# MartinPippel/DAmar

Measured on AMD Instinct MI355X. Metric: aligned base-pairs/sec (daligner block-vs-block), higher is better.
Workload: dtype int32

## Files before the change

damar_amd/csrc/kernels/kernels.h:

```cpp
#ifndef DAMAR_KERNELS_H
#define DAMAR_KERNELS_H

#include "dev_common.h"

size_t damar_scan_workspace_bytes(u64 n);
void   damar_exclusive_scan_u32(const u32 *in, u32 *out, u64 n, void *work, u64 *total_dev, hipStream_t st);
#define DAMAR_SCAN_TILE 4096
void   damar_tile_offsets_u32(const u32 *in, u64 n, void *work, u64 *total_dev, hipStream_t st);
void   damar_scan_tile_counts(u32 *tcount, u32 ntiles, u64 *total_dev, hipStream_t st);
size_t damar_sort_workspace_bytes(u64 n);
void   damar_sort_set_threads(int threads);
const u32 *damar_sort_error_word(const void *work);
int    damar_radix_sort_keys_u64(u64 *k0, u64 *k1, u64 n, int lobit, int hibit, void *work, hipStream_t st);
void   damar_radix_sort_split_u64(u64 *k0, u64 *k1, u64 n, int lobit, int hibit, u32 *ohi, u32 *olo, void *work,
                                  hipStream_t st);
int    damar_radix_sort_u32(u32 *k0, u32 *v0, u32 *k1, u32 *v1, u64 n, int nbits, void *work, hipStream_t st);
int    damar_radix_sort_keys_u32(u32 *k0, u32 *k1, u64 n, int nbits, void *work, hipStream_t st);
int    damar_radix_sort_u64(u64 *k0, u32 *v0, u64 *k1, u32 *v1, u64 n, int nbits, void *work, hipStream_t st);

typedef struct
{ const u8  *bases;
  const u32 *pk;
  u32        rbias;
  const u32 *boff;
  const u32 *coarse;
  u32        nreads;
  u32        total;
  int        maxlen;
  int        rpbits;
  const u32 *moff;
  const int *mdat;
} DevBlock;

#define SEED_PRIO_VAR(name, dflt) static __device__ int name = dflt;  static int name##_host = dflt;
#define SEED_PRIO(name)     do { if (name) __builtin_amdgcn_s_setprio(3); } while (0)
#define SEED_PRIO_SETTER(fn, name) \
  void fn(int on) { if (on != name##_host) { HIP_CHECK(hipMemcpyToSymbol(HIP_SYMBOL(name), &on, sizeof(int)));  name##_host = on; } }

#define COARSE_SHIFT 9
#define PK_PAD 4

#ifdef __HIPCC__
__device__ __forceinline__ u32 read_of_pos(const DevBlock &b, u32 p)
{ u32 r = b.coarse[p >> COARSE_SHIFT];
  while (b.boff[r + 1] <= p)
    r += 1;
  return r;
}
__device__ __forceinline__ void pos_decode(const DevBlock &b, u32 v, u32 *r, u32 *x)
{ if (b.rpbits)
    { *r = v >> b.rpbits;
      *x = v & ((1u << b.rpbits) - 1u);
    }
  else
    { const u32 rr = read_of_pos(b, v);
      *r = rr;
      *x = v - b.boff[rr];
    }
}
__device__ __forceinline__ u32 pos_encode(const DevBlock &b, u32 r, u32 x, u32 p)
{ return b.rpbits ? ((r << b.rpbits) | x) : p; }
#endif

long long damar_pack_words(u32 total);
void damar_launch_pack_bases(const u8 *bases, u32 total, u32 *pk, hipStream_t st);
void damar_launch_unpack_bps(const u8 *raw, const u32 *foff, const DevBlock *blk, int comp, u8 *bases, hipStream_t st);

void damar_preload_index(void);  void damar_preload_scan(void);  void damar_preload_sort(void);
void damar_preload_merge(void);  void damar_preload_report(void);
void damar_sort_set_prio(int on);
void damar_merge_set_prio(int on);
void damar_index_set_prio(int on);
void damar_launch_kmer_tuples(const DevBlock *blk, int kmer, u32 nkmers, void *codes, int wide, u32 *pos, hipStream_t st);
void damar_launch_mask_flags(const DevBlock *blk, int kmer, const u32 *pos, u32 n, u32 *keep, hipStream_t st);
void damar_launch_biased_tuples(const DevBlock *blk, int kmer, const int *logbase, void *codes, int wide, u32 *pos,
                                u32 *keep, hipStream_t st);
void damar_launch_suppress_flags(const void *codes, int wide, u32 n, int suppress, u32 *keep, hipStream_t st);
void damar_launch_compact_pairs(const void *k, int wide, const u32 *v, const u32 *keep, const u32 *off, u32 n,
                                void *ko, u32 *vo, hipStream_t st);

void damar_launch_tandem_links(const DevBlock *blk, int kmer, const void *codes, int wide, const u32 *pos, u32 n,
                               int *dist, hipStream_t st);

typedef struct
{ const void *acode;  const u32 *apos;  u32 alen;
  const void *bcode;  const u32 *bpos;  u32 blen;
  int  wide;
  int  kbits;
  int  self, comp, identity;
  u32  limit;
  DevBlock ablk, bblk;
  int  pbits, abits;
  int  dbits;
} MergeArgs;

typedef struct { u32 b0, b1, ja, ia;
                 u32 sh, pad[3]; } MergeTile;

size_t damar_merge_workspace_bytes(u32 alen);
u32   *damar_merge_tile_counts(void *work, u32 alen);
u32    damar_merge_tiles(u32 alen);
void   damar_launch_merge_count(const MergeArgs *m, void *work, unsigned long long *gram, u32 ngram, hipStream_t st);
void damar_launch_merge_emit(const MergeArgs *m, void *work, u64 nhits, u64 *keys, u32 *vals, u32 *pid, hipStream_t st);
void damar_launch_pair_heads_ids(const u32 *pids, u64 nhits, int abits, int minhit, int nshift,
                                 u64 *send, u64 *bits, void *scan_work, u64 *total_dev, u32 *heads, hipStream_t st);
void damar_launch_pair_bitmap(const u32 *pids, const u32 *heads, u32 nheads, int abits, u32 b_lo, u32 b_hi, u32 *bitmap,
                              hipStream_t st);
void damar_launch_seed_cut_count(const u64 *keys, u64 nhits, int pbits, const u32 *bitmap, u32 *tcount, u64 *total_dev,
                                 hipStream_t st);
void damar_launch_seed_cut_scatter(const u64 *keys, const u32 *vals, u64 nhits, int pbits, const u32 *bitmap,
                                   const u32 *toff, u64 *okeys, u32 *ovals, hipStream_t st);
void damar_launch_pair_heads(const u64 *keys, u64 nhits, int pbits, int abits, int minhit, int nshift,
                             u64 *send , u64 *bits, void *scan_work, u64 *total_dev,
                             u32 *heads, hipStream_t st);
void damar_launch_pair_work(u64 *keys, const u32 *vals, u64 nhits, int ppos, int dbits, int abits, int minhit, int nshift,
                            u64 *send , u64 *bits, void *scan_work, u64 *total_dev ,
                            int binshift, int kmer, int hitmin, u32 b_lo, u32 b_hi, int unsorted, hipStream_t st);
void damar_launch_order_runs(u64 *keys, u64 nhits, int ppos, int dbits, const u32 *work, u32 nwork, hipStream_t st);
void damar_launch_pair_work_expand(const u64 *bits, const void *scan_work, u64 nhits, u32 *work, hipStream_t st);
#define WORK_COST_BITS 16
#define WORK_COST_MAX  ((1u << WORK_COST_BITS) - 1)
void damar_launch_work_cost(const u64 *keys, const u32 *vals, u64 nhits, int pbits, int abits, int dbits, const u32 *aboff,
                            const u32 *bboff, const u32 *work, u32 nwork, u32 coarse, u32 *key, u32 *val, hipStream_t st);
void damar_launch_pair_screen(const u64 *keys, const u32 *vals, u64 nhits, int pbits, int dbits, const u32 *heads, u32 nheads,
                              int minhit, int binshift, int kmer, int hitmin, int abits, u32 b_lo, u32 b_hi, u32 *keep, hipStream_t st);
void damar_launch_compact_u32(const u32 *src, const u32 *keep, const u32 *off, u32 n, u32 *out, hipStream_t st);
void damar_launch_compact_index(const u32 *flags, const u32 *off, u64 n, u32 *out, hipStream_t st);

#ifdef __HIPCC__
__device__ __forceinline__ int seed_diag(u64 k, const u32 *__restrict__ vals, u64 i, u64 pmask, int dbits)
{ if (dbits)
    return (int) ((k >> dbits) & pmask) - (int) (k & ((1ull << dbits) - 1));
  return (int) vals[i];
}
#endif

typedef struct
{ int abpos, bbpos, aepos, bepos, diffs;
  int atlen, btlen;
  int aread, bread;
  u32 item, seq;
  u32 toff;
} LaRecord;

typedef struct
{
  const u64 *keys;  const u32 *vals;  u64 nhits;
  const u32 *work;  u32 nwork;
  DevBlock ablk, bblk;
  int  pbits, abits, dbits;
  int  kmer, hitmin, binshift, minhit;
  int  comp, self, symmetric, minover, hgap_min;
  int  tspace, ave_path, reach;
  const short *score, *table;
  int  mscore, dscore;
  void *state;   u64 state_stride;   int span;
  int  *marks;   u64 marks_stride;
  void *cells;   u32 cell_cap;
  int  *buckets; u64 bucket_stride;  int bwidth;
  int  bucket_bits;
  u16  *ttmp;    u32 ttmp_stride;
  LaRecord *recs;  u32 rec_cap;
  u16  *tpool;     u32 tpool_cap;
  u32  *widemap;
  void *wcells;    u32 wcell_cap;
  u32  cell_max;
  int  t8, t8max;
  const u32 *order;
  u32  *counters;
  u32  *cursor;
  u32  *nfilt;
  int   job;
} ReportArgs;

#define DAMAR_MAX_JOBS 32
#define DAMAR_MAX_TSPACE 8192
#define DAMAR_CNT_CELLS     8
#define DAMAR_CNT_HALFSTEPS 10
#define DAMAR_CNT_ITERS     12
#define DAMAR_CNT_WIDE    14
#define DAMAR_ITEM_WIDE   0x80000000u
#define DAMAR_CNT_CURSOR  16
#define DAMAR_CNT_NFILT   (DAMAR_CNT_CURSOR + DAMAR_MAX_JOBS)
#define DAMAR_COUNTER_WORDS (DAMAR_CNT_NFILT + DAMAR_MAX_JOBS)
#define DAMAR_SEQ_BITS 24

#define DAMAR_ERR_CELLS   1u
#define DAMAR_ERR_RECS    2u
#define DAMAR_ERR_TPOOL   4u
#define DAMAR_ERR_BAND    8u
#define DAMAR_ERR_T8     32u
#define DAMAR_ERR_WIDE   16u

int  damar_report_waves_per_simd(void);
int  damar_report2_waves_per_simd(void);
int  damar_report2_slots_per_wave(void);
void damar_launch_report(const ReportArgs *jobs, int njobs, int nslots, hipStream_t st);
void damar_launch_report_wide(const ReportArgs *jobs, int njobs, int nslots, hipStream_t st);
void damar_launch_tandem_report(const ReportArgs *a, const int *dist, int nslots, hipStream_t st);

typedef struct { int aread, bread, diag, anti; } LaTask;
void damar_launch_la_batch(const ReportArgs *a, const LaTask *tasks, u32 ntasks, int nslots, hipStream_t st);
void damar_launch_report2(const ReportArgs *jobs, int njobs, const LaTask *tasks, u32 ntasks, int nslots, hipStream_t st);
void damar_launch_tandem_report2(const ReportArgs *a, const int *dist, int nslots, hipStream_t st);
void damar_launch_tandem_report_wide(const ReportArgs *a, const int *dist, int nslots, hipStream_t st);
void damar_launch_la_batch_wide(const ReportArgs *a, const LaTask *tasks, u32 ntasks, int nslots, hipStream_t st);
#define DAMAR_MAX_MARKS 16000
#define DAMAR_MAX_CELLS (1u << 18)

u64 damar_report_state_stride(int span);

typedef struct
{ u32 aread, bread;
  u32 flags;
  int abpos, bbpos, aepos, bepos;
  u32 poff;
  int tlen;
  u32 seg0;
  u32 stage0;
  int dmax;
  u32 slots;
} TraceRecIn;

typedef struct
{ u32 apos, bpos;
  int a0, b0;
  u32 mn;
  u32 flags;
  u32 stage;
  u32 rec;
} TraceSeg;

typedef struct
{ const TraceSeg *segs;
  const u32 *list;  u32 nwork;
  const u8 *abases, *bbases;
  const u32 *apk, *bpk;
  short *vf;  signed char *hf;  u32 cap;
  int *stage;  u32 *count;  int *dist;
  int *mid;
  u32 *over;  u32 over_cap;  u32 *nover;  u32 *need;  u32 *err;
  u32 *next;
} TraceArgs;

#define DAMAR_TRACE_ERR_POINTS 1u
#define DAMAR_TRACE_ERR_ALIGN  2u
#define DAMAR_TRACE_ERR_INTERNAL 4u

void damar_launch_trace_layout(const TraceRecIn *recs, u32 nrecs, const void *pts, int tbytes, int tspace,
                               const DevBlock *ablk, const DevBlock *bblk, TraceSeg *segs, u32 *key, u32 *val, u32 *err,
                               hipStream_t st);
void damar_launch_trace_waves(const TraceArgs *t, int mode, int kind, u32 nblocks, hipStream_t st);
size_t damar_trace_slot_area_cells(void);
size_t damar_trace_slot_vf_bytes(int mode, int kind);
void damar_launch_trace_waves_slots(const TraceArgs *t, int mode, int kind, u32 nblocks, hipStream_t st);
void damar_launch_trace_gather(const TraceRecIn *recs, u32 nrecs, int mid, const u32 *count, const int *dist, u32 *segoff,
                               u32 *tlen, int *diffs, hipStream_t st);
void damar_launch_trace_mid_layout(const TraceRecIn *recs, u32 nrecs, const TraceSeg *segs, const int *mid,
                                   const DevBlock *ablk, const DevBlock *bblk, TraceSeg *out, u32 *key, u32 *val, u32 *err,
                                   hipStream_t st);
void damar_launch_trace_pack(const TraceSeg *segs, u32 nsegs, const u32 *count, const u32 *segoff, const u32 *recoff,
                             const int *stage, int *script, hipStream_t st);
#endif
```

damar_amd/csrc/kernels/kmer_index.hip:

```cpp
#include "dev_common.h"
#include "kernels.h"

SEED_PRIO_VAR(g_index_prio, 0)
SEED_PRIO_SETTER(damar_index_set_prio, g_index_prio)


template <typename CodeT, bool PACK>
__global__ __launch_bounds__(256)
void kmer_tuples(DevBlock blk, int kmer, u32 nkmers, CodeT *__restrict__ codes, u32 *__restrict__ pos)
{ SEED_PRIO(g_index_prio);
  const u32 p = blockIdx.x * 256u + threadIdx.x;
  if (p >= blk.total)
    return;
  const u32 r = read_of_pos(blk, p), b0 = blk.boff[r];
  if (p - b0 < (u32) (kmer - 1) || p + 1 == blk.boff[r + 1])
    return;
  const u32 i = p - (r + 1) * (u32) kmer + 1;
  if (i >= nkmers)
    return;
  CodeT c = 0;
  if (PACK)
    {
      const u32 f = p - (u32) (kmer - 1), wq = f >> 4, o = (f & 15) << 1;
      u64 win = ((u64) blk.pk[wq + 1] << 32) | (u64) blk.pk[wq];
      win >>= o;
      u64 r = __brevll(win);
      r = ((r >> 1) & 0x5555555555555555ull) | ((r & 0x5555555555555555ull) << 1);
      c = (CodeT) (r >> (64 - 2 * kmer));
    }
  else
    { const u8 *s = blk.bases + (p - (u32) (kmer - 1));
      for (int j = 0; j < kmer; j++)
        c = (CodeT) (c << 2) | (CodeT) s[j];
    }
  const u32 pw = pos_encode(blk, r, p - b0, p);
  if (PACK)
    codes[i] = (CodeT) ((u64) c << 32) | (CodeT) pw;
  else
    { codes[i] = c;
      pos[i]   = pw;
    }
}

void damar_launch_kmer_tuples(const DevBlock *blk, int kmer, u32 nkmers, void *codes, int wide, u32 *pos, hipStream_t st)
{ if (nkmers == 0)
    return;
  if (wide)
    hipLaunchKernelGGL((kmer_tuples<u64, false>), dim3((blk->total + 255) / 256), dim3(256), 0, st, *blk, kmer, nkmers, (u64 *) codes, pos);
  else if (pos == NULL)
    hipLaunchKernelGGL((kmer_tuples<u64, true>), dim3((blk->total + 255) / 256), dim3(256), 0, st, *blk, kmer, nkmers, (u64 *) codes, pos);
  else
    hipLaunchKernelGGL((kmer_tuples<u32, false>), dim3((blk->total + 255) / 256), dim3(256), 0, st, *blk, kmer, nkmers, (u32 *) codes, pos);
}

__global__ __launch_bounds__(256)
void mask_flags(DevBlock blk, int kmer, const u32 *__restrict__ pos, u32 n, u32 *__restrict__ keep)
{ u32 i = blockIdx.x * 256u + threadIdx.x;
  if (i >= n)
    return;
  u32 r, x;
  pos_decode(blk, pos[i], &r, &x);
  const int e = (int) x, s = e - (kmer - 1);
  u32 lo = blk.moff[r] >> 1, hi = blk.moff[r + 1] >> 1;
  const u32 end = hi;
  while (lo < hi)
    { const u32 mid = (lo + hi) >> 1;
      if (blk.mdat[2 * mid + 1] > s) hi = mid; else lo = mid + 1;
    }
  keep[i] = (lo < end && blk.mdat[2 * lo] <= e) ? 0u : 1u;
}

void damar_launch_mask_flags(const DevBlock *blk, int kmer, const u32 *pos, u32 n, u32 *keep, hipStream_t st)
{ if (n == 0)
    return;
  hipLaunchKernelGGL(mask_flags, dim3((n + 255) / 256), dim3(256), 0, st, *blk, kmer, pos, n, keep);
}

template <typename CodeT>
__global__ __launch_bounds__(64)
void biased_tuples(DevBlock blk, int kmer, int lb0, int lb1, int lb2, int lb3,
                   CodeT *__restrict__ codes, u32 *__restrict__ pos, u32 *__restrict__ keep)
{ const u32 r = blockIdx.x * 64u + threadIdx.x;
  if (r >= blk.nreads)
    return;
  const int  LogNorm = 10000 * kmer, LogThresh = 10000 * (kmer - 2);
  const u64  kmask = (kmer == 32) ? ~0ull : ((1ull << (2 * kmer)) - 1);
  const u32  b0 = blk.boff[r];
  const int  rlen = (int) (blk.boff[r + 1] - b0) - 1;
  const u8  *s = blk.bases + b0;
  const bool masked = blk.moff != NULL;
  const u32  sb = masked ? blk.moff[r] : 0, sf = masked ? blk.moff[r + 1] : 0;
#define LB(x) ((x) == 0 ? lb0 : ((x) == 1 ? lb1 : ((x) == 2 ? lb2 : lb3)))
  for (u32 sa = sb; sa <= sf; sa += 2)
    { int p = (sa == sb) ? 0 : blk.mdat[sa - 1];
      const int q = (sa == sf) ? rlen : blk.mdat[sa];
      if (p + kmer > q)
        continue;
      u64 c = 0;
      int a = 0, k = 1;
      bool stop = false;
      while (p < q)
        { int x = s[p];
          a += LB(x);
          c = (c << 2) | (u64) x;
          while (a < LogNorm && k < kmer)
            { if (++p >= q)
                { stop = !masked;
                  break;
                }
              k += 1;
              x = s[p];
              a += LB(x);
              c = (c << 2) | (u64) x;
            }
          if (stop)
            break;
          for (;;)
            { const int u = a - LB((int) s[p - k + 1]);
              if (u < LogNorm) break;
              a = u;
              k -= 1;
            }
          if (a > LogThresh)
            { const u32 P = b0 + (u32) p;
              codes[P] = (CodeT) ((c << (2 * kmer - 2 * k)) & kmask);
              pos[P]   = pos_encode(blk, r, (u32) p, P);
              keep[P]  = 1u;
            }
          p += 1;
          a -= LB((int) s[p - k]);
        }
    }
#undef LB
}

void damar_launch_biased_tuples(const DevBlock *blk, int kmer, const int *logbase, void *codes, int wide, u32 *pos,
                                u32 *keep, hipStream_t st)
{ if (blk->nreads == 0)
    return;
  if (wide)
    hipLaunchKernelGGL(biased_tuples<u64>, dim3((blk->nreads + 63) / 64), dim3(64), 0, st, *blk, kmer,
                       logbase[0], logbase[1], logbase[2], logbase[3], (u64 *) codes, pos, keep);
  else
    hipLaunchKernelGGL(biased_tuples<u32>, dim3((blk->nreads + 63) / 64), dim3(64), 0, st, *blk, kmer,
                       logbase[0], logbase[1], logbase[2], logbase[3], (u32 *) codes, pos, keep);
}

template <typename CodeT>
__global__ __launch_bounds__(256)
void suppress_flags(const CodeT *__restrict__ codes, u32 n, u32 suppress, u32 *__restrict__ keep)
{ const u32 i = blockIdx.x * 256u + threadIdx.x;
  if (i >= n)
    return;
  const CodeT c = codes[i];
  u32 lo = i, step = 1;
  while (lo >= step && codes[lo - step] == c)
    { lo -= step;
      step <<= 1;
    }
  { u32 a = (lo >= step) ? lo - step + 1 : 0, b = lo;
    while (a < b)
      { const u32 mid = (a + b) >> 1;
        if (codes[mid] == c) b = mid; else a = mid + 1;
      }
    lo = a;
  }
  u32 hi = i;
  step = 1;
  while (hi + step < n && codes[hi + step] == c)
    { hi += step;
      step <<= 1;
    }
  { u32 a = hi, b = (hi + step < n) ? hi + step - 1 : n - 1;
    while (a < b)
      { const u32 mid = (a + b + 1) >> 1;
        if (codes[mid] == c) a = mid; else b = mid - 1;
      }
    hi = a;
  }
  keep[i] = (hi - lo + 1 < suppress) ? 1u : 0u;
}

void damar_launch_suppress_flags(const void *codes, int wide, u32 n, int suppress, u32 *keep, hipStream_t st)
{ if (n == 0)
    return;
  if (wide)
    hipLaunchKernelGGL(suppress_flags<u64>, dim3((n + 255) / 256), dim3(256), 0, st, (const u64 *) codes, n, (u32) suppress, keep);
  else
    hipLaunchKernelGGL(suppress_flags<u32>, dim3((n + 255) / 256), dim3(256), 0, st, (const u32 *) codes, n, (u32) suppress, keep);
}

template <typename CodeT>
__global__ __launch_bounds__(256)
void compact_pairs(const CodeT *__restrict__ k, const u32 *__restrict__ v, const u32 *__restrict__ keep,
                   const u32 *__restrict__ off, u32 n, CodeT *__restrict__ ko, u32 *__restrict__ vo)
{ u32 i = blockIdx.x * 256u + threadIdx.x;
  if (i < n && keep[i])
    { ko[off[i]] = k[i];
      vo[off[i]] = v[i];
    }
}

__global__ __launch_bounds__(256)
void compact_pack(const u32 *__restrict__ k, const u32 *__restrict__ v, const u32 *__restrict__ keep,
                  const u32 *__restrict__ off, u32 n, u64 *__restrict__ ko)
{ u32 i = blockIdx.x * 256u + threadIdx.x;
  if (i < n && keep[i])
    ko[off[i]] = ((u64) k[i] << 32) | (u64) v[i];
}

void damar_launch_compact_pairs(const void *k, int wide, const u32 *v, const u32 *keep, const u32 *off, u32 n,
                                void *ko, u32 *vo, hipStream_t st)
{ if (n == 0)
    return;
  if (wide)
    hipLaunchKernelGGL(compact_pairs<u64>, dim3((n + 255) / 256), dim3(256), 0, st, (const u64 *) k, v, keep, off, n, (u64 *) ko, vo);
  else if (vo == NULL)
    hipLaunchKernelGGL(compact_pack, dim3((n + 255) / 256), dim3(256), 0, st, (const u32 *) k, v, keep, off, n, (u64 *) ko);
  else
    hipLaunchKernelGGL(compact_pairs<u32>, dim3((n + 255) / 256), dim3(256), 0, st, (const u32 *) k, v, keep, off, n, (u32 *) ko, vo);
}

template <typename CodeT>
__global__ __launch_bounds__(256)
void tandem_links(DevBlock blk, int kmer, const CodeT *__restrict__ codes, const u32 *__restrict__ pos, u32 n,
                  int *__restrict__ dist)
{ u32 i = blockIdx.x * 256u + threadIdx.x;
  if (i >= n)
    return;
  u32 r, x;
  pos_decode(blk, pos[i], &r, &x);
  const u32 p = blk.boff[r] + x;
  int d = 0;
  if (i == 0)
    d = (int) codes[0];
  else if (codes[i] == codes[i - 1])
    { u32 rq, xq;
      pos_decode(blk, pos[i - 1], &rq, &xq);
      if (rq == r)
        d = (int) (x - xq);
    }
  dist[p - (r + 1) * (u32) kmer + 1] = d;
}

void damar_launch_tandem_links(const DevBlock *blk, int kmer, const void *codes, int wide, const u32 *pos, u32 n,
                               int *dist, hipStream_t st)
{ if (n == 0)
    return;
  if (wide)
    hipLaunchKernelGGL(tandem_links<u64>, dim3((n + 255) / 256), dim3(256), 0, st, *blk, kmer, (const u64 *) codes, pos, n, dist);
  else
    hipLaunchKernelGGL(tandem_links<u32>, dim3((n + 255) / 256), dim3(256), 0, st, *blk, kmer, (const u32 *) codes, pos, n, dist);
}

__global__ __launch_bounds__(256)
void pack_bases(const u8 *__restrict__ bases, long long nwords, long long total, u32 *__restrict__ pk)
{ long long w = (long long) blockIdx.x * 256 + threadIdx.x - PK_PAD;
  if (w >= nwords - PK_PAD)
    return;
  const u8 *s = bases + 16 * w;
  u32 v = 0, r = 0;
  for (int j = 0; j < 16; j++)
    { v |= (u32) (s[j] & 3) << (2 * j);
      const long long q = total - 1 - (16 * w + j);
      const u32 c = (q >= -64 && q < total + 64) ? (u32) (bases[q] & 3) : 0u;
      r |= c << (2 * j);
    }
  pk[w] = v;
  pk[nwords + w] = r;
}

__global__ __launch_bounds__(256)
void unpack_bps(const u8 *__restrict__ raw, const u32 *__restrict__ foff, DevBlock blk, int comp, u8 *__restrict__ bases)
{ const u32 p0 = (blockIdx.x * 256u + threadIdx.x) * 4u;
  if (p0 >= blk.total)
    return;
  u32 r = read_of_pos(blk, p0);
  u32 b0 = blk.boff[r], len = blk.boff[r + 1] - b0 - 1, fo = foff[r];
  u32 word = 0;
#pragma unroll
  for (int j = 0; j < 4; j++)
    { const u32 p = p0 + (u32) j;
      u32 v = 4;
      if (p < blk.total)
        { if (p >= b0 + len + 1)
            { r += 1;
              b0 = blk.boff[r];  len = blk.boff[r + 1] - b0 - 1;  fo = foff[r];
            }
          const u32 x = p - b0;
          if (x < len)
            { const u32 y = comp ? len - 1 - x : x;
              v = ((u32) raw[fo + (y >> 2)] >> (6 - 2 * (y & 3))) & 3u;
              if (comp)
                v = 3 - v;
            }
        }
      word |= v << (8 * j);
    }
  *(u32 *) (bases + p0) = word;
}

void damar_launch_unpack_bps(const u8 *raw, const u32 *foff, const DevBlock *blk, int comp, u8 *bases, hipStream_t st)
{ if (blk->total == 0)
    return;
  hipLaunchKernelGGL(unpack_bps, dim3((blk->total / 4 + 256) / 256), dim3(256), 0, st, raw, foff, *blk, comp, bases);
}

long long damar_pack_words(u32 total) { return (long long) (total >> 4) + 1 + 2 * PK_PAD; }

void damar_launch_pack_bases(const u8 *bases, u32 total, u32 *pk, hipStream_t st)
{ const long long nwords = damar_pack_words(total);
  hipLaunchKernelGGL(pack_bases, dim3((u32) ((nwords + 255) / 256)), dim3(256), 0, st, bases, nwords, (long long) total, pk);
}

void damar_preload_index(void)
{ hipFuncAttributes fa;
  (void) hipFuncGetAttributes(&fa, (const void *) pack_bases);
}
```

damar_amd/csrc/kernels/radix_sort.hip:

```cpp
#include <atomic>
#include <type_traits>
#include "dev_common.h"
#include "kernels.h"

SEED_PRIO_VAR(g_sort_prio, 1)
SEED_PRIO_SETTER(damar_sort_set_prio, g_sort_prio)

#ifndef OS_THREADS
#define OS_THREADS 1024
#endif
#ifndef OS_MINW
#define OS_MINW    4
#endif
#ifndef OS_RANK_LDS
#define OS_RANK_LDS 1
#endif
#define OS_MINTILE (256 * 8)
#define OS_MAXPASS 8

#define OH_ITEMS   16

#define LB_COUNT   1u
#define LB_PREFIX  2u
#define LB_SPINS   (1u << 24)
#ifndef LB_AHEAD
#define LB_AHEAD   8
#endif

#define WS_HIST    256
#define WS_CTR     (256 + OS_MAXPASS * 256 * 4)
#define WS_LB      16384

template <typename GT> __device__ __forceinline__ GT lb_load(const GT *p)
{ return __hip_atomic_load(p, __ATOMIC_RELAXED, __HIP_MEMORY_SCOPE_AGENT); }
template <typename GT> __device__ __forceinline__ void lb_store(GT *p, GT v)
{ __hip_atomic_store(p, v, __ATOMIC_RELAXED, __HIP_MEMORY_SCOPE_AGENT); }

__device__ __forceinline__ u32 os_scan256(u32 v, u32 *lds4)
{ const int l = lane_id(), w = threadIdx.x >> 6;
  const u32 inc = (u32) wave_incl_scan_i((int) v);
  if (l == 63 && w < 4) lds4[w] = inc;
  __syncthreads();
  u32 base = 0;
  for (int i = 0; i < 4; i++)
    if (i < w) base += lds4[i];
  __syncthreads();
  return base + inc - v;
}


#define OH_THREADS 1024
#define OH_BINMAX  61440

template <typename KeyT>
__global__ __launch_bounds__(OH_THREADS)
void onesweep_hist(const KeyT *__restrict__ keys, u64 n, int lobit, int npass, u64 dsh ,
                   u64 dwd , u32 *__restrict__ ghist, uint4 *__restrict__ clr, u64 clr16)
{ extern __shared__ u32 sh[];
  constexpr u32 nthr = OH_THREADS;
  const int nw = npass * 128 * 32;
  for (int j = threadIdx.x; j < nw; j += nthr)
    sh[j] = 0;
  __syncthreads();
  const u32 c = threadIdx.x & 31u;
  const u64 ntile = (n + (u64) nthr * OH_ITEMS - 1) / ((u64) nthr * OH_ITEMS);
  for (u64 t = blockIdx.x; t < ntile; t += gridDim.x)
    { const u64 base = t * ((u64) nthr * OH_ITEMS);
      KeyT k[OH_ITEMS];
#pragma unroll
      for (int r = 0; r < OH_ITEMS; r++)
        { const u64 i = base + (u64) r * nthr + threadIdx.x;
          k[r] = (i < n) ? keys[i] : (KeyT) 0;
        }
#pragma unroll
      for (int r = 0; r < OH_ITEMS; r++)
        { const u64 i = base + (u64) r * nthr + threadIdx.x;
          if (i < n)
            { const KeyT x = k[r] >> lobit;
              for (int p = 0; p < npass; p++)
                { const u32 d = (u32) (x >> (int) ((dsh >> (8 * p)) & 0xffu)) & (u32) ((dwd >> (8 * p)) & 0xffu);
                  atomicAdd(&sh[((u32) p << 12) + ((d >> 1) << 5) + c], 1u << ((d & 1u) << 4));
                }
            }
        }
    }
  __syncthreads();
  for (int j = threadIdx.x; j < npass * 256; j += nthr)
    { const u32 pl = (u32) j >> 8, d = (u32) j & 0xffu, sft = (d & 1u) << 4;
      u32 sum = 0;
#pragma unroll 8
      for (u32 q = 0; q < 32; q++)
        sum += (sh[(pl << 12) + ((d >> 1) << 5) + ((q + threadIdx.x) & 31u)] >> sft) & 0xffffu;
      if (sum)
        atomicAdd(&ghist[j], sum);
    }
  const uint4 z = make_uint4(0, 0, 0, 0);
  for (u64 i = (u64) blockIdx.x * nthr + threadIdx.x; i < clr16; i += (u64) gridDim.x * nthr)
    clr[i] = z;
}

#define OH_COPIES  8
template <typename KeyT>
__global__ __launch_bounds__(256)
void onesweep_hist8(const KeyT *__restrict__ keys, u64 n, int lobit, int npass, u64 dsh ,
                   u64 dwd , u32 *__restrict__ ghist, uint4 *__restrict__ clr, u64 clr16)
{ SEED_PRIO(g_sort_prio);
  extern __shared__ u32 sh[];
  const int nb = npass * 256 * OH_COPIES;
  for (int j = threadIdx.x; j < nb; j += 256)
    sh[j] = 0;
  __syncthreads();
  const u32 c = threadIdx.x & (OH_COPIES - 1);
  const u64 ntile = (n + 256 * OH_ITEMS - 1) / (256 * OH_ITEMS);
  for (u64 t = blockIdx.x; t < ntile; t += gridDim.x)
    { const u64 base = t * (256 * OH_ITEMS);
      KeyT k[OH_ITEMS];
#pragma unroll
      for (int r = 0; r < OH_ITEMS; r++)
        { const u64 i = base + (u64) r * 256 + threadIdx.x;
          k[r] = (i < n) ? keys[i] : (KeyT) 0;
        }
#pragma unroll
      for (int r = 0; r < OH_ITEMS; r++)
        { const u64 i = base + (u64) r * 256 + threadIdx.x;
          if (i < n)
            { const KeyT x = k[r] >> lobit;
              for (int p = 0; p < npass; p++)
                { const u32 d = (u32) (x >> (int) ((dsh >> (8 * p)) & 0xffu)) & (u32) ((dwd >> (8 * p)) & 0xffu);
                  atomicAdd(&sh[(((u32) p << 8) + d) * OH_COPIES + c], 1u);
                }
            }
        }
    }
  __syncthreads();
  for (int j = threadIdx.x; j < npass * 256; j += 256)
    { u32 s = 0;
#pragma unroll
      for (int q = 0; q < OH_COPIES; q++)
        s += sh[j * OH_COPIES + q];
      if (s)
        atomicAdd(&ghist[j], s);
    }
  const uint4 z = make_uint4(0, 0, 0, 0);
  for (u64 i = (u64) blockIdx.x * 256 + threadIdx.x; i < clr16; i += (u64) gridDim.x * 256)
    clr[i] = z;
}


template <typename KeyT, typename GT, bool HV, bool SPLIT, int TH, int IT>
__global__ __launch_bounds__(TH, (IT <= 8 ? 8 : OS_MINW))
void onesweep_pass(const KeyT *__restrict__ kin, const u32 *__restrict__ vin, KeyT *__restrict__ kout,
                   u32 *__restrict__ vout, u32 *__restrict__ ohi, u64 n, int shift, u32 mask,
                   const u32 *__restrict__ ghist, GT *__restrict__ lb, GT *__restrict__ lbclear,
                   u32 *__restrict__ ctr, u32 *__restrict__ err)
{ SEED_PRIO(g_sort_prio);
  constexpr int OS_TILE = TH * IT, OS_WAVES = TH / 64, OS_WSPAN = 64 * IT;
  __shared__ __attribute__((aligned(16))) KeyT skey[OS_TILE];
  u32 *const sval = (u32 *) skey;
  typedef typename std::conditional<(OS_WAVES > 8), u16, u32>::type CntT;
  __shared__ CntT cnt[OS_WAVES][256];
  __shared__ u32  dstart[256];
  __shared__ u32  gadj[256];
  __shared__ u32  lds4[4];
  __shared__ u32  s_tile;
  constexpr int SH = (int) sizeof(GT) * 8 - 2;
  constexpr GT  VM = (((GT) 1) << SH) - 1;

  const int l = lane_id(), w = threadIdx.x >> 6;
  if (threadIdx.x == 0)
    s_tile = atomicAdd(ctr, 1u);
  for (int i = 0; i < OS_WAVES; i++)
    if (threadIdx.x < 256)
      cnt[i][threadIdx.x] = 0;
#if OS_RANK_LDS
  static_assert((size_t) OS_TILE * sizeof(KeyT) >= (size_t) OS_WAVES * 256 * sizeof(u64), "the rank words do not fit the stage");
  for (int i = threadIdx.x; i < OS_WAVES * 256; i += TH)
    ((u64 *) skey)[i] = 0;
#endif
  __syncthreads();
  const u32 tile  = (u32) __builtin_amdgcn_readfirstlane((int) s_tile);
  const u64 tbase = (u64) tile * OS_TILE;
  const u32 have = (n - tbase < (u64) OS_TILE) ? (u32) (n - tbase) : (u32) OS_TILE;
  const u32 t0 = (u32) w * OS_WSPAN + (u32) l;
  const KeyT *const tin = kin + tbase;

  KeyT key[IT];
  u32  rnk[IT];
#pragma unroll
  for (int r = 0; r < IT; r++)
    { const u32 ti = t0 + (u32) r * 64;
      key[r] = tin[ti < have ? ti : have - 1];
    }
#if OS_RANK_LDS
  u64 *const wmask = (u64 *) skey + (u32) w * 256u;
  const u64 lanebit = 1ull << l;
#pragma unroll
  for (int r = 0; r < IT; r++)
    { const bool ok = t0 + (u32) r * 64 < have;
      const u32  d  = (u32) (key[r] >> shift) & mask;
      if (ok)
        __hip_atomic_fetch_or(&wmask[d], lanebit, __ATOMIC_RELAXED, __HIP_MEMORY_SCOPE_WAVEFRONT);
      __builtin_amdgcn_fence(__ATOMIC_SEQ_CST, "wavefront");
      const u64 peers  = __hip_atomic_load(&wmask[d], __ATOMIC_RELAXED, __HIP_MEMORY_SCOPE_WAVEFRONT);
      const u32 before = cnt[w][d];
      __builtin_amdgcn_fence(__ATOMIC_SEQ_CST, "wavefront");
      const u32 mine   = __builtin_amdgcn_mbcnt_hi((u32) (peers >> 32), __builtin_amdgcn_mbcnt_lo((u32) peers, 0u));
      rnk[r] = before + mine;
      if (ok && mine == 0)
        { cnt[w][d] = (CntT) (before + (u32) __popcll(peers));
          __hip_atomic_store(&wmask[d], 0ull, __ATOMIC_RELAXED, __HIP_MEMORY_SCOPE_WAVEFRONT);
        }
      __builtin_amdgcn_fence(__ATOMIC_SEQ_CST, "wavefront");
    }
#else
#pragma unroll
  for (int r = 0; r < IT; r++)
    { const bool ok = t0 + (u32) r * 64 < have;
      const u32  d  = (u32) (key[r] >> shift) & mask;
      const u64 okm = __ballot(ok);
      u32 plo = (u32) okm, phi = (u32) (okm >> 32);
#pragma unroll
      for (int b = 0; b < 8; b++)
        { const int t  = ((int) (d << (31 - b))) >> 31;
          const u64 nm = ~__ballot(t < 0);
          plo &= (u32) nm ^ (u32) t;
          phi &= (u32) (nm >> 32) ^ (u32) t;
        }
      const u32 before = cnt[w][d];
      const u32 mine   = __builtin_amdgcn_mbcnt_hi(phi, __builtin_amdgcn_mbcnt_lo(plo, 0u));
      rnk[r] = before + mine;
      if (ok && mine == 0)
        cnt[w][d] = (CntT) (before + (u32) __popc(plo) + (u32) __popc(phi));
    }
#endif
  __syncthreads();

  u32 tot = 0;
  if (threadIdx.x < 256)
    { u32 run = 0;
#pragma unroll
      for (int i = 0; i < OS_WAVES; i++)
        { const u32 c = cnt[i][threadIdx.x];
          cnt[i][threadIdx.x] = (CntT) run;
          run += c;
        }
      tot = run;
      lb_store<GT>(&lb[(u64) tile * 256 + threadIdx.x],
                   ((GT) (tile == 0 ? LB_PREFIX : LB_COUNT) << SH) | (GT) tot);
      lbclear[(u64) tile * 256 + threadIdx.x] = 0;
    }
  const u32 dbase = os_scan256(threadIdx.x < 256 ? ghist[threadIdx.x] : 0u, lds4);
  const u32 ex    = os_scan256(tot, lds4);
  if (threadIdx.x < 256)
    dstart[threadIdx.x] = ex;
  __syncthreads();

#pragma unroll
  for (int r = 0; r < IT; r++)
    { if (t0 + (u32) r * 64 < have)
        { const u32 d  = (u32) (key[r] >> shift) & mask;
          const u32 lp = dstart[d] + cnt[w][d] + rnk[r];
          rnk[r] = lp;
          skey[lp] = key[r];
        }
    }

  if (threadIdx.x < 256)
    { GT before = 0;
      if (tile > 0 && threadIdx.x <= mask)
        { u32 t = tile - 1, spins = 0;
#ifdef OS_STATS
          u32 nstep = 0;
#endif
          bool found = false;
          while (!found)
            { GT g[LB_AHEAD];
#pragma unroll
              for (int k = 0; k < LB_AHEAD; k++)
                g[k] = lb_load<GT>(&lb[(u64) (t >= (u32) k ? t - (u32) k : 0u) * 256 + threadIdx.x]);
              int used = LB_AHEAD;
#pragma unroll
              for (int k = 0; k < LB_AHEAD; k++)
                if (used == LB_AHEAD)
                  { const u32 st = (u32) (g[k] >> SH);
                    if (st == 0)
                      used = k;
                    else
                      { before += g[k] & VM;
#ifdef OS_STATS
                        nstep += 1;
#endif
                        if (st == LB_PREFIX)
                          { found = true;  used = -1; }
                      }
                  }
              if (found)
                break;
              t -= (u32) used;
              if (used < LB_AHEAD)
                { if (++spins > LB_SPINS)
                    { atomicOr(err, 1u);
                      break;
                    }
                  __builtin_amdgcn_s_sleep(1);
                }
            }
#ifdef OS_STATS
          if (threadIdx.x == 0)
            { atomicAdd(err + 1, nstep);  atomicAdd(err + 2, spins);  atomicAdd(err + 3, 1u); }
#endif
          lb_store<GT>(&lb[(u64) tile * 256 + threadIdx.x], ((GT) LB_PREFIX << SH) | ((before + tot) & VM));
        }
      gadj[threadIdx.x] = dbase + (u32) before - ex;
    }
  __syncthreads();

  u32 gdst[HV ? IT : 1];
#pragma unroll
  for (int q = 0; q < IT; q++)
    { const u32 i = threadIdx.x + (u32) q * TH;
      if (i < have)
        { const KeyT k = skey[i];
          const u32  d = (u32) (k >> shift) & mask;
          const u32  g = gadj[d] + i;
          if (HV) gdst[q] = g;
          if (SPLIT)
            { ohi[g]  = (u32) ((u64) k >> 32);
              vout[g] = (u32) k;
            }
          else
            kout[g] = k;
        }
    }
  if (HV)
    { const u32 *const tvin = vin + tbase;
      __syncthreads();
#pragma unroll
      for (int r = 0; r < IT; r++)
        { const u32 ti = t0 + (u32) r * 64;
          if (ti < have)
            sval[rnk[r]] = tvin[ti];
        }
      __syncthreads();
#pragma unroll
      for (int q = 0; q < IT; q++)
        { const u32 i = threadIdx.x + (u32) q * TH;
          if (i < have)
            vout[gdst[q]] = sval[i];
        }
    }
}


static int G_sort_threads = 0;

void damar_sort_set_threads(int threads) { G_sort_threads = (threads == 256 || threads == 512) ? threads : 1024; }

static int sort_threads(void)
{ if (G_sort_threads == 0)
    { const char *e = getenv("DAMAR_SORT_THREADS");
      damar_sort_set_threads(e ? atoi(e) : OS_THREADS);
    }
  return G_sort_threads;
}

size_t damar_sort_workspace_bytes(u64 n)
{ const u64 ntiles = (n + OS_MINTILE - 1) / OS_MINTILE;
  return (size_t) WS_LB + 2 * (((size_t) ntiles * 256 * sizeof(u64) + 255) & ~(size_t) 255) + 256;
}

const u32 *damar_sort_error_word(const void *work) { return (const u32 *) work; }

template <typename KeyT, typename GT, bool HV, int TH, int IT>
static void onesweep_passes(KeyT *k0, u32 *v0, KeyT *k1, u32 *v1, u64 n, int lobit, int hibit, u32 *ohi, u32 *olo,
                            char *ws, hipStream_t st)
{ constexpr int OS_TILE = TH * IT;
  const u32 ntiles = (u32) ((n + OS_TILE - 1) / OS_TILE);
  const int npass  = (hibit - lobit + 7) / 8;
  int dshift[OS_MAXPASS], dwidth[OS_MAXPASS];
  u64 dsh = 0, dwd = 0;
  { const int bits = hibit - lobit, base = bits / npass, extra = bits % npass;
    int at = 0;
    static int even = -1;
    if (even < 0)
      { const char *e = getenv("DAMAR_SORT_EVEN");
        even = e ? atoi(e) : 1;
      }
    for (int p = 0; p < npass; p++)
      { dshift[p] = at;
        dwidth[p] = even ? base + (p < extra ? 1 : 0) : (p < npass - 1 ? 8 : bits - 8 * (npass - 1));
        at += dwidth[p];
        dsh |= (u64) dshift[p] << (8 * p);
        dwd |= (u64) ((1u << dwidth[p]) - 1u) << (8 * p);
      }
  }
  const size_t region = ((size_t) ntiles * 256 * sizeof(GT) + 255) & ~(size_t) 255;
  u32 *err = (u32 *) ws, *ghist = (u32 *) (ws + WS_HIST), *ctr = (u32 *) (ws + WS_CTR);
  GT  *lbr[2] = { (GT *) (ws + WS_LB), (GT *) (ws + WS_LB + region) };
  HIP_CHECK(hipMemsetAsync(ws, 0, WS_LB, st));
  if (sort_threads() >= 512)
    { const u64 nt = (n + (u64) OH_THREADS * OH_ITEMS - 1) / ((u64) OH_THREADS * OH_ITEMS);
      const u64 maxit = OH_BINMAX / ((OH_THREADS / 32) * OH_ITEMS);
      u64 grid = nt < 512 ? nt : 512;
      if ((nt + grid - 1) / grid > maxit)
        grid = (nt + maxit - 1) / maxit;
      const size_t lds = (size_t) npass * 128 * 32 * sizeof(u32);
      {
        static std::atomic<unsigned long long> big_lds(0ull);
        int dev = 0;
        HIP_CHECK(hipGetDevice(&dev));
        const unsigned long long bit = 1ull << (dev & 63);
        if (!(big_lds.load(std::memory_order_acquire) & bit))
          { HIP_CHECK(hipFuncSetAttribute((const void *) onesweep_hist<u32>, hipFuncAttributeMaxDynamicSharedMemorySize, 8 * 16384));
            HIP_CHECK(hipFuncSetAttribute((const void *) onesweep_hist<u64>, hipFuncAttributeMaxDynamicSharedMemorySize, 8 * 16384));
            big_lds.fetch_or(bit, std::memory_order_release);
          }
      }
      hipLaunchKernelGGL(onesweep_hist<KeyT>, dim3((u32) grid), dim3(OH_THREADS), lds, st,
                         k0, n, lobit, npass, dsh, dwd, ghist, (uint4 *) lbr[0], (u64) (region / 16));
      HIP_CHECK(hipGetLastError());
    }
  else
    { const u64 nt = (n + 256 * OH_ITEMS - 1) / (256 * OH_ITEMS);
      const u32 grid = (u32) (nt < 2048 ? nt : 2048);
      hipLaunchKernelGGL(onesweep_hist8<KeyT>, dim3(grid), dim3(256), (size_t) npass * 256 * OH_COPIES * sizeof(u32), st,
                         k0, n, lobit, npass, dsh, dwd, ghist, (uint4 *) lbr[0], (u64) (region / 16));
    }
  for (int p = 0; p < npass; p++)
    { const int  side = p & 1;
      const bool last = (p == npass - 1);
      KeyT *ki = side ? k1 : k0, *ko = side ? k0 : k1;
      u32  *vi = side ? v1 : v0, *vo = side ? v0 : v1;
      const u32 mask = (1u << dwidth[p]) - 1u;
      if (last && ohi != NULL)
        hipLaunchKernelGGL((onesweep_pass<KeyT, GT, false, true, TH, IT>), dim3(ntiles), dim3(TH), 0, st,
                           ki, (const u32 *) NULL, (KeyT *) NULL, olo, ohi, n, lobit + dshift[p], mask,
                           ghist + 256 * p, lbr[side], lbr[side ^ 1], ctr + p, err);
      else
        hipLaunchKernelGGL((onesweep_pass<KeyT, GT, HV, false, TH, IT>), dim3(ntiles), dim3(TH), 0, st,
                           ki, vi, ko, vo, (u32 *) NULL, n, lobit + dshift[p], mask,
                           ghist + 256 * p, lbr[side], lbr[side ^ 1], ctr + p, err);
    }
}

template <typename KeyT, bool HV>
static int onesweep_impl(KeyT *k0, u32 *v0, KeyT *k1, u32 *v1, u64 n, int lobit, int hibit, u32 *ohi, u32 *olo,
                         void *work, hipStream_t st)
{ const int npass = (hibit - lobit + 7) / 8;
  if (n == 0 || npass <= 0)
    return 0;
  if (npass > OS_MAXPASS || n >= 0xfffffff0ull)
    { fprintf(stderr, "damar: internal error, radix sort of %llu items on %d bits\n", (unsigned long long) n, hibit - lobit);
      fflush(NULL);
      _exit(1);
    }
  const int shape = sort_threads();
  static int lb64 = -1;
  if (lb64 < 0)
    lb64 = getenv("DAMAR_SORT_LB64") != NULL;
  if (n < (1ull << 30) && !lb64)
    { if (shape == 1024)     onesweep_passes<KeyT, u32, HV, 1024, 8>(k0, v0, k1, v1, n, lobit, hibit, ohi, olo, (char *) work, st);
      else if (shape == 512) onesweep_passes<KeyT, u32, HV, 512, 16>(k0, v0, k1, v1, n, lobit, hibit, ohi, olo, (char *) work, st);
      else              onesweep_passes<KeyT, u32, HV, 256, 16>(k0, v0, k1, v1, n, lobit, hibit, ohi, olo, (char *) work, st);
    }
  else
    onesweep_passes<KeyT, u64, HV, 256, 16>(k0, v0, k1, v1, n, lobit, hibit, ohi, olo, (char *) work, st);
  return npass & 1;
}

int damar_radix_sort_u32(u32 *k0, u32 *v0, u32 *k1, u32 *v1, u64 n, int nbits, void *work, hipStream_t st)
{ return onesweep_impl<u32, true>(k0, v0, k1, v1, n, 0, nbits, NULL, NULL, work, st); }

int damar_radix_sort_keys_u32(u32 *k0, u32 *k1, u64 n, int nbits, void *work, hipStream_t st)
{ return onesweep_impl<u32, false>(k0, NULL, k1, NULL, n, 0, nbits, NULL, NULL, work, st); }

int damar_radix_sort_u64(u64 *k0, u32 *v0, u64 *k1, u32 *v1, u64 n, int nbits, void *work, hipStream_t st)
{ return onesweep_impl<u64, true>(k0, v0, k1, v1, n, 0, nbits, NULL, NULL, work, st); }

int damar_radix_sort_keys_u64(u64 *k0, u64 *k1, u64 n, int lobit, int hibit, void *work, hipStream_t st)
{ return onesweep_impl<u64, false>(k0, NULL, k1, NULL, n, lobit, hibit, NULL, NULL, work, st); }

void damar_radix_sort_split_u64(u64 *k0, u64 *k1, u64 n, int lobit, int hibit, u32 *ohi, u32 *olo, void *work,
                                hipStream_t st)
{ onesweep_impl<u64, false>(k0, NULL, k1, NULL, n, lobit, hibit, ohi, olo, work, st); }

void damar_preload_sort(void)
{ hipFuncAttributes fa;
  (void) hipFuncGetAttributes(&fa, (const void *) onesweep_hist<u64>);
}
```

damar_amd/csrc/kernels/seed_merge.hip:

```cpp
#include "dev_common.h"
#include "kernels.h"

SEED_PRIO_VAR(g_merge_prio, 0)
SEED_PRIO_SETTER(damar_merge_set_prio, g_merge_prio)


__device__ __forceinline__ u32 count_below(const u32 *__restrict__ bpos, u32 jb, u32 ib, u32 bound)
{ u32 a = jb, b = ib;
  while (a < b)
    { u32 m = (a + b) >> 1;
      if (bpos[m] < bound) a = m + 1; else b = m;
    }
  return a - jb;
}


#ifndef MT_PER
#define MT_PER  4
#endif
#define MT_A    (MT_PER * 256)
#define MT_BCAP (3 * MT_A)
#define MT_HITS 4
#define MT_NBK  2048

// ... 281 lines not shown
      { re[k] = (cb == NONE || cb > nat) ? nat : cb;
        if ((hbits >> k) & 1) cb = e0 + k;
      }
  }

  u32 n[MT_PER];
#pragma unroll
  for (int k = 0; k < MT_PER; k++)
    { n[k] = 0;
      if (k < nv && nb[k] > 0)
        { if (!m.self)
            { const u32 ja = rs_open[k] ? tl.ja : a0 + rs[k];
              const u32 ia = (re[k] >= nat) ? tl.ia : a0 + re[k];
              if ((u64) (ia - ja) * (u64) nb[k] < (u64) m.limit)
                n[k] = nb[k];
            }
          else
            n[k] = self_hits(m, m.apos[a0 + e0 + k], tl.b0 + jb[k], nb[k]);
        }
    }

  u64 T64;
  for (int round = 0; ; round++)
    { u32 s = 0;
      u64 s64 = 0;
#pragma unroll
      for (int k = 0; k < MT_PER; k++)
        { s += n[k];  s64 += n[k]; }
      u32 inc = (u32) wave_incl_scan_i((int) s);
      if (l == 63) sw4[w] = inc;
      __syncthreads();
      u32 ex = inc - s;
      for (int i = 0; i < 4; i++)
        if (i < w) ex += sw4[i];
      __syncthreads();
#pragma unroll
      for (int k = 0; k < MT_PER; k++)
        { loc[e0 + k] = ex;
          ex += n[k];
        }
      if (threadIdx.x == 255)
        loc[MT_A] = ex;
      T64 = block_sum_u64(s64, red);
      if (!m.self || round == 1)
        break;
      u64 xhead = 0, xtail = 0;
      if (tl.ja < a0)
        { if (threadIdx.x == 0) { sjb[0] = jb[0];  sjb[1] = nb[0]; }
          __syncthreads();
          const u32 j0 = tl.b0 + sjb[0], nn = sjb[1];
          u64 acc = 0;
          if (nn > 0)
            for (u32 i = tl.ja + threadIdx.x; i < a0; i += 256)
              acc += self_hits(m, m.apos[i], j0, nn);
          xhead = block_sum_u64(acc, red);
        }
      if (tl.ia > a1)
        { const u32 le = nat - 1;
          if (threadIdx.x == le / MT_PER)
            {
#pragma unroll
              for (int k = 0; k < MT_PER; k++)
                if (k == (int) (le % MT_PER)) { sjb[0] = jb[k];  sjb[1] = nb[k]; }
            }
          __syncthreads();
          const u32 j0 = tl.b0 + sjb[0], nn = sjb[1];
          u64 acc = 0;
          if (nn > 0)
            for (u32 i = a1 + threadIdx.x; i < tl.ia; i += 256)
              acc += self_hits(m, m.apos[i], j0, nn);
          xtail = block_sum_u64(acc, red);
        }
#pragma unroll
      for (int k = 0; k < MT_PER; k++)
        if (k < nv && nb[k] > 0)
          { u64 tot = (u64) (loc[re[k]] - loc[rs[k]]);
            if (rs_open[k]) tot += xhead;
            if (re[k] >= nat) tot += xtail;
            if (gram != NULL && ((hbits >> k) & 1) && tot < (u64) m.limit && tot < (u64) ngram)
              atomicAdd(&gram[tot], 1ull);
            if (tot >= (u64) m.limit)
              n[k] = 0;
          }
      __syncthreads();
    }

  if (!m.self && gram != NULL)
    {
#pragma unroll
      for (int k = 0; k < MT_PER; k++)
        if (k < nv && nb[k] > 0 && ((hbits >> k) & 1))
          { const u32 ia = (re[k] >= nat) ? tl.ia : a0 + re[k];
            const u64 ct = (u64) (ia - (a0 + e0 + k)) * (u64) nb[k];
            if (ct < (u64) ngram)
              atomicAdd(&gram[ct], 1ull);
          }
    }
  if (threadIdx.x == 0)
    tcount[tile] = (T64 > 0xffffffffull) ? 0xffffffffu : (u32) T64;
  typedef u32 V4 __attribute__((ext_vector_type(4)));
  if (nv == MT_PER && MT_PER == 4)
    { V4 vc, vj;
#pragma unroll
      for (int k = 0; k < 4; k++)
        { vc[k] = n[k];  vj[k] = tl.b0 + jb[k]; }
      *(V4 *) (cnt + a0 + e0) = vc;
      *(V4 *) (jbg + a0 + e0) = vj;
    }
  else
    {
#pragma unroll
      for (int k = 0; k < MT_PER; k++)
        if (k < nv)
          { cnt[a0 + e0 + k] = n[k];
            jbg[a0 + e0 + k] = tl.b0 + jb[k];
          }
    }
}

static_assert(MT_BCAP + 16 < (1 << 16), "a packed entry holds the piece-relative start and the hits in 16 bits each");
struct MergeFastArgs
{ const void *acode, *bcode;
  const u32  *apos, *bpos;
  u32 alen, blen;
  int self, identity, comp, rpbits;
};

template <typename CodeT>
__global__ __launch_bounds__(256, 8)
void merge_fast(MergeFastArgs m, MergeTile *__restrict__ tiles, u32 *__restrict__ tcount, u32 *__restrict__ cnt)
{ SEED_PRIO(g_merge_prio);
  __shared__ __attribute__((aligned(16))) CodeT sb[MT_BCAP + 16 / sizeof(CodeT)];
  __shared__ __attribute__((aligned(16))) u16 first[MT_NBK];
  __shared__ u32 wsum[4];
  __shared__ u32 deep;
  const CodeT *acode = (const CodeT *) m.acode, *bcode = (const CodeT *) m.bcode;
  const u32 tile = blockIdx.x;
  const MergeTile tl = tiles[tile];
  const u32 a0 = tile * (u32) MT_A, a1 = min(m.alen, a0 + (u32) MT_A), nat = a1 - a0;
  const u32 nbt = tl.b1 - tl.b0;
  if (nbt > MT_BCAP || (m.self && m.rpbits == 0))
    { if (threadIdx.x == 0)
        tiles[tile].pad[0] = 1;
      return;
    }
  const u32 e0 = threadIdx.x * MT_PER;
  const int nv = (e0 >= nat) ? 0 : (int) min((u32) MT_PER, nat - e0);
  const u32 sh = tl.sh, nmax = tl.pad[1];
  constexpr u32 VPK = 16 / sizeof(CodeT);
  typedef CodeT VecT __attribute__((ext_vector_type(16 / sizeof(CodeT))));
  typedef u32 V4 __attribute__((ext_vector_type(4)));

  const CodeT c0 = acode[a0];
  CodeT a[MT_PER];
  if (nv == MT_PER)
    {
#pragma unroll
      for (int q = 0; q < MT_PER / (int) VPK; q++)
        { const VecT v = ((const VecT *) (acode + a0 + e0))[q];
#pragma unroll
          for (int e = 0; e < (int) VPK; e++)
            a[q * VPK + e] = v[e];
        }
    }
  else
    {
#pragma unroll
      for (int k = 0; k < MT_PER; k++)
        a[k] = (k < nv) ? acode[a0 + e0 + k] : (CodeT) 0;
    }
  const u32 b0a = tl.b0 & ~(VPK - 1), shf = tl.b0 - b0a;
  { const u32 nvec = (tl.b1 - b0a + VPK - 1) / VPK;
    const u32 whole = (m.blen - b0a) / VPK;
    VecT v[MT_BCAP / (int) VPK / 256 + 1];
#pragma unroll
    for (int r = 0; r < MT_BCAP / (int) VPK / 256 + 1; r++)
      { const u32 x = threadIdx.x + (u32) r * 256;
        if (x < nvec)
          { if (x < whole)
              v[r] = ((const VecT *) (bcode + b0a))[x];
            else
              {
#pragma unroll
                for (int e = 0; e < (int) VPK; e++)
                  v[r][e] = (b0a + x * VPK + e < m.blen) ? bcode[b0a + x * VPK + e] : (CodeT) 0;
              }
          }
      }
    { const V4 ones = { 0xffffffffu, 0xffffffffu, 0xffffffffu, 0xffffffffu };
      ((V4 *) first)[threadIdx.x] = ones;
    }
    if (threadIdx.x == 0)
      deep = 0;
#pragma unroll
    for (int r = 0; r < MT_BCAP / (int) VPK / 256 + 1; r++)
      { const u32 x = threadIdx.x + (u32) r * 256;
        if (x < nvec)
          ((VecT *) sb)[x] = v[r];
      }
  }
  const CodeT *B = sb + shf;
  __syncthreads();
  for (u32 j = threadIdx.x; j < nbt; j += 256)
    { const u32 bk = (u32) ((B[j] - c0) >> sh);
      if (j == 0 || (u32) ((B[j - 1] - c0) >> sh) != bk)
        first[bk] = (u16) j;
    }
  __syncthreads();

  u32 jb[MT_PER], n[MT_PER];
  u32 longest = 0;
#pragma unroll
  for (int k = 0; k < MT_PER; k++)
    { jb[k] = 0;  n[k] = 0;
      if (k < nv)
        { const CodeT c = a[k];
          if (k > 0 && c == a[k - 1])
            { jb[k] = jb[k - 1];  n[k] = n[k - 1]; }
          else
            { u32 p = first[(u32) ((c - c0) >> sh)];
              if (p != 0xffffu)
                { int steps = 0;
                  while (p < nbt && B[p] < c)
                    { p += 1;
                      if (++steps == 4) { p = lower_bound_c<CodeT>(B, p, nbt, c);  break; }
                    }
                  u32 q = p;
                  steps = 0;
                  while (q < nbt && B[q] == c)
                    { q += 1;
                      if (++steps == 4) { q = upper_bound_c<CodeT>(B, q, nbt, c);  break; }
                    }
                  jb[k] = p;  n[k] = q - p;
                }
            }
          longest = max(longest, n[k]);
        }
    }
  if (longest > nmax)
    deep = 1;
  u32 sum = 0;
  if (m.self)
    { const int rp = m.rpbits;
#pragma unroll
      for (int k = 0; k < MT_PER; k++)
        if (n[k] > 0)
          { const u32 p = m.apos[a0 + e0 + k], ra = p >> rp;
            u32 bound = m.identity ? (m.comp ? (ra + 1) << rp : p) : ra << rp;
            if (!(m.identity && m.comp && ((ra + 1) >> (32 - rp)) != 0))
              n[k] = count_below(m.bpos, tl.b0 + jb[k], tl.b0 + jb[k] + n[k], bound);
          }
    }
#pragma unroll
  for (int k = 0; k < MT_PER; k++)
    sum += n[k];
  sum = (u32) wave_sum_i((int) sum);
  if (lane_id() == 0)
    wsum[threadIdx.x >> 6] = sum;
  __syncthreads();
  if (deep)
    { if (threadIdx.x == 0)
        tiles[tile].pad[0] = 1;
      return;
    }
  if (threadIdx.x == 0)
    { tcount[tile] = wsum[0] + wsum[1] + wsum[2] + wsum[3];
      tiles[tile].pad[2] = 1;
    }
  if (nv == MT_PER && MT_PER == 4)
    { V4 vc;
#pragma unroll
      for (int k = 0; k < 4; k++)
        vc[k] = (n[k] << 16) | jb[k];
      *(V4 *) (cnt + a0 + e0) = vc;
    }
  else
    {
#pragma unroll
      for (int k = 0; k < MT_PER; k++)
        if (k < nv)
          cnt[a0 + e0 + k] = (n[k] << 16) | jb[k];
    }
}

template <typename CodeT>
__global__ __launch_bounds__(256, 8)
void merge_sweep(MergeArgs m, const MergeTile *__restrict__ tiles, u32 *__restrict__ tcount, u32 *__restrict__ cnt,
                 u32 *__restrict__ jbg, unsigned long long *__restrict__ gram, u32 ngram, int only_flagged)
{ SEED_PRIO(g_merge_prio);
  __shared__ __attribute__((aligned(16))) CodeT sb[MT_BCAP + 16 / sizeof(CodeT)];
  __shared__ u32 loc[MT_A + 1];
  __shared__ u32 sjb[2];
  __shared__ u32 sw4[4];
  __shared__ u64 red[4];
  const MergeTile tl = tiles[blockIdx.x];
  if (only_flagged && tl.pad[0] == 0)
    return;
  if (tl.b1 - tl.b0 <= MT_BCAP)
    merge_sweep_tile<CodeT, true>(m, tl, blockIdx.x, tcount, cnt, jbg, gram, ngram, sb, loc, sjb, sw4, red);
  else
    merge_sweep_tile<CodeT, false>(m, tl, blockIdx.x, tcount, cnt, jbg, gram, ngram, sb, loc, sjb, sw4, red);
}

__global__ __launch_bounds__(256, 8)
void merge_emit(MergeArgs m, const MergeTile *__restrict__ tiles, const u32 *__restrict__ cnt, const u32 *__restrict__ jbg,
                const u32 *__restrict__ toff, u64 nhits, u64 *__restrict__ keys, u32 *__restrict__ vals, u32 *__restrict__ pid)
{ SEED_PRIO(g_merge_prio);
  __shared__ u32 loc[MT_A + 1];
  __shared__ u32 sjb[MT_A];
  __shared__ u32 sw4[4];
  const int l = lane_id(), w = threadIdx.x >> 6;
  const u32 tile = blockIdx.x;
  const u32 a0 = tile * (u32) MT_A, a1 = min(m.alen, a0 + (u32) MT_A), nat = a1 - a0;
  const u32 e0 = threadIdx.x * MT_PER;
  const u64 h0 = toff[tile];
  const u64 hn = (tile + 1 < gridDim.x) ? (u64) toff[tile + 1] : nhits;
  if (hn == h0)
    return;
  u32 n[MT_PER], s = 0;
  const bool packed = tiles[tile].pad[2] != 0;
  const u32 pb0 = tiles[tile].b0;
#pragma unroll
  for (int k = 0; k < MT_PER; k++)
    { const bool ok = e0 + k < nat;
      const u32 w = ok ? cnt[a0 + e0 + k] : 0;
      n[k] = packed ? w >> 16 : w;
      sjb[e0 + k] = !ok ? 0 : packed ? pb0 + (w & 0xffffu) : jbg[a0 + e0 + k];
      s += n[k];
    }
  u32 inc = (u32) wave_incl_scan_i((int) s);
  if (l == 63) sw4[w] = inc;
  __syncthreads();
  u32 ex = inc - s;
  for (int i = 0; i < 4; i++)
    if (i < w) ex += sw4[i];
#pragma unroll
  for (int k = 0; k < MT_PER; k++)
    { loc[e0 + k] = ex;
      ex += n[k];
    }
  if (threadIdx.x == 255)
    loc[MT_A] = ex;
  __syncthreads();
  const u32 T = loc[MT_A];
  for (u32 t0 = threadIdx.x; t0 < T; t0 += 256 * MT_HITS)
    { u32 ai[MT_HITS], bi[MT_HITS], pa[MT_HITS], pb[MT_HITS];
#pragma unroll
      for (int x = 0; x < MT_HITS; x++)
        { const u32 t = t0 + (u32) x * 256;
          u32 lo = 0, hi = MT_A;
          if (t < T)
            while (hi - lo > 1)
              { const u32 mid = (lo + hi) >> 1;
                if (loc[mid] <= t) lo = mid; else hi = mid;
              }
          ai[x] = a0 + lo;
          bi[x] = (t < T) ? sjb[lo] + (t - loc[lo]) : 0;
        }
#pragma unroll
      for (int x = 0; x < MT_HITS; x++)
        { const bool ok = t0 + (u32) x * 256 < T;
          pa[x] = ok ? m.apos[ai[x]] : 0;
          pb[x] = ok ? m.bpos[bi[x]] : 0;
        }
      u32 ra[MT_HITS], rb[MT_HITS], xa[MT_HITS], xb[MT_HITS];
      if (m.ablk.rpbits && m.bblk.rpbits)
        {
#pragma unroll
          for (int x = 0; x < MT_HITS; x++)
            { ra[x] = pa[x] >> m.ablk.rpbits;  xa[x] = pa[x] & ((1u << m.ablk.rpbits) - 1u);
              rb[x] = pb[x] >> m.bblk.rpbits;  xb[x] = pb[x] & ((1u << m.bblk.rpbits) - 1u);
            }
        }
      else
        {
#pragma unroll
          for (int x = 0; x < MT_HITS; x++)
            { pos_decode(m.ablk, pa[x], &ra[x], &xa[x]);
              pos_decode(m.bblk, pb[x], &rb[x], &xb[x]);
            }
        }
#pragma unroll
      for (int x = 0; x < MT_HITS; x++)
        { const u32 t = t0 + (u32) x * 256;
          const u64 h = h0 + t;
          if (t < T && h < nhits)
            { const u64 key = ((u64) rb[x] << (m.abits + m.pbits)) | ((u64) ra[x] << m.pbits) | (u64) xa[x];
              if (m.dbits)
                keys[h] = (key << m.dbits) | (u64) xb[x];
              else
                { keys[h] = key;
                  vals[h] = (u32) ((int) xa[x] - (int) xb[x]);
                }
              if (pid != NULL)
                pid[h] = (rb[x] << m.abits) | ra[x];
            }
        }
    }
}

static size_t mw_tiles(u32 alen)  { return ((size_t) alen + MT_A - 1) / MT_A; }
static size_t mw_off_counts(u32 alen) { return (mw_tiles(alen) * sizeof(MergeTile) + 255) & ~(size_t) 255; }
static size_t mw_off_cnt(u32 alen)    { return mw_off_counts(alen) + (((mw_tiles(alen) + 1) * sizeof(u32) + 255) & ~(size_t) 255); }
static size_t mw_off_jb(u32 alen)     { return mw_off_cnt(alen) + (((size_t) alen * sizeof(u32) + 255) & ~(size_t) 255); }

size_t damar_merge_workspace_bytes(u32 alen)
{ return mw_off_jb(alen) + (((size_t) alen * sizeof(u32) + 255) & ~(size_t) 255); }

u32 *damar_merge_tile_counts(void *work, u32 alen) { return (u32 *) ((char *) work + mw_off_counts(alen)); }

u32 damar_merge_tiles(u32 alen) { return (u32) mw_tiles(alen); }

void damar_launch_merge_count(const MergeArgs *m, void *work, unsigned long long *gram, u32 ngram, hipStream_t st)
{ if (m->alen == 0)
    return;
  const u32 ntiles = (u32) mw_tiles(m->alen);
  MergeTile *tiles = (MergeTile *) work;
  u32 *tcount = damar_merge_tile_counts(work, m->alen);
  u32 *cnt = (u32 *) ((char *) work + mw_off_cnt(m->alen)), *jb = (u32 *) ((char *) work + mw_off_jb(m->alen));
  static int general = -1;
  if (general < 0)
    general = getenv("DAMAR_MERGE_GENERAL") != NULL;
  const bool fast = gram == NULL && !general;
  MergeFastArgs f;
  f.acode = m->acode;  f.bcode = m->bcode;  f.apos = m->apos;  f.bpos = m->bpos;  f.alen = m->alen;  f.blen = m->blen;
  f.self = m->self;  f.identity = m->identity;  f.comp = m->comp;  f.rpbits = m->ablk.rpbits;
  if (m->wide)
    { hipLaunchKernelGGL(merge_tiles<u64>, dim3((ntiles + 255) / 256), dim3(256), 0, st, *m, ntiles, tiles);
      if (fast)
        hipLaunchKernelGGL(merge_fast<u64>, dim3(ntiles), dim3(256), 0, st, f, tiles, tcount, cnt);
      hipLaunchKernelGGL(merge_sweep<u64>, dim3(ntiles), dim3(256), 0, st, *m, tiles, tcount, cnt, jb, gram, ngram, fast ? 1 : 0);
    }
  else
    { hipLaunchKernelGGL(merge_tiles<u32>, dim3((ntiles + 255) / 256), dim3(256), 0, st, *m, ntiles, tiles);
      if (fast)
        hipLaunchKernelGGL(merge_fast<u32>, dim3(ntiles), dim3(256), 0, st, f, tiles, tcount, cnt);
      hipLaunchKernelGGL(merge_sweep<u32>, dim3(ntiles), dim3(256), 0, st, *m, tiles, tcount, cnt, jb, gram, ngram, fast ? 1 : 0);
    }
}

void damar_launch_merge_emit(const MergeArgs *m, void *work, u64 nhits, u64 *keys, u32 *vals, u32 *pid, hipStream_t st)
{ if (nhits == 0)
    return;
  const u32 ntiles = (u32) mw_tiles(m->alen);
  const u32 *toff = damar_merge_tile_counts(work, m->alen);
  const u32 *cnt = (const u32 *) ((char *) work + mw_off_cnt(m->alen)), *jb = (const u32 *) ((char *) work + mw_off_jb(m->alen));
  hipLaunchKernelGGL(merge_emit, dim3(ntiles), dim3(256), 0, st, *m, (const MergeTile *) work, cnt, jb, toff, nhits, keys, vals, pid);
}

#define SCREEN_MAX   48
#define SCREEN_PANEL 50000
template <typename K>
__global__ __launch_bounds__(64)
void slice_ends(const K *__restrict__ keys, u64 nhits, int bshift, int nshift, u64 *__restrict__ send)
{ const int nthr = 1 << nshift, t = threadIdx.x;
  if (t >= nthr)
    return;
  u64 e;
  if (t == nthr - 1)
    e = nhits;
  else
    { e = (nhits * (u64) (t + 1)) >> nshift;
      if (e > 0)
        { u64 d = keys[e - 1] >> bshift, a = e, b = nhits;
          while (a < b)
            { u64 mid = (a + b) >> 1;
              if ((keys[mid] >> bshift) == d) a = mid + 1; else b = mid;
            }
          e = a;
        }
    }
  send[t] = e;
}

#define PH_ROUNDS (DAMAR_SCAN_TILE / 256)
template <typename K>
__global__ __launch_bounds__(256)
void pair_heads_mark(const K *__restrict__ keys, u64 nhits, int pbits, int minhit, int nshift,
                     const u64 *__restrict__ send, u64 *__restrict__ bits, u32 *__restrict__ tcount)
{ SEED_PRIO(g_merge_prio);
  __shared__ u32 wsum[4];
  const int nthr = nshift < 0 ? 0 : 1 << nshift;
  const int l = lane_id(), w = threadIdx.x >> 6;
  const u64 base = (u64) blockIdx.x * DAMAR_SCAN_TILE;
  u32 mine = 0;
  u64 e0 = ~0ull, e1 = ~0ull;
  for (int t = 0; t < nthr; t++)
    { const u64 e = send[t];
      if (e > base)
        { e0 = e;
          if (t + 1 < nthr)
            e1 = send[t + 1];
          break;
        }
    }
  for (int r0 = 0; r0 < PH_ROUNDS; r0 += 4)
    { K k0[4], km[4], kp[4];
#pragma unroll
      for (int q = 0; q < 4; q++)
        { const u64 i = base + (u64) (r0 + q) * 256u + threadIdx.x;
          const u64 ic = i < nhits ? i : nhits - 1;
          const u64 ip = ic + (u64) (minhit - 1);
          k0[q] = keys[ic];
          km[q] = keys[ic > 0 ? ic - 1 : 0];
          kp[q] = keys[ip < nhits ? ip : nhits - 1];
        }
#pragma unroll
      for (int q = 0; q < 4; q++)
        { const int r = r0 + q;
          const u64 i = base + (u64) r * 256u + threadIdx.x;
          bool f = false;
          if (i < nhits)
            { const K pr = k0[q] >> pbits;
              if ((i == 0 || (km[q] >> pbits) != pr) && i + (u64) (minhit - 1) < nhits && (kp[q] >> pbits) == pr)
                { f = true;
                  if (i < e0)
                    { if (i + (u64) minhit >= e0) f = false; }
                  else if (i < e1)
                    { if (i + (u64) minhit >= e1) f = false; }
                  else
                    for (int t = 0; t < nthr; t++)
                      { u64 e = send[t];
                        if (i < e)
                          { if (i + (u64) minhit >= e) f = false;
                            break;
                          }
                      }
                }
            }
          const u64 m = __ballot(f);
          if (l == 0)
            { bits[(base >> 6) + (u64) r * 4 + w] = m;
              mine += (u32) __popcll(m);
            }
        }
    }
  if (l == 0) wsum[w] = mine;
  __syncthreads();
  if (threadIdx.x == 0)
    tcount[blockIdx.x] = wsum[0] + wsum[1] + wsum[2] + wsum[3];
}

__global__ __launch_bounds__(64)
void pair_heads_expand(const u64 *__restrict__ bits, const u32 *__restrict__ toff, u32 *__restrict__ heads)
{ const u64 wi = (u64) blockIdx.x * 64u + threadIdx.x;
  u64 m = bits[wi];
  const int c = __popcll(m);
  u32 o = toff[blockIdx.x] + (u32) (wave_incl_scan_i(c) - c);
  const u32 first = (u32) (wi << 6);
  while (m)
    { const int b = __ffsll((long long) m) - 1;
      m &= m - 1;
      heads[o++] = first + (u32) b;
    }
}

template <typename K>
static void pair_heads_impl(const K *keys, u64 nhits, int pbits, int abits, int minhit, int nshift,
                            u64 *send , u64 *bits, void *scan_work, u64 *total_dev,
                            u32 *heads, hipStream_t st)
{ if (nhits == 0)
    { HIP_CHECK(hipMemsetAsync(total_dev, 0, sizeof(u64), st));
      return;
    }
  if (nshift > 6)
    nshift = 6;
  const u32 ntiles = (u32) ((nhits + DAMAR_SCAN_TILE - 1) / DAMAR_SCAN_TILE);
  u32 *tcount = (u32 *) scan_work;
  if (nshift >= 0)
    hipLaunchKernelGGL(slice_ends<K>, dim3(1), dim3(64), 0, st, keys, nhits, abits + pbits, nshift, send);
  hipLaunchKernelGGL(pair_heads_mark<K>, dim3(ntiles), dim3(256), 0, st, keys, nhits, pbits, minhit, nshift, send, bits, tcount);
  damar_scan_tile_counts(tcount, ntiles, total_dev, st);
  hipLaunchKernelGGL(pair_heads_expand, dim3(ntiles), dim3(64), 0, st, bits, tcount, heads);
}

void damar_launch_pair_heads(const u64 *keys, u64 nhits, int pbits, int abits, int minhit, int nshift,
                             u64 *send, u64 *bits, void *scan_work, u64 *total_dev, u32 *heads, hipStream_t st)
{ pair_heads_impl<u64>(keys, nhits, pbits, abits, minhit, nshift, send, bits, scan_work, total_dev, heads, st);
}


void damar_launch_pair_heads_ids(const u32 *pids, u64 nhits, int abits, int minhit, int nshift,
                                 u64 *send, u64 *bits, void *scan_work, u64 *total_dev, u32 *heads, hipStream_t st)
{ pair_heads_impl<u32>(pids, nhits, 0, abits, minhit, nshift, send, bits, scan_work, total_dev, heads, st);
}

__global__ __launch_bounds__(256)
void pair_bitmap_set(const u32 *__restrict__ pids, const u32 *__restrict__ heads, u32 nheads, int abits, u32 b_lo, u32 b_hi,
                     u32 *__restrict__ bitmap)
{ const u32 t = blockIdx.x * 256u + threadIdx.x;
  if (t >= nheads)
    return;
  const u32 p = pids[heads[t]], rb = p >> abits;
  if (rb < b_lo || rb >= b_hi)
    return;
  atomicOr(&bitmap[p >> 5], 1u << (p & 31));
}

void damar_launch_pair_bitmap(const u32 *pids, const u32 *heads, u32 nheads, int abits, u32 b_lo, u32 b_hi, u32 *bitmap,
                              hipStream_t st)
{ if (nheads == 0)
    return;
  hipLaunchKernelGGL(pair_bitmap_set, dim3((nheads + 255) / 256), dim3(256), 0, st, pids, heads, nheads, abits, b_lo, b_hi, bitmap);
}

__global__ __launch_bounds__(256)
void seed_cut_count(const u64 *__restrict__ keys, u64 nhits, int pbits, const u32 *__restrict__ bitmap, u32 *__restrict__ tcount)
{ __shared__ u32 wsum[4];
  const int l = lane_id(), w = threadIdx.x >> 6;
  const u64 base = (u64) blockIdx.x * DAMAR_SCAN_TILE;
  u32 mine = 0;
  for (int r = 0; r < PH_ROUNDS; r++)
    { const u64 i = base + (u64) r * 256u + threadIdx.x;
      bool f = false;
      if (i < nhits)
        { const u32 p = (u32) (keys[i] >> pbits);
          f = (bitmap[p >> 5] >> (p & 31)) & 1;
        }
      mine += (u32) __popcll(__ballot(f));
    }
  if (l == 0) wsum[w] = mine;
  __syncthreads();
  if (threadIdx.x == 0)
    tcount[blockIdx.x] = wsum[0] + wsum[1] + wsum[2] + wsum[3];
}

__global__ __launch_bounds__(256)
void seed_cut_scatter(const u64 *__restrict__ keys, const u32 *__restrict__ vals, u64 nhits, int pbits,
                      const u32 *__restrict__ bitmap, const u32 *__restrict__ toff, u64 *__restrict__ okeys, u32 *__restrict__ ovals)
{ __shared__ u32 wsum[PH_ROUNDS][4];
  const int l = lane_id(), w = threadIdx.x >> 6;
  const u64 base = (u64) blockIdx.x * DAMAR_SCAN_TILE;
  u64 key[PH_ROUNDS];
  u64 mask[PH_ROUNDS];
  for (int r = 0; r < PH_ROUNDS; r++)
    { const u64 i = base + (u64) r * 256u + threadIdx.x;
      bool f = false;
      key[r] = 0;
      if (i < nhits)
        { key[r] = keys[i];
          const u32 p = (u32) (key[r] >> pbits);
          f = (bitmap[p >> 5] >> (p & 31)) & 1;
        }
      mask[r] = __ballot(f);
      if (l == 0) wsum[r][w] = (u32) __popcll(mask[r]);
    }
  __syncthreads();
  u32 o = toff[blockIdx.x];
  for (int r = 0; r < PH_ROUNDS; r++)
    { u32 before = 0;
      for (int x = 0; x < 4; x++)
        { const u32 c = wsum[r][x];
          if (x < w) before += c;
        }
      const u64 i = base + (u64) r * 256u + threadIdx.x;
      if ((mask[r] >> l) & 1)
        { const u32 g = o + before + (u32) __popcll(mask[r] & lanes_below(l));
          okeys[g] = key[r];
          if (vals != NULL)
            ovals[g] = vals[i];
        }
      o += wsum[r][0] + wsum[r][1] + wsum[r][2] + wsum[r][3];
    }
}

void damar_launch_seed_cut_count(const u64 *keys, u64 nhits, int pbits, const u32 *bitmap, u32 *tcount, u64 *total_dev,
                                 hipStream_t st)
{ const u32 ntiles = (u32) ((nhits + DAMAR_SCAN_TILE - 1) / DAMAR_SCAN_TILE);
  hipLaunchKernelGGL(seed_cut_count, dim3(ntiles), dim3(256), 0, st, keys, nhits, pbits, bitmap, tcount);
  damar_scan_tile_counts(tcount, ntiles, total_dev, st);
}

void damar_launch_seed_cut_scatter(const u64 *keys, const u32 *vals, u64 nhits, int pbits, const u32 *bitmap,
                                   const u32 *toff, u64 *okeys, u32 *ovals, hipStream_t st)
{ const u32 ntiles = (u32) ((nhits + DAMAR_SCAN_TILE - 1) / DAMAR_SCAN_TILE);
  hipLaunchKernelGGL(seed_cut_scatter, dim3(ntiles), dim3(256), 0, st, keys, vals, nhits, pbits, bitmap, toff, okeys, ovals);
}

__global__ __launch_bounds__(256)
void pair_screen(const u64 *__restrict__ keys, const u32 *__restrict__ vals, u64 nhits, int pbits, int dbits,
                 const u32 *__restrict__ heads, u32 nheads, int minhit, int binshift, int kmer, int hitmin,
                 int abits, u32 b_lo, u32 b_hi, u32 *__restrict__ keep)
{ SEED_PRIO(g_merge_prio);
  u32 t = blockIdx.x * 256u + threadIdx.x;
  if (t >= nheads)
    return;
  const u64 i = heads[t];
  const u64 pmask = (1ull << pbits) - 1;
  pbits += dbits;
  const u64 pr = keys[i] >> pbits;
  u32 f = 1;
  int n = minhit;
  { const u32 rb = (u32) (pr >> abits);
    if (rb < b_lo || rb >= b_hi)
      { keep[t] = 0;
        return;
      }
  }
  while (n <= SCREEN_MAX && i + (u64) n < nhits && (keys[i + (u64) n] >> pbits) == pr)
    n += 1;
  if (n <= SCREEN_MAX && (int) ((keys[i + (u64) (n - 1)] >> dbits) & pmask) <= SCREEN_PANEL)
    { bool ok = false;
      int dlast = 0x7fffffff;
      for (int x = 0; x < n && !ok; x++)
        { const int dx = seed_diag(keys[i + (u64) x], vals, i + (u64) x, pmask, dbits) >> binshift;
          if (dx == dlast)
            continue;
          dlast = dx;
          int s0 = 0, s1 = 0, p0 = 0, p1 = 0;
          for (int y = 0; y < n; y++)
            { const u64 ky = keys[i + (u64) y];
              const int dy = seed_diag(ky, vals, i + (u64) y, pmask, dbits) >> binshift;
              const int ap = (int) ((ky >> dbits) & pmask);
              if (dy == dx)
                { s0 += (ap - p0 >= kmer) ? kmer : ap - p0;  p0 = ap; }
              else if (dy == dx + 1)
                { s1 += (ap - p1 >= kmer) ? kmer : ap - p1;  p1 = ap; }
            }
          ok = s0 + s1 >= hitmin;
        }
      if (!ok)
        f = 0;
    }
  keep[t] = f;
}

void damar_launch_pair_screen(const u64 *keys, const u32 *vals, u64 nhits, int pbits, int dbits, const u32 *heads, u32 nheads,
                              int minhit, int binshift, int kmer, int hitmin, int abits, u32 b_lo, u32 b_hi,
                              u32 *keep, hipStream_t st)
{ if (nheads == 0)
    return;
  hipLaunchKernelGGL(pair_screen, dim3((nheads + 255) / 256), dim3(256), 0, st, keys, vals, nhits, pbits, dbits, heads, nheads,
                     minhit, binshift, kmer, hitmin, abits, b_lo, b_hi, keep);
}

#define PW_HALO 64
#define PW_SMALL 8
#define PW_SHORT 4

template <int N, bool UNS>
__device__ __forceinline__ bool pw_screen_small(const u64 *run, int n, u64 pmask, int dbits, int binshift, int kmer, int hitmin)
{ int d[N], c[N];
  const u64 dmask = (1ull << dbits) - 1;
  int top = 0;
#pragma unroll
  for (int q = 0; q < N; q++)
    { const u64 k = run[q < n ? q : 0];
      c[q] = (int) ((k >> dbits) & pmask);
      d[q] = (q < n) ? ((c[q] - (int) (k & dmask)) >> binshift) : 0x40000000 + 4 * q;
      if (UNS)
// ... 476 lines not shown
```

damar_amd/csrc/shim.hip:

```cpp
#include <algorithm>
#include <vector>
#include <deque>
#include <string>
#include <thread>
#include <atomic>
#include <mutex>
#include <condition_variable>
#include <functional>
#include <string.h>
#include <unistd.h>

#include "kernels/dev_common.h"
#include <ctype.h>
#include "kernels/kernels.h"

extern "C" {
#include "damar_filter.h"
#include "damar_hip.h"
#include "host/damar_host.h"
}

#define MAXGRAM 10000

static void die(void)
// ... 339 lines not shown

static int G_debug = -1;
static void stage(const char *name)
{ if (G_debug < 0)
    G_debug = (getenv("DAMAR_DEBUG") != NULL);
  if (G_debug)
    { hipError_t e = hipStreamSynchronize(G_st);
      fprintf(stderr, "[damar] stage %-14s %s\n", name, hipGetErrorName(e));
      fflush(stderr);
    }
}
static void stream_wait(hipStream_t st)
{ static int spin = -1;
  if (spin < 0)
    { const char *e = getenv("DAMAR_SYNC_SPIN");
      spin = e ? atoi(e) : 0;
    }
  if (spin)
    { hipError_t q;
      while ((q = hipStreamQuery(st)) == hipErrorNotReady)
        __builtin_ia32_pause();
      HIP_CHECK(q);
      return;
    }
  HIP_CHECK(hipStreamSynchronize(st));
}

static void  tick(int i)            { HIP_CHECK(hipEventRecord(G_ev[i], G_st)); }
static void  tick_on(int i, hipStream_t st) { HIP_CHECK(hipEventRecord(G_ev[i], st)); }
static float lap(int i, int j)      { float ms = 0; HIP_CHECK(hipEventElapsedTime(&ms, G_ev[i], G_ev[j])); return ms; }

extern "C" void damar_last_timings(double *ms)  { memcpy(ms, G_ms, sizeof(G_ms)); }
extern "C" void damar_last_counters(int64 *c)   { memcpy(c, G_cnt, sizeof(G_cnt)); }
extern "C" int  damar_last_limit(void)          { return G_limit; }


struct damar_dev_block
{ DevBlock d;
  float freq[4];
  int   minlen;
  u32 *pk_alloc;
  u32 *moff;
  int *mdat;
  u8  *bases_alloc;
  u32 *boff, *coarse;
  int  nreads;
};

static damar_dev_block *block_upload_on(const HITS_DB *block, hipStream_t st, const damar_packed *pk = NULL, int comp = 0);

extern "C" damar_dev_block *damar_block_upload(const HITS_DB *block)
{ ensure_init();
  return block_upload_on(block, G_st);
}

static std::mutex PL_mu;
static std::vector<std::pair<const void *, damar_dev_block *>> PL_ready;
static hipStream_t PL_st = NULL;
static std::atomic<int> PL_state(0);
static hipStream_t preload_stream(void)
{ int s = PL_state.load(std::memory_order_acquire);
  if (s == 2)
    return PL_st;
  int zero = 0;
  if (s == 0 && PL_state.compare_exchange_strong(zero, 1))
    { HIP_CHECK(hipStreamCreateWithFlags(&PL_st, hipStreamNonBlocking));
      PL_state.store(2, std::memory_order_release);
      return PL_st;
    }
  while (PL_state.load(std::memory_order_acquire) != 2)
    usleep(50);
  return PL_st;
}

extern "C" void damar_block_preload(const HITS_DB *block)
{ ensure_init();
  HIP_CHECK(hipSetDevice(G_device));
  (void) preload_stream();
  damar_dev_block *b = block_upload_on(block, PL_st);
  std::lock_guard<std::mutex> lk(PL_mu);
  PL_ready.push_back(std::make_pair((const void *) block->bases, b));
}

extern "C" damar_dev_block *damar_block_upload_bg(const HITS_DB *block)
{ ensure_init();
  HIP_CHECK(hipSetDevice(G_device));
  (void) preload_stream();
  return block_upload_on(block, PL_st);
}

static std::mutex PK_mu;
static std::vector<std::pair<const HITS_READ *, const damar_packed *>> PK_reg;

extern "C" damar_dev_block *damar_block_upload_packed(const HITS_DB *block, const damar_packed *pk, int comp)
{ ensure_init();
  HIP_CHECK(hipSetDevice(G_device));
  (void) preload_stream();
  { std::lock_guard<std::mutex> lk(PK_mu);
    bool have = false;
    for (auto &e : PK_reg)
      if (e.first == block->reads)
        { e.second = pk;  have = true; }
    if (!have)
      PK_reg.push_back(std::make_pair((const HITS_READ *) block->reads, pk));
  }
  return block_upload_on(block, PL_st, pk, comp);
}

extern "C" void damar_packed_forget(const HITS_DB *block)
{ std::lock_guard<std::mutex> lk(PK_mu);
  for (size_t i = 0; i < PK_reg.size(); i++)
    if (PK_reg[i].first == block->reads)
      { PK_reg.erase(PK_reg.begin() + i);
        break;
      }
}

static const char *host_read(const HITS_DB *block, int r, int comp, std::vector<char> &buf)
{ if (block->bases != NULL)
    return (const char *) block->bases + block->reads[r].boff;
  const damar_packed *pk = NULL;
  { std::lock_guard<std::mutex> lk(PK_mu);
    for (auto &e : PK_reg)
      if (e.first == block->reads)
        pk = e.second;
  }
  if (pk == NULL)
    { fprintf(stderr, "damar: internal error, a block without bases that was never uploaded packed\n");
      die();
    }
  buf.resize((size_t) block->reads[r].rlen + 2);
  damar_unpack_read(pk, block, r, comp, buf.data() + 1);
  return buf.data() + 1;
}

static damar_dev_block *take_preloaded(const HITS_DB *block)
{ std::lock_guard<std::mutex> lk(PL_mu);
  for (size_t i = 0; i < PL_ready.size(); i++)
    if (PL_ready[i].first == (const void *) block->bases)
      { damar_dev_block *b = PL_ready[i].second;
        PL_ready.erase(PL_ready.begin() + i);
        return b;
      }
  return NULL;
}

struct PackStage { u8 *raw; size_t nraw; u32 *foff; size_t nfoff; int64 holds; };
static thread_local PackStage TL_stage = { NULL, 0, NULL, 0, 0 };

static damar_dev_block *block_upload_on(const HITS_DB *block, hipStream_t st, const damar_packed *pk, int comp)
{ damar_dev_block *b = (damar_dev_block *) calloc(1, sizeof(damar_dev_block));
  int    n = block->nreads;
  int64  total = block->reads[n].boff;
  if (total > 0x7fffffffll)
    { fprintf(stderr, "damar: Fatal error, DB blocks are greater than 2Gbp!\n");
      die();
    }
  std::vector<u32> boff((size_t) n + 1);
  for (int i = 0; i <= n; i++)
    boff[i] = (u32) block->reads[i].boff;
  int minlen = 0x7fffffff;
  for (int i = 0; i < n; i++)
    minlen = std::min(minlen, (int) (boff[i + 1] - boff[i]) - 1);
  size_t nq = ((size_t) total >> COARSE_SHIFT) + 2;
  std::vector<u32> coarse(nq);
  { u32 r = 0;
    for (size_t q = 0; q < nq; q++)
      { u64 p = (u64) q << COARSE_SHIFT;
        while (r + 1 < (u32) n && (u64) boff[r + 1] <= p)
          r += 1;
        coarse[q] = r;
      }
  }
  b->bases_alloc = (u8 *) dmalloc((size_t) total + 192);
  HIP_CHECK(hipMemsetAsync(b->bases_alloc, 4, (size_t) total + 192, st));
  b->boff   = (u32 *) dmalloc(sizeof(u32) * ((size_t) n + 1));
  b->coarse = (u32 *) dmalloc(sizeof(u32) * nq);
  if (pk == NULL)
    HIP_CHECK(hipMemcpyAsync(b->bases_alloc + 63, ((const char *) block->bases) - 1, (size_t) total + 1,
                             hipMemcpyHostToDevice, st));
  HIP_CHECK(hipMemcpyAsync(b->boff, boff.data(), sizeof(u32) * ((size_t) n + 1), hipMemcpyHostToDevice, st));
  HIP_CHECK(hipMemcpyAsync(b->coarse, coarse.data(), sizeof(u32) * nq, hipMemcpyHostToDevice, st));
  if (pk != NULL)
    {
      DevBlock tmp;
      memset(&tmp, 0, sizeof(tmp));
      tmp.boff = b->boff;  tmp.coarse = b->coarse;  tmp.total = (u32) total;  tmp.nreads = (u32) n;
      if (TL_stage.holds != pk->serial)
        { if (TL_stage.nraw < (size_t) pk->nraw + 64)
            { if (TL_stage.raw) HIP_CHECK(hipFree(TL_stage.raw));
              TL_stage.nraw = (size_t) pk->nraw + ((size_t) pk->nraw >> 3) + 4096;
              TL_stage.raw  = (u8 *) dmalloc(TL_stage.nraw);
            }
          if (TL_stage.nfoff < (size_t) n + 1)
            { if (TL_stage.foff) HIP_CHECK(hipFree(TL_stage.foff));
              TL_stage.nfoff = (size_t) n + ((size_t) n >> 3) + 1024;
              TL_stage.foff  = (u32 *) dmalloc(sizeof(u32) * TL_stage.nfoff);
            }
          HIP_CHECK(hipMemcpyAsync(TL_stage.raw, pk->raw, (size_t) pk->nraw, hipMemcpyHostToDevice, st));
          HIP_CHECK(hipMemcpyAsync(TL_stage.foff, pk->foff, sizeof(u32) * (size_t) n, hipMemcpyHostToDevice, st));
          TL_stage.holds = pk->serial;
        }
      damar_launch_unpack_bps(TL_stage.raw, TL_stage.foff, &tmp, comp, b->bases_alloc + 64, st);
    }
  HIP_CHECK(hipStreamSynchronize(st));
  b->d.bases  = b->bases_alloc + 64;
  b->pk_alloc = (u32 *) dmalloc(sizeof(u32) * 2 * (size_t) damar_pack_words((u32) total));
  b->d.pk     = b->pk_alloc + PK_PAD;
  b->d.rbias  = (u32) (16 * damar_pack_words((u32) total) + 16 * PK_PAD);
  damar_launch_pack_bases(b->d.bases, (u32) total, b->pk_alloc + PK_PAD, st);
  HIP_CHECK(hipStreamSynchronize(st));
  b->d.boff   = b->boff;
  b->d.coarse = b->coarse;
  for (int i = 0; i < 4; i++)
    b->freq[i] = block->freq[i];
  b->minlen = minlen;
  b->d.nreads = (u32) n;
  b->d.total  = (u32) total;
  b->d.maxlen = block->maxlen;
  { const int pb = std::max(1, ilog2_ceil((u64) block->maxlen + 1)), ab = std::max(1, ilog2_ceil((u64) n));
    static int rp_on = -1;
    if (rp_on < 0)
      { const char *e = getenv("DAMAR_PACK_POS");
        rp_on = e ? atoi(e) : 1;
      }
    b->d.rpbits = (rp_on && pb + ab <= 32 && pb < 32) ? pb : 0;
  }
  if (block->tracks != NULL)
    { const int64 *anno = (const int64 *) block->tracks->anno;
      const int   *data = (const int *) block->tracks->data;
      std::vector<u32> moff((size_t) n + 1);
      for (int i = 0; i <= n; i++)
        moff[i] = (u32) anno[i];
      b->moff = (u32 *) dmalloc(sizeof(u32) * ((size_t) n + 1));
      b->mdat = (int *) dmalloc(sizeof(int) * ((size_t) anno[n] + 2));
      HIP_CHECK(hipMemcpyAsync(b->moff, moff.data(), sizeof(u32) * ((size_t) n + 1), hipMemcpyHostToDevice, st));
      if (anno[n] > 0)
        HIP_CHECK(hipMemcpyAsync(b->mdat, data, sizeof(int) * (size_t) anno[n], hipMemcpyHostToDevice, st));
      HIP_CHECK(hipStreamSynchronize(st));
      b->d.moff = b->moff;
      b->d.mdat = b->mdat;
    }
  b->nreads   = n;
  return b;
}


extern "C" void damar_block_free(damar_dev_block *b)
{ if (b == NULL)
    return;
  finish_all();
  HIP_CHECK(hipStreamSynchronize(G_st));
  HIP_CHECK(hipFree(b->bases_alloc));
  HIP_CHECK(hipFree(b->pk_alloc));
  if (b->moff) HIP_CHECK(hipFree(b->moff));
  if (b->mdat) HIP_CHECK(hipFree(b->mdat));
  HIP_CHECK(hipFree(b->boff));
  HIP_CHECK(hipFree(b->coarse));
  free(b);
}


struct damar_dev_index
{ size_t codes_bytes, pos_bytes;
  damar_dev_block *blk;
  int   own_block;
  void *codes;
  u32  *pos;
  u32   n;
  int   kbits, wide;
};

static u32 *H_serr = NULL;
static int  H_nserr = 0;
static void sort_verify(void)
{ for (int i = 0; i < H_nserr; i++)
    if (H_serr[i] != 0)
      { fprintf(stderr, "damar: FATAL: the radix sort's look-back timed out\n");
        die();
      }
  H_nserr = 0;
}
static void sort_check(const void *sw)
{ if (H_serr == NULL)
    HIP_CHECK(hipHostMalloc((void **) &H_serr, 64 * sizeof(u32), hipHostMallocDefault));
  if (H_nserr == 64)
    { HIP_CHECK(hipStreamSynchronize(G_st));
      sort_verify();
    }
  HIP_CHECK(hipMemcpyAsync(&H_serr[H_nserr++], damar_sort_error_word(sw), sizeof(u32), hipMemcpyDeviceToHost, G_st));
}

static bool overlap_on(void);
static bool corun_on(void);
static void pick_sort_shape(void)
{ static int forced = -1;
  if (forced < 0)
    { const char *e = getenv("DAMAR_SORT_THREADS");
      forced = e ? atoi(e) : 0;
    }
  damar_sort_set_threads(forced ? forced : 1024);
}

static int ilog2_ceil(u64 n)
{ int b = 0;
  while ((1ull << b) < n)
    b += 1;
  return b;
}

static int  B_have = 0, B_log[4];

extern "C" void damar_bias_reset(void) { B_have = 0; }

static damar_dev_index *index_build_k(damar_dev_block *blk, int own_block, int *len, int K, int suppress, int use_bias)
{ ensure_init();
  pick_sort_shape();
  if (K > 32)
    { fprintf(stderr, "damar: FATAL: -k%d: a k-mer code holds at most 32 bases\n", K);
      die();
    }
  if (blk->nreads > 0 && blk->minlen < K)
    { fprintf(stderr, "[ERROR] - daligner: Block contains reads < %dbp long !  Run DBsplit.\n", K);
      die();
    }
  int64 nk64 = (int64) blk->d.total - (int64) K * blk->nreads;
  if (nk64 <= 0)
    { *len = 0;
      if (own_block)
        damar_block_free(blk);
      return NULL;
    }
  u32 nk = (u32) nk64;
  const int kbits = 2 * K;
  const int wide = K > 16;
  const size_t cs = wide ? sizeof(u64) : sizeof(u32);
  const bool masked = blk->d.moff != NULL;
  const bool biased = use_bias != 0;
  if (biased && !B_have)
    { const double scale = -10000. / log(4.);
      for (int i = 0; i < 4; i++)
        B_log[i] = (int) ceil(scale * log((double) blk->freq[i]));
      B_have = 1;
    }
  const u32 cap = biased ? blk->d.total : nk;
  const int npass = (kbits + 7) / 8;
  damar_dev_index *ix = (damar_dev_index *) calloc(1, sizeof(damar_dev_index));
  ix->blk = blk;  ix->own_block = own_block;  ix->kbits = kbits;  ix->wide = wide;
  if (wide)
    { ix->codes = dpool_get(cs * (size_t) cap, &ix->codes_bytes);
      ix->pos   = (u32 *) dpool_get(sizeof(u32) * (size_t) cap, &ix->pos_bytes);
    }
  else
    { ix->codes = dpool_get(2 * sizeof(u32) * (size_t) cap, &ix->codes_bytes);
      ix->pos   = (u32 *) ix->codes + cap;
    }

  size_t swb = damar_sort_workspace_bytes(cap);
  arena_reserve(&G_work, pad256(sizeof(u64) * (size_t) cap) + 3 * pad256(sizeof(u32) * (size_t) cap) + pad256(swb) +
                         pad256(damar_scan_workspace_bytes(cap)) + (1 << 16));
  void *tk = arena_take(&G_work, sizeof(u64) * (size_t) cap);
  u32 *tv = (u32 *) arena_take(&G_work, sizeof(u32) * (size_t) cap);
  void *sw = arena_take(&G_work, swb);
  u32 *keep = NULL, *off = NULL;
  void *scw = NULL;
  u64 *tot = NULL;
  if (masked || biased || suppress > 0)
    { keep = (u32 *) arena_take(&G_work, sizeof(u32) * (size_t) cap);
      off  = (u32 *) arena_take(&G_work, sizeof(u32) * (size_t) cap);
      scw  = arena_take(&G_work, damar_scan_workspace_bytes(cap));
      tot  = (u64 *) arena_take(&G_work, 64);
    }

  void *k0, *k1;
  u32  *v0, *v1;
  if (wide)
    { k0 = (npass & 1) ? tk : ix->codes;  k1 = (npass & 1) ? ix->codes : tk;
      v0 = (npass & 1) ? tv : ix->pos;    v1 = (npass & 1) ? ix->pos : tv;
    }
  else
    { k0 = (npass & 1) ? tk : ix->codes;  k1 = (npass & 1) ? ix->codes : tk;
      v0 = v1 = NULL;
    }

  tick(0);
  if (biased || masked)
    {
      void *k9 = k1;
      u32  *v9 = wide ? ((v0 == tv) ? ix->pos : tv) : (u32 *) k1 + cap;
      u64   kept = 0;
      u32   nin = nk;
      if (biased)
        { nin = cap;
          HIP_CHECK(hipMemsetAsync(keep, 0, sizeof(u32) * (size_t) cap, G_st));
          damar_launch_biased_tuples(&blk->d, K, B_log, k9, wide, v9, keep, G_st);
        }
      else
        { damar_launch_kmer_tuples(&blk->d, K, nk, k9, wide, v9, G_st);
          damar_launch_mask_flags(&blk->d, K, v9, nk, keep, G_st);
        }
      damar_exclusive_scan_u32(keep, off, nin, scw, tot, G_st);
      damar_launch_compact_pairs(k9, wide, v9, keep, off, nin, k0, v0, G_st);
      HIP_CHECK(hipMemcpyAsync(&kept, tot, sizeof(u64), hipMemcpyDeviceToHost, G_st));
      HIP_CHECK(hipStreamSynchronize(G_st));
      nk = (u32) kept;
      if (nk == 0)
        { damar_index_free(ix);
          *len = 0;
          return NULL;
        }
      if (VERBOSE && biased)
        printf("\n   Revised kmer count = %u\n", nk);
    }
  else
    damar_launch_kmer_tuples(&blk->d, K, nk, k0, wide, v0, G_st);
  tick(1);
  if (wide)
    { int side = damar_radix_sort_u64((u64 *) k0, v0, (u64 *) k1, v1, nk, kbits, sw, G_st);
      if ((side ? k1 : k0) != ix->codes)
        { fprintf(stderr, "damar: internal error, sort ended on the wrong side\n");
          die();
        }
    }
  else
    damar_radix_sort_split_u64((u64 *) k0, (u64 *) k1, nk, 32, 32 + kbits, (u32 *) ix->codes, ix->pos, sw, G_st);
  sort_check(sw);
  tick(2);
  u32 n = nk;
  if (suppress > 0)
    { u64  kept = 0;
      damar_launch_suppress_flags(ix->codes, wide, n, suppress, keep, G_st);
      damar_exclusive_scan_u32(keep, off, n, scw, tot, G_st);
      damar_launch_compact_pairs(ix->codes, wide, ix->pos, keep, off, n, tk, tv, G_st);
      HIP_CHECK(hipMemcpyAsync(&kept, tot, sizeof(u64), hipMemcpyDeviceToHost, G_st));
      HIP_CHECK(hipStreamSynchronize(G_st));
      n = (u32) kept;
      HIP_CHECK(hipMemcpyAsync(ix->codes, tk, cs * (size_t) n, hipMemcpyDeviceToDevice, G_st));
      HIP_CHECK(hipMemcpyAsync(ix->pos, tv, sizeof(u32) * (size_t) n, hipMemcpyDeviceToDevice, G_st));
    }
  tick(3);
  HIP_CHECK(hipStreamSynchronize(G_st));
  sort_verify();
  G_ms[DAMAR_T_TUPLES] = lap(0, 1);
  G_ms[DAMAR_T_KSORT]  = lap(1, 2);
  G_ms[DAMAR_T_TABLE]  = lap(2, 3);
  ix->n = n;
  if (VERBOSE)
    { printf("\n   Kmer count = %u\n   Index occupies %.2fGb of HBM\n", n, ((cs + 4.) * n) / 1073741824.);
      fflush(stdout);
    }
  if (n == 0)
    { damar_index_free(ix);
      *len = 0;
      return NULL;
    }
  *len = (int) n;
  return ix;
}

extern "C" damar_dev_index *damar_index_build(damar_dev_block *blk, int own_block, int *len)
{ double t0 = now_ms();
  damar_dev_index *ix = index_build_k(blk, own_block, len, P_kmer, P_suppress, BIASED);
  H_ms[0] += now_ms() - t0;
  return ix;
}

extern "C" void damar_index_free(damar_dev_index *ix)
{ if (ix == NULL)
    return;
  HIP_CHECK(hipStreamSynchronize(G_st));
  dpool_put(ix->codes, ix->codes_bytes);
  if (ix->pos_bytes)
    dpool_put(ix->pos, ix->pos_bytes);
  if (ix->own_block)
    damar_block_free(ix->blk);
  free(ix);
}

extern "C" void damar_hbm_info(uint64_t *free_bytes, uint64_t *total_bytes)
{ ensure_init();
  size_t f = 0, t = 0;
  HIP_CHECK(hipMemGetInfo(&f, &t));
  if (free_bytes)  *free_bytes = (uint64_t) f + (uint64_t) DP_bytes;
  if (total_bytes) *total_bytes = (uint64_t) t;
}

extern "C" uint64_t damar_block_bytes(const damar_dev_block *b)
{ if (b == NULL)
    return 0;
  const uint64_t tot = b->d.total;
  return tot + 128 + (tot >> 2) + 64 + sizeof(u32) * ((uint64_t) b->nreads + 1) + sizeof(u32) * ((tot >> COARSE_SHIFT) + 2);
}

extern "C" void damar_pool_trim(void)
{ finish_all();
  HIP_CHECK(hipStreamSynchronize(G_st));
  for (size_t i = 0; i < DP_free.size(); i++)
    HIP_CHECK(hipFree(DP_free[i].p));
  DP_free.clear();
  DP_bytes = 0;
}

extern "C" uint64_t damar_index_bytes(const damar_dev_index *ix)
{ return ix == NULL ? 0 : (uint64_t) (ix->codes_bytes + ix->pos_bytes); }

extern "C" void damar_index_download(const damar_dev_index *ix, void *out)
{ struct KP { uint64 code; int rpos; int read; } *kp = (KP *) out;
  std::vector<u32> pos(ix->n), boff((size_t) ix->blk->nreads + 1);
  std::vector<u64> codes(ix->n);
  if (ix->wide)
    HIP_CHECK(hipMemcpy(codes.data(), ix->codes, sizeof(u64) * (size_t) ix->n, hipMemcpyDeviceToHost));
  else
    { std::vector<u32> c32(ix->n);
      HIP_CHECK(hipMemcpy(c32.data(), ix->codes, sizeof(u32) * (size_t) ix->n, hipMemcpyDeviceToHost));
      for (u32 i = 0; i < ix->n; i++)
        codes[i] = c32[i];
    }
  HIP_CHECK(hipMemcpy(pos.data(), ix->pos, sizeof(u32) * (size_t) ix->n, hipMemcpyDeviceToHost));
  HIP_CHECK(hipMemcpy(boff.data(), ix->blk->boff, sizeof(u32) * boff.size(), hipMemcpyDeviceToHost));
  const int rp = ix->blk->d.rpbits;
  for (u32 i = 0; i < ix->n; i++)
    { kp[i].code = codes[i];
      if (rp)
        { kp[i].rpos = (int) (pos[i] & ((1u << rp) - 1u));
          kp[i].read = (int) (pos[i] >> rp);
        }
      else
        { u32 r = (u32) (std::upper_bound(boff.begin(), boff.end(), pos[i]) - boff.begin()) - 1;
          kp[i].rpos = (int) (pos[i] - boff[r]);
          kp[i].read = (int) r;
        }
    }
}

extern "C" void *Sort_Kmers(HITS_DB *block, int *len)
{
  damar_dev_block *b = take_preloaded(block);
  if (b == NULL)
    b = damar_block_upload(block);
  return (void *) damar_index_build(b, 1, len);
}


struct ReportScratch
{ int nslots_wanted; int   nslots, span, bwidth;
  u32   cell_cap;
  u32   ttmp_stride;
  void *state;  int *marks;  void *cells;  int *buckets;  u16 *ttmp;
  u64   state_stride, marks_stride, bucket_stride;
  short *tables;
  const void *tables_of;
  u32  *counters;
  LaRecord *recs;  u32 rec_cap;
  u16  *tpool;     u32 tpool_cap;
  u32  *ctr;
  LaRecord *recs_set[2];  u16 *tpool_set[2];  u32 rec_cap_set[2], tpool_cap_set[2];  int cur;
  u32  *widemap[2];  u32 widemap_cap[2];
  void *wcells;  u32 wcell_cap;  int wslots;
};
static ReportScratch RS = {};

static bool overlap_on(void);
static bool corun_on(void);

static int default_slots(void)
{ const char *e = getenv("DAMAR_SLOTS");
  if (e && atoi(e) > 0)
    return atoi(e);
  if (const char *w = getenv("DAMAR_REPORT_WPS"))
    if (atoi(w) > 0)
      return G_prop.multiProcessorCount * 4 * damar_report2_slots_per_wave() * std::min(atoi(w), damar_report2_waves_per_simd());
  if (corun_on())
    return G_prop.multiProcessorCount * 4 * damar_report2_slots_per_wave() * (damar_report2_waves_per_simd() >= 8 ? 8 : std::min(4, damar_report2_waves_per_simd()));
  return G_prop.multiProcessorCount * 4 * std::max(damar_report_waves_per_simd(), damar_report2_slots_per_wave() * damar_report2_waves_per_simd());
}

static int G_ring = 0;
#define DEFAULT_CELLS (1u << 13)

static u32 max_cells(void)
{ static u32 m = 0;
  if (m == 0)
    { const char *e = getenv("DAMAR_TEST_MAX_CELLS");
      m = (e && atoi(e) >= 16) ? std::min<u32>((u32) atoi(e), DAMAR_MAX_CELLS) : DAMAR_MAX_CELLS;
    }
  return m;
}

static u32 grow_cells(u32 cell_cap)
{ if (cell_cap >= max_cells())
    { fprintf(stderr, "damar: FATAL: an alignment needs more than %u trace pebbles; use a larger trace spacing (-s)\n", max_cells());
      die();
    }
  return std::min(cell_cap * 4, max_cells());
}

static void marks_must_fit(int amax, int bmax, int tspace)
{ if (tspace > 0 && std::max(amax, bmax) / tspace + 8 > DAMAR_MAX_MARKS)
    { fprintf(stderr, "damar: FATAL: reads of %d bases need a trace spacing (-s) of at least %d here\n", std::max(amax, bmax),
              std::max(amax, bmax) / (DAMAR_MAX_MARKS - 8) + 1);
      die();
    }
}

static void scratch_prepare(int amax, int bmax, int binshift, int tspace, u32 cell_cap, hipStream_t st)
{ if (tspace <= 0)
    { fprintf(stderr, "damar: FATAL: trace spacing %d\n", tspace);
      die();
    }
  if (tspace > DAMAR_MAX_TSPACE)
    { fprintf(stderr, "damar: FATAL: a trace spacing (-s) above %d is not supported by this build\n", DAMAR_MAX_TSPACE);
      die();
    }
  if (G_last_d2h[RS.cur] != NULL)
    { HIP_CHECK(hipStreamWaitEvent(st, G_last_d2h[RS.cur], 0));
      G_last_d2h[RS.cur] = NULL;
    }
  if (G_ring == 0)
    { const char *e = getenv("DAMAR_RING");
      G_ring = e ? atoi(e) : 1024;
      if (G_ring < 128) G_ring = 128;
      while (G_ring & (G_ring - 1)) G_ring += G_ring & -G_ring;
    }
  int span = 128;
  while (span < amax + bmax + 72) span *= 2;
  if (span > G_ring) span = G_ring;
  int bwidth = (amax >> binshift) - ((-bmax) >> binshift) + 1;
  int mtp    = 2 * (std::max(amax, bmax) / tspace + 2) + 8;
  u32 tstr   = (u32) (4 * mtp + 32);
  if (RS.bwidth < bwidth)      bwidth = ((bwidth + bwidth / 4) + 255) & ~255;
  if (RS.ttmp_stride < tstr)   tstr   = ((tstr + tstr / 4) + 255u) & ~255u;
  int nslots = default_slots();
  bool grow = RS.span < span || RS.bwidth < bwidth || RS.cell_cap < cell_cap || RS.ttmp_stride < tstr;
  if (grow || (RS.nslots != nslots && RS.nslots_wanted != nslots))
    { const double g0 = now_ms();
      HIP_CHECK(hipStreamSynchronize(G_st));
      late_streams();
      HIP_CHECK(hipStreamSynchronize(G_rep));
      if (RS.state)   { HIP_CHECK(hipFree(RS.state)); HIP_CHECK(hipFree(RS.marks)); HIP_CHECK(hipFree(RS.cells));
                        HIP_CHECK(hipFree(RS.buckets)); HIP_CHECK(hipFree(RS.ttmp)); RS.state = NULL; }
      RS.nslots_wanted = nslots;
      { size_t freeb = 0, totb = 0;
        const u64 nspan = (u64) std::max(RS.span, span), ncell = std::max(RS.cell_cap, cell_cap);
        const u64 per = damar_report_state_stride((int) nspan) + 4ull * 2 * nspan + 8ull * ncell +
                        4ull * (3ull * std::max(RS.bwidth, bwidth) + 16) + 2ull * std::max(RS.ttmp_stride, tstr);
        const double g1 = now_ms();
        HIP_CHECK(hipMemGetInfo(&freeb, &totb));
        if (getenv("DAMAR_HOSTPROF")) fprintf(stderr, "damar: scratch grow: sync+free %.1f ms, hipMemGetInfo %.1f ms\n", g1 - g0, now_ms() - g1);
        const u64 budget = (u64) (freeb * 0.6);
        if ((u64) nslots * per > budget)
          { int fit = (int) (budget / per);
            if (fit < 64)
              { fprintf(stderr, "damar: FATAL: not enough device memory for the alignment scratch (%.1f MB per wave slot, %.1f GB free)\n",
                        per / 1048576., freeb / 1073741824.);
                die();
              }
            if (VERBOSE)
              fprintf(stderr, "damar: %d instead of %d resident alignments (%.1f MB of scratch each)\n", fit, nslots, per / 1048576.);
            nslots = fit - fit % damar_report2_slots_per_wave();
          }
      }
      RS.nslots = nslots;
      RS.span   = std::max(RS.span, span);
      RS.bwidth = std::max(RS.bwidth, bwidth);
      RS.cell_cap = std::max(RS.cell_cap, cell_cap);
      RS.ttmp_stride = std::max(RS.ttmp_stride, tstr);
      RS.state_stride  = damar_report_state_stride(RS.span);
      RS.marks_stride  = (u64) 2 * RS.span;
      RS.bucket_stride = (u64) 3 * RS.bwidth + 16;
      const double g2 = now_ms();
      RS.state   = dmalloc((size_t) RS.state_stride * nslots);
      RS.marks   = (int *) dmalloc(sizeof(int) * (size_t) RS.marks_stride * nslots);
      RS.cells   = dmalloc((size_t) 8 * RS.cell_cap * nslots);
      RS.buckets = (int *) dmalloc(sizeof(int) * (size_t) RS.bucket_stride * nslots);
      RS.ttmp    = (u16 *) dmalloc(sizeof(u16) * (size_t) RS.ttmp_stride * nslots);
      HIP_CHECK(hipMemsetAsync(RS.state, 0, (size_t) RS.state_stride * nslots, st));
      HIP_CHECK(hipMemsetAsync(RS.marks, 0, sizeof(int) * (size_t) RS.marks_stride * nslots, st));
      if (getenv("DAMAR_HOSTPROF"))
        fprintf(stderr, "damar: scratch grow: 5 allocations of %.2f GB in all %.1f ms (span %d bwidth %d cells %u)\n",
                ((double) RS.state_stride + 4. * RS.marks_stride + 8. * RS.cell_cap + 4. * RS.bucket_stride + 2. * RS.ttmp_stride) * nslots / 1073741824.,
                now_ms() - g2, RS.span, RS.bwidth, RS.cell_cap);
    }
  if (RS.counters == NULL)
    { RS.counters = (u32 *) dmalloc(sizeof(u32) * DAMAR_COUNTER_WORDS * 2);
      RS.tables   = (short *) dmalloc(sizeof(short) * 65536 * DAMAR_MAX_JOBS);
    }
  HIP_CHECK(hipMemsetAsync(RS.buckets, 0, sizeof(int) * (size_t) RS.bucket_stride * RS.nslots, st));
}

static void scratch_outputs(u32 rec_cap, u32 tpool_cap)
{ const int c = RS.cur;
  if (RS.rec_cap_set[c] < rec_cap || RS.tpool_cap_set[c] < tpool_cap)
    { late_streams();
      HIP_CHECK(hipStreamSynchronize(G_copy));
      G_last_d2h[c] = NULL;
      if (RS.rec_cap_set[c] < rec_cap)
        { RS.rec_cap_set[c] = rec_cap + (rec_cap >> 2);
          if (RS.recs_set[c]) HIP_CHECK(hipFree(RS.recs_set[c]));
          RS.recs_set[c] = (LaRecord *) dmalloc(sizeof(LaRecord) * (size_t) RS.rec_cap_set[c]);
        }
      if (RS.tpool_cap_set[c] < tpool_cap)
        { RS.tpool_cap_set[c] = tpool_cap + (tpool_cap >> 2);
          if (RS.tpool_set[c]) HIP_CHECK(hipFree(RS.tpool_set[c]));
          RS.tpool_set[c] = (u16 *) dmalloc(sizeof(u16) * (size_t) RS.tpool_cap_set[c]);
        }
    }
  RS.recs  = RS.recs_set[c];   RS.rec_cap   = RS.rec_cap_set[c];
  RS.tpool = RS.tpool_set[c];  RS.tpool_cap = RS.tpool_cap_set[c];
  RS.ctr   = RS.counters + (size_t) c * DAMAR_COUNTER_WORDS;
}

static void fill_report_args(ReportArgs *ra, const damar_dev_block *ab, const damar_dev_block *bb,
                             int comp, int self, Align_Spec *spec, hipStream_t st, int job, int tslot, const JobParams &jp)
{ memset(ra, 0, sizeof(*ra));
  ra->job = job;
  ra->ablk = ab->d;  ra->bblk = bb->d;
  ra->kmer = jp.kmer;  ra->hitmin = jp.hitmin;  ra->binshift = jp.binshift;
  ra->minhit = (jp.hitmin - 1) / jp.kmer + 1;
  ra->comp = comp;  ra->self = self;  ra->symmetric = jp.symmetric;
  ra->minover = jp.minover;  ra->hgap_min = jp.hgap_min;
  ra->tspace = Trace_Spacing(spec);
  ra->ave_path = damar_spec_ave_path(spec);
  ra->reach = Overlap_If_Possible(spec);
  {
    static short *shadow = NULL;
    static bool   valid[DAMAR_MAX_JOBS];
// ... 519 lines not shown
          A_tail_ms += now_ms() - t0;
        }
      stage_done(A_s1);
    }
}

static void write_worker(void)
{ for (;;)
    { TailJob *job = stage_next(A_s2);
      if (job == NULL)
        return;
      double t0 = now_ms();
      damar_write_detached(&job->wp, job->bufs, job->has1 ? job->d1.c_str() : NULL,
                           job->has2 ? job->d2.c_str() : NULL, job->a.c_str(), job->b.c_str(), job->last);
      delete job;
      { std::lock_guard<std::mutex> lk(A_mu);
        A_write_ms += now_ms() - t0;
      }
      stage_done(A_s2);
    }
}

static void async_submit(TailJob *job)
{ stage_submit(A_s1, job);
}

extern "C" void damar_async_drain(void)
{ if (!A_on)
    return;
  finish_all();
  stage_drain(A_s1);
  stage_drain(A_s2);
}

extern "C" void damar_set_async(int on)
{ if (on && !A_on)
    { A_s1.quit = A_s2.quit = false;
      A_s1.threads.push_back(new std::thread(tail_worker));
      { const char *e = getenv("DAMAR_WRITE_THREADS");
        int n = e ? atoi(e) : 2;
        if (n < 1) n = 1;
        if (n > 16) n = 16;
        for (int i = 0; i < n; i++)
          A_s2.threads.push_back(new std::thread(write_worker));
      }
      A_on = true;
    }
  else if (!on && A_on)
    { damar_async_drain();
      Stage *st[2] = { &A_s1, &A_s2 };
      for (int i = 0; i < 2; i++)
        { { std::lock_guard<std::mutex> lk(st[i]->mu);
            st[i]->quit = true;
          }
          st[i]->cv.notify_all();
          for (std::thread *th : st[i]->threads)
            { th->join();
              delete th;
            }
          st[i]->threads.clear();
        }
      A_on = false;
      helpers_join();
    }
}

extern "C" void damar_async_totals(int64 *ncheck, double *tail_ms, double *write_ms)
{ const double d0 = now_ms();
  damar_async_drain();
  H_ms[7] += now_ms() - d0;
  if (getenv("DAMAR_HOSTPROF"))
    { fprintf(stderr, "damar host wall ms:");
      for (int i = 0; i < 8; i++)
        { fprintf(stderr, " %s=%.1f", H_name[i], H_ms[i]);
          H_ms[i] = 0;
        }
      fprintf(stderr, " | between calls=%.1f launch->next front=%.1f flush->exit=%.1f entry->front=%.1f front->tick0=%.1f\n",
              Q_ms[2], Q_ms[3], Q_seg[0], Q_seg[2], Q_seg[3]);
      Q_ms[2] = Q_ms[3] = 0;  Q_exit = 0;  Q_seg[0] = Q_seg[2] = Q_seg[3] = 0;
    }
  std::lock_guard<std::mutex> lk(A_mu);
  if (ncheck)   *ncheck = A_ncheck;
  if (tail_ms)  *tail_ms = A_tail_ms;
  if (write_ms) *write_ms = A_write_ms;
  A_ncheck = 0;  A_tail_ms = 0;  A_write_ms = 0;
}

extern "C" double damar_async_d2h_ms(void)
{ damar_async_drain();
  std::lock_guard<std::mutex> lk(A_mu);
  double v = A_d2h_ms;
  A_d2h_ms = 0;
  return v;
}


static std::vector<u64> G_seed_keys;
static std::vector<u32> G_seed_vals;
static int  G_seed_pbits = 0, G_seed_abits = 0, G_seed_dbits = 0;
static int  G_keep_seeds = 0;

static int64 sizeof_db(const HITS_DB *db)
{ return (int64) sizeof(HITS_DB) + (int64) sizeof(HITS_READ) * (db->nreads + 2) + db->totlen + db->nreads + 4 +
         (db->path ? (int64) strlen(db->path) + 1 : 0);
}


struct Front
{ const u64 *keys;  const u32 *vals;  u64 total;
  const u32 *work;  u32 nwork;
  const u32 *order;
  int pbits, abits, dbits;
  JobParams jp;
  size_t bytes;
  double t_entry;
};

static bool match_front(damar_match_job *job, int slot, Front *f)
{ const HITS_DB *ablock = job->ablock, *bblock = job->bblock;
  damar_dev_index *aidx = job->aidx, *bidx = job->bidx;
  const int self = job->self, comp = job->comp;
  Arena &G_hits = G_hitsJ[slot], &G_ord = G_ordJ[slot];
  int64 nhits = 0;
  const double t_entry = now_ms();
  pick_sort_shape();
  memset(f, 0, sizeof(*f));
  f->t_entry = t_entry;
  f->jp = params_now();
  job->counts[0] = job->counts[1] = job->counts[2] = 0;
  if (aidx == NULL || bidx == NULL || aidx->n == 0 || bidx->n == 0)
    return false;
  if (aidx->kbits != bidx->kbits)
    { fprintf(stderr, "damar: internal error, index parameters differ\n");
      die();
    }
  const u32 alen = aidx->n, blen = bidx->n;
  MergeArgs m;
  memset(&m, 0, sizeof(m));
  m.acode = aidx->codes;  m.apos = aidx->pos;  m.alen = alen;
  m.bcode = bidx->codes;  m.bpos = bidx->pos;  m.blen = blen;
  m.wide = aidx->wide;
  m.kbits = aidx->kbits;
  m.self = self;  m.comp = comp;  m.identity = IDENTITY;
  m.limit = (MEM_LIMIT > 0) ? MAXGRAM : 0x7fffffffu;
  m.ablk = aidx->blk->d;  m.bblk = bidx->blk->d;
  m.pbits = std::max(1, ilog2_ceil((u64) ablock->maxlen + 1));
  m.abits = std::max(1, ilog2_ceil((u64) ablock->nreads));
  int bbits = std::max(1, ilog2_ceil((u64) bblock->nreads));
  if (m.pbits + m.abits + bbits > 64)
    { fprintf(stderr, "damar: FATAL: seed key needs %d bits (> 64)\n", m.pbits + m.abits + bbits);
      die();
    }
  { static int pack_on = -1;
    if (pack_on < 0)
      { const char *e = getenv("DAMAR_PACK_SEEDS");
        pack_on = e ? atoi(e) : 1;
      }
    const int db = std::max(1, ilog2_ceil((u64) bblock->maxlen + 1));
    m.dbits = (pack_on && m.pbits + m.abits + bbits + db <= 64) ? db : 0;
  }

  const u32 mtiles = damar_merge_tiles(alen);
  void *mw;
  u32  *tcount;
  u64  *tot;
  u64   total = 0;

  if (Q_flush > 0)
    { Q_ms[3] += now_ms() - Q_flush;  Q_flush = 0; }
  Q_seg[3] += now_ms() - f->t_entry;
  tick(0);
  arena_reserve(&G_work, pad256(damar_merge_workspace_bytes(alen)) + pad256(damar_scan_workspace_bytes(mtiles)) + 4096);
  mw = arena_take(&G_work, damar_merge_workspace_bytes(alen));
  tcount = damar_merge_tile_counts(mw, alen);
  tot = (u64 *) arena_take(&G_work, 64);
  void *mscw = arena_take(&G_work, damar_scan_workspace_bytes(mtiles));
  damar_launch_merge_count(&m, mw, NULL, 0, G_st);
  stage("merge_count");
  damar_exclusive_scan_u32(tcount, tcount, mtiles, mscw, tot, G_st);
  stage("merge_scan");
  HIP_CHECK(hipMemcpyAsync(&total, tot, sizeof(u64), hipMemcpyDeviceToHost, G_st));
  stream_wait(G_st);
  if (MEM_LIMIT > 0)
    {
      int   limit = MAXGRAM;
      int64 avail = (int64) (MEM_LIMIT - (uint64) (sizeof_db(ablock) + sizeof_db(bblock))) / 16;
      if (aidx == bidx || avail > (int64) alen + 2 * (int64) blen)
        avail = (avail - alen) / 2;
      else
        avail = avail - ((int64) alen + blen);
      avail = (int64) (avail * .98);
      if ((int64) total > avail)
        { std::vector<unsigned long long> histo(MAXGRAM);
          unsigned long long *dgram = (unsigned long long *) dmalloc(sizeof(unsigned long long) * MAXGRAM);
          HIP_CHECK(hipMemsetAsync(dgram, 0, sizeof(unsigned long long) * MAXGRAM, G_st));
          damar_launch_merge_count(&m, mw, dgram, MAXGRAM, G_st);
          HIP_CHECK(hipMemcpyAsync(histo.data(), dgram, sizeof(unsigned long long) * MAXGRAM, hipMemcpyDeviceToHost, G_st));
          HIP_CHECK(hipStreamSynchronize(G_st));
          HIP_CHECK(hipFree(dgram));
          int64 tom = 0;
          int   j;
          for (j = 0; j < MAXGRAM; j++)
            { tom += (int64) j * (int64) histo[j];
              if (tom > avail)
                break;
            }
          limit = j;
          if (limit <= 1)
            { fprintf(stderr, "\nError: Insufficient ");
              if (MEM_LIMIT == MEM_PHYSICAL)
                fprintf(stderr, " physical memory (%.1fGb), reduce block size\n", (1. * MEM_LIMIT) / 0x40000000ll);
              else
                { fprintf(stderr, " memory allocation (%.1fGb),", (1. * MEM_LIMIT) / 0x40000000ll);
                  fprintf(stderr, " reduce block size or increase allocation\n");
                }
              fflush(stderr);
              exit(1);
            }
          if (limit < 10)
            { fprintf(stderr, "\nWarning: Sensitivity hampered by low ");
              if (MEM_LIMIT == MEM_PHYSICAL)
                fprintf(stderr, " physical memory (%.1fGb), reduce block size\n", (1. * MEM_LIMIT) / 0x40000000ll);
              else
                { fprintf(stderr, " memory allocation (%.1fGb),", (1. * MEM_LIMIT) / 0x40000000ll);
                  fprintf(stderr, " reduce block size or increase allocation\n");
                }
              fflush(stderr);
            }
          m.limit = (u32) limit;
          damar_launch_merge_count(&m, mw, NULL, 0, G_st);
          damar_exclusive_scan_u32(tcount, tcount, mtiles, mscw, tot, G_st);
          HIP_CHECK(hipMemcpyAsync(&total, tot, sizeof(u64), hipMemcpyDeviceToHost, G_st));
          HIP_CHECK(hipStreamSynchronize(G_st));
        }
      G_limit = limit;
      if (VERBOSE)
        printf("\n   Capping mutual k-mer matches over %d (effectively -t%d)\n", limit, (int) sqrt(1. * limit));
    }
  else
    G_limit = 0x7fffffff;
  nhits = (int64) total;
  if (VERBOSE)
    { printf("   Hit count = %lld\n", (long long) nhits);
      fflush(stdout);
    }
  if (total >= 0xfffffff0ull)
    { fprintf(stderr, "damar: FATAL: %llu seed pairs exceed the 32-bit seed index of this build\n",
              (unsigned long long) total);
      die();
    }
  if (total == 0)
    return false;

  const int sbits = m.pbits + m.abits + bbits;
  const int spasses = (sbits + 7) / 8;
  const int minhit = (P_hitmin - 1) / P_kmer + 1;
  const int idbits = m.abits + bbits;
  static int cut_on = -1;
  if (cut_on < 0)
    { const char *e = getenv("DAMAR_EARLY_CUT");
      cut_on = e ? atoi(e) : 0;
    }
  const bool ranged = P_bread_lo > 0 || P_bread_hi != 0xffffffffu;
  const bool cut = (cut_on || ranged) && !G_keep_seeds && idbits <= 32;
  static int two_step = -1;
  if (two_step < 0)
    { const char *e = getenv("DAMAR_WORK_TWOSTEP");
      two_step = (e && atoi(e) > 0) ? 1 : 0;
    }
  static int pair_sort = -1;
  static long long pair_ratio = 4000;
  static u64 prev_seeds = 0, prev_work = 1;
  if (pair_sort < 0)
    { const char *e = getenv("DAMAR_SORT_PAIR"), *r = getenv("DAMAR_ADAPT_RATIO");
      pair_sort = e ? atoi(e) : 2;
      if (r)
        pair_ratio = atoll(r);
    }
  const bool pair_on = pair_sort == 1 || (pair_sort == 2 && pair_ratio > 0 && prev_seeds / prev_work > (u64) pair_ratio);
  bool psort = pair_on && !cut && !two_step && !G_keep_seeds && m.dbits != 0 && m.pbits + 11 <= 32 && m.pbits >= 8;
  const int spasses_used = psort ? (sbits - m.pbits + 7) / 8 : spasses;
  u64 *keys, *tk;
  u32 *vals, *flags, *foff;
  void *scw2, *resort_ws = NULL;
  u64 *sends;
  int  hshift = P_nshift;
  if (!cut)
    { arena_reserve(&G_hits, pad256(sizeof(u64) * (size_t) total) + pad256(sizeof(u32) * (size_t) total) + 4096);
      arena_reserve(&G_tmp,  pad256(sizeof(u64) * (size_t) total) + 3 * pad256(sizeof(u32) * (size_t) total) +
                             pad256(damar_sort_workspace_bytes(total)) + pad256(damar_scan_workspace_bytes(total)) + 8192);
      u64 *pk = (u64 *) arena_take(&G_hits, sizeof(u64) * (size_t) total);
      u32 *pv = m.dbits ? NULL : (u32 *) arena_take(&G_hits, sizeof(u32) * (size_t) total);
      tk = (u64 *) arena_take(&G_tmp, sizeof(u64) * (size_t) total);
      u32 *tv = m.dbits ? NULL : (u32 *) arena_take(&G_tmp, sizeof(u32) * (size_t) total);
      u64 *k0 = (spasses_used & 1) ? tk : pk, *k1 = (spasses_used & 1) ? pk : tk;
      u32 *v0 = (spasses_used & 1) ? tv : pv, *v1 = (spasses_used & 1) ? pv : tv;
      void *sw = arena_take(&G_tmp, damar_sort_workspace_bytes(total));
      resort_ws = sw;
      flags = (u32 *) arena_take(&G_tmp, sizeof(u32) * (size_t) total);
      foff  = (u32 *) arena_take(&G_tmp, std::max(sizeof(u32) * (size_t) total, bit_words_bytes(total)));
      scw2  = arena_take(&G_tmp, damar_scan_workspace_bytes(total));
      sends = (u64 *) arena_take(&G_tmp, 64 * sizeof(u64));

      damar_launch_merge_emit(&m, mw, total, k0, v0, NULL, G_st);
      stage("merge_emit");
      tick(1);
      int side = m.dbits ? damar_radix_sort_keys_u64(k0, k1, total, m.dbits + (psort ? m.pbits : 0), m.dbits + sbits, sw, G_st)
                         : damar_radix_sort_u64(k0, v0, k1, v1, total, sbits, sw, G_st);
      sort_check(sw);
      keys = side ? k1 : k0;
      vals = side ? v1 : v0;
      if (keys != pk)
        { fprintf(stderr, "damar: internal error, the seed sort ended on the wrong side\n");
          die();
        }
    }
  else
    {
      const size_t bmwords = (((size_t) 1 << idbits) + 31) / 32;
      arena_reserve(&G_tmp, pad256(sizeof(u64) * (size_t) total) + 4 * pad256(sizeof(u32) * (size_t) total) +
                            pad256(sizeof(u32) * ((size_t) total / minhit + 64)) +
                            pad256(damar_sort_workspace_bytes(total)) + pad256(damar_scan_workspace_bytes(total)) +
                            pad256(sizeof(u32) * bmwords) + 16384);
      u64 *uk   = (u64 *) arena_take(&G_tmp, sizeof(u64) * (size_t) total);
      u32 *uv   = (u32 *) arena_take(&G_tmp, sizeof(u32) * (size_t) total);
      u32 *pid0 = (u32 *) arena_take(&G_tmp, sizeof(u32) * (size_t) total);
      u32 *pid1 = (u32 *) arena_take(&G_tmp, sizeof(u32) * (size_t) total);
      u32 *hbit = (u32 *) arena_take(&G_tmp, sizeof(u32) * (size_t) total);
      u32 *hd   = (u32 *) arena_take(&G_tmp, sizeof(u32) * ((size_t) total / minhit + 64));
      void *sw  = arena_take(&G_tmp, damar_sort_workspace_bytes(total));
      void *scc = arena_take(&G_tmp, damar_scan_workspace_bytes(total));
      u32 *bitmap = (u32 *) arena_take(&G_tmp, sizeof(u32) * bmwords);
      u64 *snd  = (u64 *) arena_take(&G_tmp, 64 * sizeof(u64));

      damar_launch_merge_emit(&m, mw, total, uk, uv, pid0, G_st);
      stage("merge_emit");
      tick(1);
      const u32 *spid = damar_radix_sort_keys_u32(pid0, pid1, total, idbits, sw, G_st) ? pid1 : pid0;
      sort_check(sw);
      u64 n64 = 0;
      damar_launch_pair_heads_ids(spid, total, m.abits, minhit, P_nshift, snd, (u64 *) hbit, scc, tot, hd, G_st);
      HIP_CHECK(hipMemsetAsync(bitmap, 0, sizeof(u32) * bmwords, G_st));
      HIP_CHECK(hipMemcpyAsync(&n64, tot, sizeof(u64), hipMemcpyDeviceToHost, G_st));
      HIP_CHECK(hipStreamSynchronize(G_st));
      damar_launch_pair_bitmap(spid, hd, (u32) n64, m.abits, P_bread_lo, P_bread_hi, bitmap, G_st);
      damar_launch_seed_cut_count(uk, total, m.pbits + m.dbits, bitmap, (u32 *) scc, tot, G_st);
      HIP_CHECK(hipMemcpyAsync(&n64, tot, sizeof(u64), hipMemcpyDeviceToHost, G_st));
      HIP_CHECK(hipStreamSynchronize(G_st));
      stage("early_cut");
      const u64 nsurv = n64;
      G_cnt[6] += (int64) nsurv;
      if (nsurv == 0)
        { tick(2);  tick(3);
          G_ms[DAMAR_T_MERGE] += lap(0, 1);
          G_ms[DAMAR_T_SSORT] += lap(1, 2);
          G_cnt[0] += nhits;
          job->counts[0] = nhits;
          return false;
        }
      arena_reserve(&G_hits, pad256(sizeof(u64) * (size_t) nsurv) + pad256(sizeof(u32) * (size_t) nsurv) + 4096);
      arena_reserve(&G_tmp2, pad256(sizeof(u64) * (size_t) nsurv) + 3 * pad256(sizeof(u32) * (size_t) nsurv) +
                             pad256(damar_sort_workspace_bytes(nsurv)) + pad256(damar_scan_workspace_bytes(nsurv)) + 8192);
      u64 *pk = (u64 *) arena_take(&G_hits, sizeof(u64) * (size_t) nsurv);
      u32 *pv = m.dbits ? NULL : (u32 *) arena_take(&G_hits, sizeof(u32) * (size_t) nsurv);
      tk = (u64 *) arena_take(&G_tmp2, sizeof(u64) * (size_t) nsurv);
      u32 *tv = m.dbits ? NULL : (u32 *) arena_take(&G_tmp2, sizeof(u32) * (size_t) nsurv);
      u64 *k0 = (spasses & 1) ? tk : pk, *k1 = (spasses & 1) ? pk : tk;
      u32 *v0 = (spasses & 1) ? tv : pv, *v1 = (spasses & 1) ? pv : tv;
      void *sw2 = arena_take(&G_tmp2, damar_sort_workspace_bytes(nsurv));
      flags = (u32 *) arena_take(&G_tmp2, sizeof(u32) * (size_t) nsurv);
      foff  = (u32 *) arena_take(&G_tmp2, std::max(sizeof(u32) * (size_t) nsurv, bit_words_bytes(nsurv)));
      scw2  = arena_take(&G_tmp2, damar_scan_workspace_bytes(nsurv));
      sends = (u64 *) arena_take(&G_tmp2, 64 * sizeof(u64));
      damar_launch_seed_cut_scatter(uk, m.dbits ? NULL : uv, total, m.pbits + m.dbits, bitmap, (const u32 *) scc, k0, v0, G_st);
      int side = m.dbits ? damar_radix_sort_keys_u64(k0, k1, nsurv, m.dbits, m.dbits + sbits, sw2, G_st)
                         : damar_radix_sort_u64(k0, v0, k1, v1, nsurv, sbits, sw2, G_st);
      sort_check(sw2);
      keys = side ? k1 : k0;
      vals = side ? v1 : v0;
      if (keys != pk)
        { fprintf(stderr, "damar: internal error, the seed sort ended on the wrong side\n");
          die();
        }
      total  = nsurv;
      hshift = -1;
    }
  stage("seed_sort");
  tick(2);

  u64 nwork64 = 0;
  u32 *work = NULL;
  if (!two_step)
    {
      u64 got[2] = { 0, 0 };
      if (cut)
        psort = false;
      damar_launch_pair_work(keys, vals, total, m.pbits, m.dbits, m.abits, minhit, hshift, sends, (u64 *) foff ,
                             scw2, tot, P_binshift, P_kmer, P_hitmin, P_bread_lo, P_bread_hi, psort ? 1 : 0, G_st);
      stage("run_heads");
      tick(3);
      HIP_CHECK(hipMemcpyAsync(got, tot, 2 * sizeof(u64), hipMemcpyDeviceToHost, G_st));
      stream_wait(G_st);
      if (psort && got[1] != 0)
        {
          G_cnt[7] += 1;
          u64 *other = (keys == tk) ? NULL : tk;
          if (other == NULL || resort_ws == NULL)
            { fprintf(stderr, "damar: internal error, no room to sort the seeds again\n");
              die();
            }
          int side = damar_radix_sort_keys_u64(keys, other, total, m.dbits, m.dbits + sbits, resort_ws, G_st);
          sort_check(resort_ws);
          if (side)
            HIP_CHECK(hipMemcpyAsync(keys, other, sizeof(u64) * (size_t) total, hipMemcpyDeviceToDevice, G_st));
          damar_launch_pair_work(keys, vals, total, m.pbits, m.dbits, m.abits, minhit, hshift, sends, (u64 *) foff, scw2, tot,
                                 P_binshift, P_kmer, P_hitmin, P_bread_lo, P_bread_hi, 0, G_st);
          HIP_CHECK(hipMemcpyAsync(got, tot, 2 * sizeof(u64), hipMemcpyDeviceToHost, G_st));
          stream_wait(G_st);
          psort = false;
        }
      nwork64 = got[0];
      arena_reserve(&G_ord, 5 * pad256(sizeof(u32) * (size_t) nwork64) + pad256(damar_sort_workspace_bytes(nwork64)) + 8192);
      work = (u32 *) arena_take(&G_ord, sizeof(u32) * ((size_t) nwork64 + 1));
      if (nwork64 > 0)
        { damar_launch_pair_work_expand((const u64 *) foff, scw2, total, work, G_st);
          if (psort)
            damar_launch_order_runs(keys, total, m.pbits, m.dbits, work, (u32) nwork64, G_st);
        }
      stage("work_list");
    }
  else
    { u32 *heads = (u32 *) tk;
      damar_launch_pair_heads(keys, total, m.pbits + m.dbits, m.abits, minhit, hshift, sends, (u64 *) foff ,
                              scw2, tot, heads, G_st);
      stage("run_heads");
      HIP_CHECK(hipMemcpyAsync(&nwork64, tot, sizeof(u64), hipMemcpyDeviceToHost, G_st));
      HIP_CHECK(hipStreamSynchronize(G_st));
      const u32 nheads = (u32) nwork64;
      arena_reserve(&G_ord, 5 * pad256(sizeof(u32) * (size_t) nheads) + pad256(damar_sort_workspace_bytes(nheads)) + 8192);
      work = (u32 *) arena_take(&G_ord, sizeof(u32) * ((size_t) nheads + 1));
      nwork64 = 0;
      if (nheads > 0)
        { damar_launch_pair_screen(keys, vals, total, m.pbits, m.dbits, heads, nheads, minhit, P_binshift, P_kmer, P_hitmin, m.abits,
                                   P_bread_lo, P_bread_hi, flags, G_st);
          damar_exclusive_scan_u32(flags, foff, nheads, scw2, tot, G_st);
          damar_launch_compact_u32(heads, flags, foff, nheads, work, G_st);
          stage("work_list");
          HIP_CHECK(hipMemcpyAsync(&nwork64, tot, sizeof(u64), hipMemcpyDeviceToHost, G_st));
        }
    }
  if (two_step)
    { tick(3);
      HIP_CHECK(hipStreamSynchronize(G_st));
    }
  sort_verify();
  const u32 nwork = (u32) nwork64;
  G_ms[DAMAR_T_MERGE] += lap(0, 1);
  G_ms[DAMAR_T_SSORT] += lap(1, 2);
  G_ms[DAMAR_T_WORK]  += lap(2, 3);
  G_cnt[0] += nhits;  G_cnt[1] += nwork;
  job->counts[0] = nhits;
  prev_seeds = total;  prev_work = nwork > 0 ? nwork : 1;

  if (G_keep_seeds)
    { G_seed_keys.resize(total);  G_seed_vals.resize(total);
      HIP_CHECK(hipMemcpy(G_seed_keys.data(), keys, sizeof(u64) * (size_t) total, hipMemcpyDeviceToHost));
      if (vals != NULL)
        HIP_CHECK(hipMemcpy(G_seed_vals.data(), vals, sizeof(u32) * (size_t) total, hipMemcpyDeviceToHost));
      G_seed_pbits = m.pbits;  G_seed_abits = m.abits;  G_seed_dbits = m.dbits;
    }

  const u32 *order = NULL;
  static int order_mode = -1;
  if (order_mode < 0)
    { const char *e = getenv("DAMAR_ORDER");
      order_mode = e ? atoi(e) : 11;
    }
  if (nwork > 1 && order_mode > 0)
    { u32 *ok0 = (u32 *) arena_take(&G_ord, sizeof(u32) * (size_t) nwork);
      u32 *ov0 = (u32 *) arena_take(&G_ord, sizeof(u32) * (size_t) nwork);
      u32 *ok1 = (u32 *) arena_take(&G_ord, sizeof(u32) * (size_t) nwork);
      u32 *ov1 = (u32 *) arena_take(&G_ord, sizeof(u32) * (size_t) nwork);
      void *osw = arena_take(&G_ord, damar_sort_workspace_bytes(nwork));
      const u32 cmode = order_mode == 2 ? 1u : order_mode == 9 ? 0xffffffffu : order_mode == 10 ? 0xfffffffeu :
                        order_mode == 11 ? 0xfffffffdu : order_mode == 12 ? 0xfffffffcu : (order_mode > 2 ? (u32) order_mode : 0u);
      damar_launch_work_cost(keys, vals, total, m.pbits, m.abits, m.dbits, m.ablk.boff, m.bblk.boff, work, nwork, cmode, ok0, ov0, G_st);
      order = damar_radix_sort_u32(ok0, ov0, ok1, ov1, nwork, WORK_COST_BITS, osw, G_st) ? ov1 : ov0;
      sort_check(osw);
      stage("work_order");
    }


  f->keys = keys;  f->vals = vals;  f->total = total;
  f->work = work;  f->nwork = nwork;  f->order = order;
  f->pbits = m.pbits;  f->abits = m.abits;  f->dbits = m.dbits;
  f->bytes = G_hits.cap + G_ord.cap;
  return nwork > 0;
}

struct Pending
{ bool live;
  int  n;
  int  slot[DAMAR_MAX_JOBS];
  damar_match_job  job[DAMAR_MAX_JOBS];
  damar_match_job *orig[DAMAR_MAX_JOBS];
  Front fr[DAMAR_MAX_JOBS];
  const damar_dev_block *ablk[DAMAR_MAX_JOBS], *bblk[DAMAR_MAX_JOBS];
  int  amax, bmax, tsmin;
  u32  cell_cap, rec_cap, tp_cap;
  int  t8;
  bool wide_ok;
  bool wide_done;
  u32  wm_off[DAMAR_MAX_JOBS + 1];
  int  attempt;
  int  oset;
  hipEvent_t done;
  hipStream_t st;
  double t_launch;
  ReportArgs ra[DAMAR_MAX_JOBS];
  std::vector<TailJob *> writes;
};
static Pending *PQ = new Pending[2]();
static int      PQ_head = 0, PQ_n = 0;
static bool     G_slot_busy[DAMAR_MAX_JOBS];

struct Accum
{ int    n;
  int    slot[DAMAR_MAX_JOBS / 2];
  damar_match_job  job[DAMAR_MAX_JOBS / 2];
  damar_match_job *orig[DAMAR_MAX_JOBS / 2];
  Front  fr[DAMAR_MAX_JOBS / 2];
  const damar_dev_block *ablk[DAMAR_MAX_JOBS / 2], *bblk[DAMAR_MAX_JOBS / 2];
  size_t bytes;
  u64    nwork;
  std::vector<TailJob *> writes;
};
static Accum &AC = *new Accum();


static int64   A_nfilt = 0;
static int64   W_tot[3] = { 0, 0, 0 };
static double  A_report_ms = 0;
static int64   A_launches = 0;

static void report_launch(Pending &pd)
{ ReportArgs *const ra = pd.ra;
  const hipStream_t st = pd.st;
  double q0 = now_ms();
  RS.cur = pd.oset;
  scratch_prepare(pd.amax, pd.bmax, pd.fr[0].jp.binshift, pd.tsmin, pd.cell_cap, st);
  double q1 = now_ms();
  scratch_outputs(pd.rec_cap, pd.tp_cap);
  double q2 = now_ms();
  Q_ms[0] += q1 - q0;  Q_ms[1] += q2 - q1;
  bool packed = true;
  for (int j = 0; j < pd.n; j++)
    { const damar_match_job &jb = pd.job[j];
      fill_report_args(&ra[j], pd.ablk[j], pd.bblk[j], jb.comp, jb.self, jb.spec, st, j, pd.slot[j], pd.fr[j].jp);
      ra[j].keys = pd.fr[j].keys;  ra[j].vals = pd.fr[j].vals;  ra[j].nhits = pd.fr[j].total;
      ra[j].work = pd.fr[j].work;  ra[j].nwork = pd.fr[j].nwork;
      ra[j].pbits = pd.fr[j].pbits;  ra[j].abits = pd.fr[j].abits;  ra[j].dbits = pd.fr[j].dbits;
      ra[j].order = pd.fr[j].order;
      ra[j].t8 = pd.t8;
      ra[j].widemap = NULL;  ra[j].wcells = RS.wcells;  ra[j].wcell_cap = RS.wcell_cap;  ra[j].cell_max = max_cells();
      packed = packed && use_packed(&ra[j], pd.amax, pd.bmax);
      if (ra[j].mscore != ra[0].mscore || ra[j].dscore != ra[0].dscore)
        { fprintf(stderr, "damar: internal error, the comparisons of one report launch differ in their -e\n");
          die();
        }
    }
  pd.wide_ok = packed;  pd.wide_done = false;
  if (!packed && std::max(pd.amax, pd.bmax) / std::max(1, pd.tsmin) + 8 > DAMAR_MAX_MARKS)
    { fprintf(stderr, "damar: FATAL: reads of %d bases need a trace spacing (-s) of at least %d when one read pair per wavefront "
                      "is asked for (DAMAR_PACKED=0): the wide kernel runs behind the two-pair kernel only\n",
              std::max(pd.amax, pd.bmax), std::max(pd.amax, pd.bmax) / (DAMAR_MAX_MARKS - 8) + 1);
      die();
    }
  if (packed)
    {
      u32 words = 0;
      for (int j = 0; j < pd.n; j++)
        { pd.wm_off[j] = words;
          words += (ra[j].nwork + 31) / 32 + 1;
        }
      pd.wm_off[pd.n] = words;
      const int c = pd.oset;
      if (RS.widemap_cap[c] < words)
        { if (RS.widemap[c]) HIP_CHECK(hipFree(RS.widemap[c]));
          RS.widemap_cap[c] = words + (words >> 2) + 1024;
          RS.widemap[c] = (u32 *) dmalloc(sizeof(u32) * (size_t) RS.widemap_cap[c]);
        }
      HIP_CHECK(hipMemsetAsync(RS.widemap[c], 0, sizeof(u32) * (size_t) words, st));
      for (int j = 0; j < pd.n; j++)
        ra[j].widemap = RS.widemap[c] + pd.wm_off[j];
    }
  HIP_CHECK(hipMemsetAsync(RS.ctr, 0, sizeof(u32) * DAMAR_COUNTER_WORDS, st));
  tick_on(16 + 4 * pd.oset, st);
  if (packed)
    {
      static long long ratio = -1;
      static int wps = 0;
      if (ratio < 0)
        { const char *e = getenv("DAMAR_ADAPT_RATIO"), *w = getenv("DAMAR_ADAPT_WPS");
          ratio = e ? atoll(e) : 4000;
          wps = w ? atoi(w) : 3;
          if (wps < 1) wps = 1;
        }
      int nslots = RS.nslots;
      if (ratio > 0 && corun_on() && pd.st == G_rep)
        { u64 seeds = 0, work = 0;
          for (int j = 0; j < pd.n; j++)
// ... 1216 lines not shown
```

include/damar_hip.h:

```cpp
#ifndef DAMAR_HIP_H
#define DAMAR_HIP_H

#include "damar_db.h"
#include "damar_align.h"

#ifdef __cplusplus
extern "C" {
#endif

int   damar_hip_init(int device);
int   damar_hip_numa_node(int device);
const char *damar_hip_device_name(void);
void  damar_hip_sync(void);
void  damar_prewarm(int gigabytes);

typedef struct damar_dev_block damar_dev_block;
damar_dev_block *damar_block_upload(const HITS_DB *block);
void damar_block_preload(const HITS_DB *block);
damar_dev_block *damar_block_upload_bg(const HITS_DB *block);
damar_dev_block *damar_block_upload_packed(const HITS_DB *block, const damar_packed *pk, int comp);
void             damar_packed_forget(const HITS_DB *block);
void             damar_block_free(damar_dev_block *blk);

typedef struct damar_dev_index damar_dev_index;
damar_dev_index *damar_index_build(damar_dev_block *blk, int own_block, int *len);
void             damar_index_free(damar_dev_index *idx);
uint64_t         damar_index_bytes(const damar_dev_index *idx);
uint64_t         damar_block_bytes(const damar_dev_block *blk);
void             damar_hbm_info(uint64_t *free_bytes, uint64_t *total_bytes);
void             damar_pool_trim(void);
void             damar_index_download(const damar_dev_index *idx, void *out);

void damar_match(const HITS_DB *ablock, const HITS_DB *bblock,
                 damar_dev_index *aidx, damar_dev_index *bidx,
                 int self, int comp, Align_Spec *spec, int64 *counts);

typedef struct
{ const HITS_DB *ablock, *bblock;
  damar_dev_index *aidx, *bidx;
  int self, comp;
  Align_Spec *spec;
  int64 counts[3];
} damar_match_job;
void damar_match_batch(damar_match_job *jobs, int njobs);

void damar_set_bread_range(int lo, int hi);

void damar_set_async(int on);
void damar_async_drain(void);
void damar_async_totals(int64 *ncheck, double *tail_ms, double *write_ms);
void damar_async_counts(int64 *seed_hits, double *report_ms, int64 *launches);
double damar_async_d2h_ms(void);
void damar_wave_totals(int64 *cells, int64 *half_steps, int64 *iterations);
void damar_write_overlaps(Align_Spec *spec, const char *dirName1, const char *dirName2,
                          const char *ablock, const char *bblock, int lastRead);

int  damar_tandem_set_params(int kmer, int binshift, int hitmin, int nthreads);
void damar_match_self(const HITS_DB *ablock, damar_dev_block *blk, Align_Spec *spec, int64 *counts);
void Match_Self(char *aname, HITS_DB *ablock, Align_Spec *settings);

int64 damar_last_seeds(void *out, int64 cap);

int damar_last_limit(void);

void damar_bias_reset(void);

int damar_local_alignment_batch(damar_dev_block *ablk, damar_dev_block *bblk, int comp,
                                Align_Spec *spec, const int *tasks, int ntasks,
                                int *paths, int64 *trace_off, uint16 *traces, int64 trace_cap);

int  damar_trace_pts(damar_dev_block *ablk, int afirst, damar_dev_block *bblk, int bfirst,
                     const Overlap *ovls, int64 novl, int tbytes, int tspace, int mode, int same,
                     int64 *soff, int *diffs, int **script);
int  damar_trace_mid(damar_dev_block *ablk, int afirst, damar_dev_block *bblk, int bfirst,
                     const Overlap *ovls, int64 novl, int tbytes, int tspace, int mode, int same,
                     int64 *soff, int *diffs, int **script);
void damar_trace_last(double *ms, int64 *cnt);
void damar_trace_release(void);

enum { DAMAR_T_TUPLES = 0, DAMAR_T_KSORT, DAMAR_T_TABLE, DAMAR_T_MERGE, DAMAR_T_SSORT,
       DAMAR_T_WORK, DAMAR_T_REPORT, DAMAR_T_D2H, DAMAR_T_TAIL, DAMAR_T_COUNT };
void damar_last_timings(double *ms );
void damar_las_totals(int64 *out );

void damar_last_counters(int64 *c );

double damar_bench_sort_u32(uint32_t n, int nbits, int reps, uint32_t seed);

#ifdef __cplusplus
}
#endif
#endif
```

Before: 51.24 billion.

## Fuse radix-sort digit histograms into k-mer tuple and merge-emit producer kernels

Computes the onesweep radix-sort digit histograms inside the kernels that produce the keys (k-mer tuple generation and merge emit), using LDS-privatized packed 16-bit counters, and skips the separate histogram pass over the keys before sorting. This removes one full read of the key array and a kernel launch per sort. In exchange the producer kernels become persistent grid-stride kernels with extra LDS and atomics, which can lower their occupancy. The path is on by default behind DAMAR_FUSED_HIST, and an optional check mode compares the fused histogram against a reference.

```diff
diff --git a/damar_amd/csrc/kernels/kernels.h b/damar_amd/csrc/kernels/kernels.h
--- a/damar_amd/csrc/kernels/kernels.h
+++ b/damar_amd/csrc/kernels/kernels.h
@@ -18,6 +18,23 @@
 int    damar_radix_sort_keys_u32(u32 *k0, u32 *k1, u64 n, int nbits, void *work, hipStream_t st);
 int    damar_radix_sort_u64(u64 *k0, u32 *v0, u64 *k1, u32 *v1, u64 n, int nbits, void *work, hipStream_t st);
 
+#define DAMAR_SORT_MAXPASS 8
+typedef struct
+{ u64 dsh;
+  u64 dwd;
+  int npass;
+  int lobit;
+} SortDigits;
+SortDigits damar_sort_digits(int lobit, int hibit);
+
+u32   *damar_sort_fused_begin(void *work, u64 n, hipStream_t st);
+int    damar_radix_sort_keys_u64_fused(u64 *k0, u64 *k1, u64 n, int lobit, int hibit, void *work, hipStream_t st);
+void   damar_radix_sort_split_u64_fused(u64 *k0, u64 *k1, u64 n, int lobit, int hibit, u32 *ohi, u32 *olo, void *work,
+                                        hipStream_t st);
+int    damar_radix_sort_u64_fused(u64 *k0, u32 *v0, u64 *k1, u32 *v1, u64 n, int nbits, void *work, hipStream_t st);
+void   damar_sort_hist_only(const u64 *keys, u64 n, int lobit, int hibit, u32 *hist, hipStream_t st);
+size_t damar_fused_hist_lds(const SortDigits *sd, int copies);
+
 typedef struct
 { const u8  *bases;
   const u32 *pk;
@@ -41,6 +58,54 @@
 #define PK_PAD 4
 
 #ifdef __HIPCC__
+__host__ __device__ __forceinline__ int sort_digit_shift(const SortDigits &sd, int p) { return sd.lobit + (int) ((sd.dsh >> (8 * p)) & 0xffu); }
+__host__ __device__ __forceinline__ u32 sort_digit_mask(const SortDigits &sd, int p)  { return (u32) ((sd.dwd >> (8 * p)) & 0xffu); }
+template <typename KeyT>
+__device__ __forceinline__ u32 sort_digit(const SortDigits &sd, int p, KeyT key)
+{ return (u32) (key >> sort_digit_shift(sd, p)) & sort_digit_mask(sd, p); }
+
+#define FUSED_BINMAX 61440
+
+__device__ __forceinline__ u32 fused_hist_words(const SortDigits &sd, u32 C)
+{ u32 nw = 0;
+  for (int p = 0; p < sd.npass; p++)
+    nw += ((sort_digit_mask(sd, p) + 1u) >> 1) * C;
+  return nw;
+}
+
+__device__ __forceinline__ void fused_hist_clear(u32 *sh, const SortDigits &sd, u32 C)
+{ const u32 nw = fused_hist_words(sd, C);
+  for (u32 j = threadIdx.x; j < nw; j += blockDim.x)
+    sh[j] = 0;
+}
+
+template <typename KeyT>
+__device__ __forceinline__ void fused_hist_add(u32 *sh, const SortDigits &sd, u32 C, KeyT key)
+{ const u32 c = threadIdx.x & (C - 1u);
+  u32 at = 0;
+  for (int p = 0; p < sd.npass; p++)
+    { const u32 d = sort_digit(sd, p, key);
+      atomicAdd(&sh[at + (d >> 1) * C + c], 1u << ((d & 1u) << 4));
+      at += ((sort_digit_mask(sd, p) + 1u) >> 1) * C;
+    }
+}
+
+__device__ __forceinline__ void fused_hist_flush(const u32 *sh, const SortDigits &sd, u32 C, u32 *__restrict__ ghist)
+{ u32 at = 0;
+  for (int p = 0; p < sd.npass; p++)
+    { const u32 nb = sort_digit_mask(sd, p) + 1u;
+      for (u32 d = threadIdx.x; d < nb; d += blockDim.x)
+        { const u32 sft = (d & 1u) << 4;
+          u32 sum = 0;
+          for (u32 q = 0; q < C; q++)
+            sum += (sh[at + (d >> 1) * C + ((q + threadIdx.x) & (C - 1u))] >> sft) & 0xffffu;
+          if (sum)
+            atomicAdd(&ghist[p * 256 + (int) d], sum);
+        }
+      at += (nb >> 1) * C;
+    }
+}
+
 __device__ __forceinline__ u32 read_of_pos(const DevBlock &b, u32 p)
 { u32 r = b.coarse[p >> COARSE_SHIFT];
   while (b.boff[r + 1] <= p)
@@ -72,6 +137,8 @@
 void damar_merge_set_prio(int on);
 void damar_index_set_prio(int on);
 void damar_launch_kmer_tuples(const DevBlock *blk, int kmer, u32 nkmers, void *codes, int wide, u32 *pos, hipStream_t st);
+void damar_launch_kmer_tuples_hist(const DevBlock *blk, int kmer, u32 nkmers, u64 *codes, const SortDigits *sd, u32 *ghist,
+                                   hipStream_t st);
 void damar_launch_mask_flags(const DevBlock *blk, int kmer, const u32 *pos, u32 n, u32 *keep, hipStream_t st);
 void damar_launch_biased_tuples(const DevBlock *blk, int kmer, const int *logbase, void *codes, int wide, u32 *pos,
                                 u32 *keep, hipStream_t st);
@@ -102,6 +169,8 @@
 u32    damar_merge_tiles(u32 alen);
 void   damar_launch_merge_count(const MergeArgs *m, void *work, unsigned long long *gram, u32 ngram, hipStream_t st);
 void damar_launch_merge_emit(const MergeArgs *m, void *work, u64 nhits, u64 *keys, u32 *vals, u32 *pid, hipStream_t st);
+int  damar_launch_merge_emit_hist(const MergeArgs *m, void *work, u64 nhits, u64 *keys, u32 *vals, const SortDigits *sd,
+                                  u32 *ghist, hipStream_t st);
 void damar_launch_pair_heads_ids(const u32 *pids, u64 nhits, int abits, int minhit, int nshift,
                                  u64 *send, u64 *bits, void *scan_work, u64 *total_dev, u32 *heads, hipStream_t st);
 void damar_launch_pair_bitmap(const u32 *pids, const u32 *heads, u32 nheads, int abits, u32 b_lo, u32 b_hi, u32 *bitmap,
diff --git a/damar_amd/csrc/kernels/kmer_index.hip b/damar_amd/csrc/kernels/kmer_index.hip
--- a/damar_amd/csrc/kernels/kmer_index.hip
+++ b/damar_amd/csrc/kernels/kmer_index.hip
@@ -6,18 +6,16 @@
 
 
 template <typename CodeT, bool PACK>
-__global__ __launch_bounds__(256)
-void kmer_tuples(DevBlock blk, int kmer, u32 nkmers, CodeT *__restrict__ codes, u32 *__restrict__ pos)
-{ SEED_PRIO(g_index_prio);
-  const u32 p = blockIdx.x * 256u + threadIdx.x;
-  if (p >= blk.total)
-    return;
+__device__ __forceinline__ bool kmer_tuple_at(const DevBlock &blk, int kmer, u32 nkmers, u32 p, CodeT *__restrict__ codes,
+                                              u32 *__restrict__ pos, CodeT *key)
+{ if (p >= blk.total)
+    return false;
   const u32 r = read_of_pos(blk, p), b0 = blk.boff[r];
   if (p - b0 < (u32) (kmer - 1) || p + 1 == blk.boff[r + 1])
-    return;
+    return false;
   const u32 i = p - (r + 1) * (u32) kmer + 1;
   if (i >= nkmers)
-    return;
+    return false;
   CodeT c = 0;
   if (PACK)
     {
@@ -35,11 +33,50 @@
     }
   const u32 pw = pos_encode(blk, r, p - b0, p);
   if (PACK)
-    codes[i] = (CodeT) ((u64) c << 32) | (CodeT) pw;
-  else
-    { codes[i] = c;
+    codes[i] = *key = (CodeT) ((u64) c << 32) | (CodeT) pw;
+  else
+    { codes[i] = *key = c;
       pos[i]   = pw;
     }
+  return true;
+}
+
+template <typename CodeT, bool PACK>
+__global__ __launch_bounds__(256)
+void kmer_tuples(DevBlock blk, int kmer, u32 nkmers, CodeT *__restrict__ codes, u32 *__restrict__ pos)
+{ SEED_PRIO(g_index_prio);
+  CodeT key;
+  (void) kmer_tuple_at<CodeT, PACK>(blk, kmer, nkmers, blockIdx.x * 256u + threadIdx.x, codes, pos, &key);
+}
+
+#define KT_THREADS 1024
+__global__ __launch_bounds__(KT_THREADS, 8)
+void kmer_tuples_hist(DevBlock blk, int kmer, u32 nkmers, u64 *__restrict__ codes, SortDigits sd, u32 *__restrict__ ghist)
+{ SEED_PRIO(g_index_prio);
+  extern __shared__ u32 sh[];
+  fused_hist_clear(sh, sd, 32u);
+  __syncthreads();
+  const u32 nround = (blk.total + KT_THREADS - 1) / KT_THREADS;
+  for (u32 t = blockIdx.x; t < nround; t += gridDim.x)
+    { u64 key;
+      if (kmer_tuple_at<u64, true>(blk, kmer, nkmers, t * KT_THREADS + threadIdx.x, codes, (u32 *) NULL, &key))
+        fused_hist_add(sh, sd, 32u, key);
+    }
+  __syncthreads();
+  fused_hist_flush(sh, sd, 32u, ghist);
+}
+
+void damar_launch_kmer_tuples_hist(const DevBlock *blk, int kmer, u32 nkmers, u64 *codes, const SortDigits *sd, u32 *ghist,
+                                   hipStream_t st)
+{ if (nkmers == 0)
+    return;
+  const u32 nround = (blk->total + KT_THREADS - 1) / KT_THREADS;
+  const u32 maxit = FUSED_BINMAX / (KT_THREADS / 32);
+  u32 grid = nround < 512 ? nround : 512;
+  if ((nround + grid - 1) / grid > maxit)
+    grid = (nround + maxit - 1) / maxit;
+  hipLaunchKernelGGL(kmer_tuples_hist, dim3(grid), dim3(KT_THREADS), damar_fused_hist_lds(sd, 32), st, *blk, kmer, nkmers, codes,
+                     *sd, ghist);
 }
 
 void damar_launch_kmer_tuples(const DevBlock *blk, int kmer, u32 nkmers, void *codes, int wide, u32 *pos, hipStream_t st)
diff --git a/damar_amd/csrc/kernels/radix_sort.hip b/damar_amd/csrc/kernels/radix_sort.hip
--- a/damar_amd/csrc/kernels/radix_sort.hip
+++ b/damar_amd/csrc/kernels/radix_sort.hip
@@ -16,7 +16,7 @@
 #define OS_RANK_LDS 1
 #endif
 #define OS_MINTILE (256 * 8)
-#define OS_MAXPASS 8
+#define OS_MAXPASS DAMAR_SORT_MAXPASS
 
 #define OH_ITEMS   16
 
@@ -50,19 +50,15 @@
 
 
 #define OH_THREADS 1024
-#define OH_BINMAX  61440
+#define OH_BINMAX  FUSED_BINMAX
 
 template <typename KeyT>
 __global__ __launch_bounds__(OH_THREADS)
-void onesweep_hist(const KeyT *__restrict__ keys, u64 n, int lobit, int npass, u64 dsh ,
-                   u64 dwd , u32 *__restrict__ ghist, uint4 *__restrict__ clr, u64 clr16)
+void onesweep_hist(const KeyT *__restrict__ keys, u64 n, SortDigits sd, u32 *__restrict__ ghist, uint4 *__restrict__ clr, u64 clr16)
 { extern __shared__ u32 sh[];
   constexpr u32 nthr = OH_THREADS;
-  const int nw = npass * 128 * 32;
-  for (int j = threadIdx.x; j < nw; j += nthr)
-    sh[j] = 0;
-  __syncthreads();
-  const u32 c = threadIdx.x & 31u;
+  fused_hist_clear(sh, sd, 32u);
+  __syncthreads();
   const u64 ntile = (n + (u64) nthr * OH_ITEMS - 1) / ((u64) nthr * OH_ITEMS);
   for (u64 t = blockIdx.x; t < ntile; t += gridDim.x)
     { const u64 base = t * ((u64) nthr * OH_ITEMS);
@@ -76,24 +72,11 @@
       for (int r = 0; r < OH_ITEMS; r++)
         { const u64 i = base + (u64) r * nthr + threadIdx.x;
           if (i < n)
-            { const KeyT x = k[r] >> lobit;
-              for (int p = 0; p < npass; p++)
-                { const u32 d = (u32) (x >> (int) ((dsh >> (8 * p)) & 0xffu)) & (u32) ((dwd >> (8 * p)) & 0xffu);
-                  atomicAdd(&sh[((u32) p << 12) + ((d >> 1) << 5) + c], 1u << ((d & 1u) << 4));
-                }
-            }
-        }
-    }
-  __syncthreads();
-  for (int j = threadIdx.x; j < npass * 256; j += nthr)
-    { const u32 pl = (u32) j >> 8, d = (u32) j & 0xffu, sft = (d & 1u) << 4;
-      u32 sum = 0;
-#pragma unroll 8
-      for (u32 q = 0; q < 32; q++)
-        sum += (sh[(pl << 12) + ((d >> 1) << 5) + ((q + threadIdx.x) & 31u)] >> sft) & 0xffffu;
-      if (sum)
-        atomicAdd(&ghist[j], sum);
-    }
+            fused_hist_add(sh, sd, 32u, k[r]);
+        }
+    }
+  __syncthreads();
+  fused_hist_flush(sh, sd, 32u, ghist);
   const uint4 z = make_uint4(0, 0, 0, 0);
   for (u64 i = (u64) blockIdx.x * nthr + threadIdx.x; i < clr16; i += (u64) gridDim.x * nthr)
     clr[i] = z;
@@ -102,9 +85,9 @@
 #define OH_COPIES  8
 template <typename KeyT>
 __global__ __launch_bounds__(256)
-void onesweep_hist8(const KeyT *__restrict__ keys, u64 n, int lobit, int npass, u64 dsh ,
-                   u64 dwd , u32 *__restrict__ ghist, uint4 *__restrict__ clr, u64 clr16)
+void onesweep_hist8(const KeyT *__restrict__ keys, u64 n, SortDigits sd, u32 *__restrict__ ghist, uint4 *__restrict__ clr, u64 clr16)
 { SEED_PRIO(g_sort_prio);
+  const int npass = sd.npass;
   extern __shared__ u32 sh[];
   const int nb = npass * 256 * OH_COPIES;
   for (int j = threadIdx.x; j < nb; j += 256)
@@ -124,11 +107,10 @@
       for (int r = 0; r < OH_ITEMS; r++)
         { const u64 i = base + (u64) r * 256 + threadIdx.x;
           if (i < n)
-            { const KeyT x = k[r] >> lobit;
+            {
+#pragma nounroll
               for (int p = 0; p < npass; p++)
-                { const u32 d = (u32) (x >> (int) ((dsh >> (8 * p)) & 0xffu)) & (u32) ((dwd >> (8 * p)) & 0xffu);
-                  atomicAdd(&sh[(((u32) p << 8) + d) * OH_COPIES + c], 1u);
-                }
+                atomicAdd(&sh[(((u32) p << 8) + sort_digit(sd, p, k[r])) * OH_COPIES + c], 1u);
             }
         }
     }
@@ -371,40 +353,45 @@
 
 const u32 *damar_sort_error_word(const void *work) { return (const u32 *) work; }
 
-template <typename KeyT, typename GT, bool HV, int TH, int IT>
-static void onesweep_passes(KeyT *k0, u32 *v0, KeyT *k1, u32 *v1, u64 n, int lobit, int hibit, u32 *ohi, u32 *olo,
-                            char *ws, hipStream_t st)
-{ constexpr int OS_TILE = TH * IT;
-  const u32 ntiles = (u32) ((n + OS_TILE - 1) / OS_TILE);
-  const int npass  = (hibit - lobit + 7) / 8;
-  int dshift[OS_MAXPASS], dwidth[OS_MAXPASS];
-  u64 dsh = 0, dwd = 0;
-  { const int bits = hibit - lobit, base = bits / npass, extra = bits % npass;
-    int at = 0;
-    static int even = -1;
-    if (even < 0)
-      { const char *e = getenv("DAMAR_SORT_EVEN");
-        even = e ? atoi(e) : 1;
-      }
-    for (int p = 0; p < npass; p++)
-      { dshift[p] = at;
-        dwidth[p] = even ? base + (p < extra ? 1 : 0) : (p < npass - 1 ? 8 : bits - 8 * (npass - 1));
-        at += dwidth[p];
-        dsh |= (u64) dshift[p] << (8 * p);
-        dwd |= (u64) ((1u << dwidth[p]) - 1u) << (8 * p);
-      }
-  }
-  const size_t region = ((size_t) ntiles * 256 * sizeof(GT) + 255) & ~(size_t) 255;
-  u32 *err = (u32 *) ws, *ghist = (u32 *) (ws + WS_HIST), *ctr = (u32 *) (ws + WS_CTR);
-  GT  *lbr[2] = { (GT *) (ws + WS_LB), (GT *) (ws + WS_LB + region) };
-  HIP_CHECK(hipMemsetAsync(ws, 0, WS_LB, st));
-  if (sort_threads() >= 512)
+SortDigits damar_sort_digits(int lobit, int hibit)
+{ SortDigits sd;
+  const int bits = hibit - lobit;
+  sd.dsh = sd.dwd = 0;
+  sd.lobit = lobit;
+  sd.npass = (bits + 7) / 8;
+  if (sd.npass <= 0 || sd.npass > OS_MAXPASS)
+    return sd;
+  static int even = -1;
+  if (even < 0)
+    { const char *e = getenv("DAMAR_SORT_EVEN");
+      even = e ? atoi(e) : 1;
+    }
+  const int base = bits / sd.npass, extra = bits % sd.npass;
+  int at = 0;
+  for (int p = 0; p < sd.npass; p++)
+    { const int width = even ? base + (p < extra ? 1 : 0) : (p < sd.npass - 1 ? 8 : bits - 8 * (sd.npass - 1));
+      sd.dsh |= (u64) at << (8 * p);
+      sd.dwd |= (u64) ((1u << width) - 1u) << (8 * p);
+      at += width;
+    }
+  return sd;
+}
+
+size_t damar_fused_hist_lds(const SortDigits *sd, int copies)
+{ size_t nw = 0;
+  for (int p = 0; p < sd->npass; p++)
+    nw += (size_t) ((sort_digit_mask(*sd, p) + 1u) >> 1) * (size_t) copies;
+  return nw * sizeof(u32);
+}
+
+template <typename KeyT>
+static void launch_hist(const KeyT *keys, u64 n, const SortDigits &sd, u32 *ghist, uint4 *clr, u64 clr16, hipStream_t st)
+{ if (sort_threads() >= 512)
     { const u64 nt = (n + (u64) OH_THREADS * OH_ITEMS - 1) / ((u64) OH_THREADS * OH_ITEMS);
       const u64 maxit = OH_BINMAX / ((OH_THREADS / 32) * OH_ITEMS);
       u64 grid = nt < 512 ? nt : 512;
       if ((nt + grid - 1) / grid > maxit)
         grid = (nt + maxit - 1) / maxit;
-      const size_t lds = (size_t) npass * 128 * 32 * sizeof(u32);
       {
         static std::atomic<unsigned long long> big_lds(0ull);
         int dev = 0;
@@ -416,36 +403,70 @@
             big_lds.fetch_or(bit, std::memory_order_release);
           }
       }
-      hipLaunchKernelGGL(onesweep_hist<KeyT>, dim3((u32) grid), dim3(OH_THREADS), lds, st,
-                         k0, n, lobit, npass, dsh, dwd, ghist, (uint4 *) lbr[0], (u64) (region / 16));
+      hipLaunchKernelGGL(onesweep_hist<KeyT>, dim3((u32) grid), dim3(OH_THREADS), damar_fused_hist_lds(&sd, 32), st,
+                         keys, n, sd, ghist, clr, clr16);
       HIP_CHECK(hipGetLastError());
     }
   else
     { const u64 nt = (n + 256 * OH_ITEMS - 1) / (256 * OH_ITEMS);
       const u32 grid = (u32) (nt < 2048 ? nt : 2048);
-      hipLaunchKernelGGL(onesweep_hist8<KeyT>, dim3(grid), dim3(256), (size_t) npass * 256 * OH_COPIES * sizeof(u32), st,
-                         k0, n, lobit, npass, dsh, dwd, ghist, (uint4 *) lbr[0], (u64) (region / 16));
+      hipLaunchKernelGGL(onesweep_hist8<KeyT>, dim3(grid), dim3(256), (size_t) sd.npass * 256 * OH_COPIES * sizeof(u32), st,
+                         keys, n, sd, ghist, clr, clr16);
+    }
+}
+
+static bool sort_lb64(void)
+{ static int lb64 = -1;
+  if (lb64 < 0)
+    lb64 = getenv("DAMAR_SORT_LB64") != NULL;
+  return lb64 != 0;
+}
+
+static size_t sort_region_bytes(u64 n)
+{ const bool wide = !(n < (1ull << 30) && !sort_lb64());
+  const u64 tile = (wide || sort_threads() == 256) ? 256 * 16 : 8192;
+  return ((size_t) ((n + tile - 1) / tile) * 256 * (wide ? sizeof(u64) : sizeof(u32)) + 255) & ~(size_t) 255;
+}
+
+template <typename KeyT, typename GT, bool HV, int TH, int IT>
+static void onesweep_passes(KeyT *k0, u32 *v0, KeyT *k1, u32 *v1, u64 n, int lobit, int hibit, u32 *ohi, u32 *olo,
+                            char *ws, bool fused, hipStream_t st)
+{ constexpr int OS_TILE = TH * IT;
+  const u32 ntiles = (u32) ((n + OS_TILE - 1) / OS_TILE);
+  const int npass  = (hibit - lobit + 7) / 8;
+  const SortDigits sd = damar_sort_digits(lobit, hibit);
+  const size_t region = ((size_t) ntiles * 256 * sizeof(GT) + 255) & ~(size_t) 255;
+  u32 *err = (u32 *) ws, *ghist = (u32 *) (ws + WS_HIST), *ctr = (u32 *) (ws + WS_CTR);
+  GT  *lbr[2] = { (GT *) (ws + WS_LB), (GT *) (ws + WS_LB + region) };
+  if (region != sort_region_bytes(n))
+    { fprintf(stderr, "damar: internal error, look-back region of the radix sort\n");
+      fflush(NULL);
+      _exit(1);
+    }
+  if (!fused)
+    { HIP_CHECK(hipMemsetAsync(ws, 0, WS_LB, st));
+      launch_hist<KeyT>(k0, n, sd, ghist, (uint4 *) lbr[0], (u64) (region / 16), st);
     }
   for (int p = 0; p < npass; p++)
     { const int  side = p & 1;
       const bool last = (p == npass - 1);
       KeyT *ki = side ? k1 : k0, *ko = side ? k0 : k1;
       u32  *vi = side ? v1 : v0, *vo = side ? v0 : v1;
-      const u32 mask = (1u << dwidth[p]) - 1u;
+      const u32 mask = sort_digit_mask(sd, p);
       if (last && ohi != NULL)
         hipLaunchKernelGGL((onesweep_pass<KeyT, GT, false, true, TH, IT>), dim3(ntiles), dim3(TH), 0, st,
-                           ki, (const u32 *) NULL, (KeyT *) NULL, olo, ohi, n, lobit + dshift[p], mask,
+                           ki, (const u32 *) NULL, (KeyT *) NULL, olo, ohi, n, sort_digit_shift(sd, p), mask,
                            ghist + 256 * p, lbr[side], lbr[side ^ 1], ctr + p, err);
       else
         hipLaunchKernelGGL((onesweep_pass<KeyT, GT, HV, false, TH, IT>), dim3(ntiles), dim3(TH), 0, st,
-                           ki, vi, ko, vo, (u32 *) NULL, n, lobit + dshift[p], mask,
+                           ki, vi, ko, vo, (u32 *) NULL, n, sort_digit_shift(sd, p), mask,
                            ghist + 256 * p, lbr[side], lbr[side ^ 1], ctr + p, err);
     }
 }
 
 template <typename KeyT, bool HV>
 static int onesweep_impl(KeyT *k0, u32 *v0, KeyT *k1, u32 *v1, u64 n, int lobit, int hibit, u32 *ohi, u32 *olo,
-                         void *work, hipStream_t st)
+                         void *work, hipStream_t st, bool fused = false)
 { const int npass = (hibit - lobit + 7) / 8;
   if (n == 0 || npass <= 0)
     return 0;
@@ -455,16 +476,13 @@
       _exit(1);
     }
   const int shape = sort_threads();
-  static int lb64 = -1;
-  if (lb64 < 0)
-    lb64 = getenv("DAMAR_SORT_LB64") != NULL;
-  if (n < (1ull << 30) && !lb64)
-    { if (shape == 1024)     onesweep_passes<KeyT, u32, HV, 1024, 8>(k0, v0, k1, v1, n, lobit, hibit, ohi, olo, (char *) work, st);
-      else if (shape == 512) onesweep_passes<KeyT, u32, HV, 512, 16>(k0, v0, k1, v1, n, lobit, hibit, ohi, olo, (char *) work, st);
-      else              onesweep_passes<KeyT, u32, HV, 256, 16>(k0, v0, k1, v1, n, lobit, hibit, ohi, olo, (char *) work, st);
+  if (n < (1ull << 30) && !sort_lb64())
+    { if (shape == 1024)     onesweep_passes<KeyT, u32, HV, 1024, 8>(k0, v0, k1, v1, n, lobit, hibit, ohi, olo, (char *) work, fused, st);
+      else if (shape == 512) onesweep_passes<KeyT, u32, HV, 512, 16>(k0, v0, k1, v1, n, lobit, hibit, ohi, olo, (char *) work, fused, st);
+      else              onesweep_passes<KeyT, u32, HV, 256, 16>(k0, v0, k1, v1, n, lobit, hibit, ohi, olo, (char *) work, fused, st);
     }
   else
-    onesweep_passes<KeyT, u64, HV, 256, 16>(k0, v0, k1, v1, n, lobit, hibit, ohi, olo, (char *) work, st);
+    onesweep_passes<KeyT, u64, HV, 256, 16>(k0, v0, k1, v1, n, lobit, hibit, ohi, olo, (char *) work, fused, st);
   return npass & 1;
 }
 
@@ -484,6 +502,27 @@
                                 hipStream_t st)
 { onesweep_impl<u64, false>(k0, NULL, k1, NULL, n, lobit, hibit, ohi, olo, work, st); }
 
+u32 *damar_sort_fused_begin(void *work, u64 n, hipStream_t st)
+{ HIP_CHECK(hipMemsetAsync(work, 0, WS_LB + sort_region_bytes(n), st));
+  return (u32 *) ((char *) work + WS_HIST);
+}
+
+int damar_radix_sort_u64_fused(u64 *k0, u32 *v0, u64 *k1, u32 *v1, u64 n, int nbits, void *work, hipStream_t st)
+{ return onesweep_impl<u64, true>(k0, v0, k1, v1, n, 0, nbits, NULL, NULL, work, st, true); }
+
+int damar_radix_sort_keys_u64_fused(u64 *k0, u64 *k1, u64 n, int lobit, int hibit, void *work, hipStream_t st)
+{ return onesweep_impl<u64, false>(k0, NULL, k1, NULL, n, lobit, hibit, NULL, NULL, work, st, true); }
+
+void damar_radix_sort_split_u64_fused(u64 *k0, u64 *k1, u64 n, int lobit, int hibit, u32 *ohi, u32 *olo, void *work,
+                                      hipStream_t st)
+{ onesweep_impl<u64, false>(k0, NULL, k1, NULL, n, lobit, hibit, ohi, olo, work, st, true); }
+
+void damar_sort_hist_only(const u64 *keys, u64 n, int lobit, int hibit, u32 *hist, hipStream_t st)
+{ const SortDigits sd = damar_sort_digits(lobit, hibit);
+  if (n > 0 && sd.npass > 0 && sd.npass <= OS_MAXPASS)
+    launch_hist<u64>(keys, n, sd, hist, (uint4 *) NULL, 0, st);
+}
+
 void damar_preload_sort(void)
 { hipFuncAttributes fa;
   (void) hipFuncGetAttributes(&fa, (const void *) onesweep_hist<u64>);
diff --git a/damar_amd/csrc/kernels/seed_merge.hip b/damar_amd/csrc/kernels/seed_merge.hip
--- a/damar_amd/csrc/kernels/seed_merge.hip
+++ b/damar_amd/csrc/kernels/seed_merge.hip
@@ -607,19 +607,17 @@
     merge_sweep_tile<CodeT, false>(m, tl, blockIdx.x, tcount, cnt, jbg, gram, ngram, sb, loc, sjb, sw4, red);
 }
 
-__global__ __launch_bounds__(256, 8)
-void merge_emit(MergeArgs m, const MergeTile *__restrict__ tiles, const u32 *__restrict__ cnt, const u32 *__restrict__ jbg,
-                const u32 *__restrict__ toff, u64 nhits, u64 *__restrict__ keys, u32 *__restrict__ vals, u32 *__restrict__ pid)
-{ SEED_PRIO(g_merge_prio);
-  __shared__ u32 loc[MT_A + 1];
-  __shared__ u32 sjb[MT_A];
-  __shared__ u32 sw4[4];
-  const int l = lane_id(), w = threadIdx.x >> 6;
-  const u32 tile = blockIdx.x;
+template <int HIST_C>
+__device__ __forceinline__ void merge_emit_tile(const MergeArgs &m, const MergeTile *__restrict__ tiles, const u32 *__restrict__ cnt,
+                                                const u32 *__restrict__ jbg, const u32 *__restrict__ toff, u32 tile, u32 ntiles,
+                                                u64 nhits, u64 *__restrict__ keys, u32 *__restrict__ vals, u32 *__restrict__ pid,
+                                                u32 *loc, u32 *sjb, u32 *sw4,
+                                                u32 *fh, const SortDigits &sd, u32 *__restrict__ ghist, u32 &facc)
+{ const int l = lane_id(), w = threadIdx.x >> 6;
   const u32 a0 = tile * (u32) MT_A, a1 = min(m.alen, a0 + (u32) MT_A), nat = a1 - a0;
   const u32 e0 = threadIdx.x * MT_PER;
   const u64 h0 = toff[tile];
-  const u64 hn = (tile + 1 < gridDim.x) ? (u64) toff[tile + 1] : nhits;
+  const u64 hn = (tile + 1 < ntiles) ? (u64) toff[tile + 1] : nhits;
   if (hn == h0)
     return;
   u32 n[MT_PER], s = 0;
@@ -648,8 +646,20 @@
     loc[MT_A] = ex;
   __syncthreads();
   const u32 T = loc[MT_A];
-  for (u32 t0 = threadIdx.x; t0 < T; t0 += 256 * MT_HITS)
-    { u32 ai[MT_HITS], bi[MT_HITS], pa[MT_HITS], pb[MT_HITS];
+  for (u32 tb = 0; tb < T; tb += 256 * MT_HITS)
+    { const u32 t0 = tb + threadIdx.x;
+      if (HIST_C > 0)
+        { if (facc + 256 * MT_HITS > (u32) FUSED_BINMAX * (u32) HIST_C)
+            { __syncthreads();
+              fused_hist_flush(fh, sd, (u32) HIST_C, ghist);
+              __syncthreads();
+              fused_hist_clear(fh, sd, (u32) HIST_C);
+              __syncthreads();
+              facc = 0;
+            }
+          facc += 256 * MT_HITS;
+        }
+      u32 ai[MT_HITS], bi[MT_HITS], pa[MT_HITS], pb[MT_HITS];
 #pragma unroll
       for (int x = 0; x < MT_HITS; x++)
         { const u32 t = t0 + (u32) x * 256;
@@ -691,17 +701,52 @@
           const u64 h = h0 + t;
           if (t < T && h < nhits)
             { const u64 key = ((u64) rb[x] << (m.abits + m.pbits)) | ((u64) ra[x] << m.pbits) | (u64) xa[x];
-              if (m.dbits)
-                keys[h] = (key << m.dbits) | (u64) xb[x];
-              else
-                { keys[h] = key;
-                  vals[h] = (u32) ((int) xa[x] - (int) xb[x]);
-                }
+              const u64 out = m.dbits ? (key << m.dbits) | (u64) xb[x] : key;
+              keys[h] = out;
+              if (!m.dbits)
+                vals[h] = (u32) ((int) xa[x] - (int) xb[x]);
               if (pid != NULL)
                 pid[h] = (rb[x] << m.abits) | ra[x];
-            }
-        }
-    }
+              if (HIST_C > 0)
+                fused_hist_add(fh, sd, (u32) HIST_C, out);
+            }
+        }
+    }
+}
+
+__global__ __launch_bounds__(256, 8)
+void merge_emit(MergeArgs m, const MergeTile *__restrict__ tiles, const u32 *__restrict__ cnt, const u32 *__restrict__ jbg,
+                const u32 *__restrict__ toff, u64 nhits, u64 *__restrict__ keys, u32 *__restrict__ vals, u32 *__restrict__ pid)
+{ SEED_PRIO(g_merge_prio);
+  __shared__ u32 loc[MT_A + 1];
+  __shared__ u32 sjb[MT_A];
+  __shared__ u32 sw4[4];
+  SortDigits none;
+  u32 facc = 0;
+  merge_emit_tile<0>(m, tiles, cnt, jbg, toff, blockIdx.x, gridDim.x, nhits, keys, vals, pid, loc, sjb, sw4,
+                     (u32 *) NULL, none, (u32 *) NULL, facc);
+}
+
+#define ME_GRID (256 * 8)
+template <int HIST_C>
+__global__ __launch_bounds__(256, 8)
+void merge_emit_hist(MergeArgs m, const MergeTile *__restrict__ tiles, const u32 *__restrict__ cnt, const u32 *__restrict__ jbg,
+                     const u32 *__restrict__ toff, u32 ntiles, u64 nhits, u64 *__restrict__ keys, u32 *__restrict__ vals,
+                     SortDigits sd, u32 *__restrict__ ghist)
+{ SEED_PRIO(g_merge_prio);
+  __shared__ u32 loc[MT_A + 1];
+  __shared__ u32 sjb[MT_A];
+  __shared__ u32 sw4[4];
+  extern __shared__ u32 fh[];
+  fused_hist_clear(fh, sd, (u32) HIST_C);
+  u32 facc = 0;
+  for (u32 tile = blockIdx.x; tile < ntiles; tile += gridDim.x)
+    { __syncthreads();
+      merge_emit_tile<HIST_C>(m, tiles, cnt, jbg, toff, tile, ntiles, nhits, keys, vals, (u32 *) NULL, loc, sjb, sw4,
+                              fh, sd, ghist, facc);
+    }
+  __syncthreads();
+  fused_hist_flush(fh, sd, (u32) HIST_C, ghist);
 }
 
 static size_t mw_tiles(u32 alen)  { return ((size_t) alen + MT_A - 1) / MT_A; }
@@ -751,6 +796,25 @@
   const u32 *toff = damar_merge_tile_counts(work, m->alen);
   const u32 *cnt = (const u32 *) ((char *) work + mw_off_cnt(m->alen)), *jb = (const u32 *) ((char *) work + mw_off_jb(m->alen));
   hipLaunchKernelGGL(merge_emit, dim3(ntiles), dim3(256), 0, st, *m, (const MergeTile *) work, cnt, jb, toff, nhits, keys, vals, pid);
+}
+
+int damar_launch_merge_emit_hist(const MergeArgs *m, void *work, u64 nhits, u64 *keys, u32 *vals, const SortDigits *sd,
+                                 u32 *ghist, hipStream_t st)
+{ if (nhits == 0)
+    return 0;
+  const u32 ntiles = (u32) mw_tiles(m->alen);
+  const u32 *toff = damar_merge_tile_counts(work, m->alen);
+  const u32 *cnt = (const u32 *) ((char *) work + mw_off_cnt(m->alen)), *jb = (const u32 *) ((char *) work + mw_off_jb(m->alen));
+  const u32 grid = ntiles < ME_GRID ? ntiles : ME_GRID;
+  const size_t own = (2 * MT_A + 1 + 4) * sizeof(u32), room = (160 * 1024) / 8;
+  if (own + damar_fused_hist_lds(sd, 8) <= room)
+    { hipLaunchKernelGGL(merge_emit_hist<8>, dim3(grid), dim3(256), damar_fused_hist_lds(sd, 8), st, *m, (const MergeTile *) work,
+                         cnt, jb, toff, ntiles, nhits, keys, vals, *sd, ghist);
+      return 8;
+    }
+  hipLaunchKernelGGL(merge_emit_hist<4>, dim3(grid), dim3(256), damar_fused_hist_lds(sd, 4), st, *m, (const MergeTile *) work,
+                     cnt, jb, toff, ntiles, nhits, keys, vals, *sd, ghist);
+  return 4;
 }
 
 #define SCREEN_MAX   48
diff --git a/damar_amd/csrc/shim.hip b/damar_amd/csrc/shim.hip
--- a/damar_amd/csrc/shim.hip
+++ b/damar_amd/csrc/shim.hip
@@ -665,6 +665,46 @@
   damar_sort_set_threads(forced ? forced : 1024);
 }
 
+static bool fused_hist_on(void)
+{ static int on = -1;
+  if (on < 0)
+    { const char *e = getenv("DAMAR_FUSED_HIST");
+      on = e ? (atoi(e) != 0) : 1;
+    }
+  return on != 0;
+}
+
+static int64 FH_checked[2] = { 0, 0 }, FH_bad[2] = { 0, 0 };
+extern "C" void damar_fused_hist_stats(int64 *out)
+{ out[0] = FH_checked[0];  out[1] = FH_bad[0];  out[2] = FH_checked[1];  out[3] = FH_bad[1]; }
+
+static void fused_hist_check(int which, const u64 *keys, u64 n, int lobit, int hibit, const u32 *ghist)
+{ static int on = -1;
+  static u32 *ref = NULL;
+  const size_t bytes = sizeof(u32) * 256 * DAMAR_SORT_MAXPASS;
+  if (on < 0)
+    { const char *e = getenv("DAMAR_FUSED_HIST_CHECK");
+      on = (e && atoi(e) > 0) ? 1 : 0;
+    }
+  if (!on)
+    return;
+  if (ref == NULL)
+    HIP_CHECK(hipMalloc((void **) &ref, bytes));
+  std::vector<u32> a(bytes / sizeof(u32)), b(bytes / sizeof(u32));
+  HIP_CHECK(hipMemsetAsync(ref, 0, bytes, G_st));
+  damar_sort_hist_only(keys, n, lobit, hibit, ref, G_st);
+  HIP_CHECK(hipMemcpyAsync(a.data(), ghist, bytes, hipMemcpyDeviceToHost, G_st));
+  HIP_CHECK(hipMemcpyAsync(b.data(), ref, bytes, hipMemcpyDeviceToHost, G_st));
+  HIP_CHECK(hipStreamSynchronize(G_st));
+  const SortDigits sd = damar_sort_digits(lobit, hibit);
+  u64 sum = 0;
+  for (int j = 0; j < 256; j++)
+    sum += b[j];
+  FH_checked[which] += 1;
+  if (memcmp(a.data(), b.data(), sizeof(u32) * 256 * (size_t) sd.npass) != 0 || sum != n)
+    FH_bad[which] += 1;
+}
+
 static int ilog2_ceil(u64 n)
 { int b = 0;
   while ((1ull << b) < n)
@@ -746,6 +786,7 @@
       v0 = v1 = NULL;
     }
 
+  bool fused = false;
   tick(0);
   if (biased || masked)
     {
@@ -775,6 +816,14 @@
       if (VERBOSE && biased)
         printf("\n   Revised kmer count = %u\n", nk);
     }
+  else if (!wide && fused_hist_on())
+    {
+      fused = true;
+      const SortDigits sd = damar_sort_digits(32, 32 + kbits);
+      u32 *ghist = damar_sort_fused_begin(sw, nk, G_st);
+      damar_launch_kmer_tuples_hist(&blk->d, K, nk, (u64 *) k0, &sd, ghist, G_st);
+      fused_hist_check(0, (const u64 *) k0, nk, 32, 32 + kbits, ghist);
+    }
   else
     damar_launch_kmer_tuples(&blk->d, K, nk, k0, wide, v0, G_st);
   tick(1);
@@ -785,6 +834,8 @@
           die();
         }
     }
+  else if (fused)
+    damar_radix_sort_split_u64_fused((u64 *) k0, (u64 *) k1, nk, 32, 32 + kbits, (u32 *) ix->codes, ix->pos, sw, G_st);
   else
     damar_radix_sort_split_u64((u64 *) k0, (u64 *) k1, nk, 32, 32 + kbits, (u32 *) ix->codes, ix->pos, sw, G_st);
   sort_check(sw);
@@ -1910,11 +1961,22 @@
       scw2  = arena_take(&G_tmp, damar_scan_workspace_bytes(total));
       sends = (u64 *) arena_take(&G_tmp, 64 * sizeof(u64));
 
-      damar_launch_merge_emit(&m, mw, total, k0, v0, NULL, G_st);
+      const int  lo = m.dbits ? m.dbits + (psort ? m.pbits : 0) : 0, hi = m.dbits + sbits;
+      const bool fused = fused_hist_on();
+      if (fused)
+        { const SortDigits sd = damar_sort_digits(lo, hi);
+          u32 *ghist = damar_sort_fused_begin(sw, total, G_st);
+          damar_launch_merge_emit_hist(&m, mw, total, k0, v0, &sd, ghist, G_st);
+          fused_hist_check(1, k0, total, lo, hi, ghist);
+        }
+      else
+        damar_launch_merge_emit(&m, mw, total, k0, v0, NULL, G_st);
       stage("merge_emit");
       tick(1);
-      int side = m.dbits ? damar_radix_sort_keys_u64(k0, k1, total, m.dbits + (psort ? m.pbits : 0), m.dbits + sbits, sw, G_st)
-                         : damar_radix_sort_u64(k0, v0, k1, v1, total, sbits, sw, G_st);
+      int side = !fused ? (m.dbits ? damar_radix_sort_keys_u64(k0, k1, total, lo, hi, sw, G_st)
+                                   : damar_radix_sort_u64(k0, v0, k1, v1, total, sbits, sw, G_st))
+                        : (m.dbits ? damar_radix_sort_keys_u64_fused(k0, k1, total, lo, hi, sw, G_st)
+                                   : damar_radix_sort_u64_fused(k0, v0, k1, v1, total, sbits, sw, G_st));
       sort_check(sw);
       keys = side ? k1 : k0;
       vals = side ? v1 : v0;
diff --git a/include/damar_hip.h b/include/damar_hip.h
--- a/include/damar_hip.h
+++ b/include/damar_hip.h
@@ -60,6 +60,7 @@
 void Match_Self(char *aname, HITS_DB *ablock, Align_Spec *settings);
 
 int64 damar_last_seeds(void *out, int64 cap);
+void  damar_fused_hist_stats(int64 *out);
 
 int damar_last_limit(void);
 
```

Result: no change. 51.21 billion, median of 3 (-0.1%).
